# stablecabal/gyre

Measured on AMD Instinct MI355X. Metric: SD1.5 512px 50-step images/sec (node), higher is better.
Workload: dtype bf16

## Files before the change

gyre_amd/_lib.py:

```python
from __future__ import annotations

import ctypes as C
import os
from typing import Optional

import torch

_HERE = os.path.dirname(os.path.abspath(__file__))
MAX_LEVELS = 8

F32, BF16, F16 = 0, 1, 2
_TORCH_DTYPE = {torch.float32: F32, torch.bfloat16: BF16, torch.float16: F16}
LIB_PATHS = {BF16: os.environ.get("GYRE_HIP_LIB") or os.path.join(_HERE, "libgyre_hip.so"),
             F16: os.environ.get("GYRE_HIP_LIB_F16") or os.path.join(_HERE, "libgyre_hip_f16.so")}
LIB_PATH = LIB_PATHS[BF16]
_default_storage = F16 if os.environ.get("GYRE_STORAGE", "").lower() in ("f16", "fp16", "float16", "half") else BF16
STORAGE_TORCH_DTYPE = {BF16: torch.bfloat16, F16: torch.float16}


def default_storage() -> int:
    return _default_storage


def set_default_storage(storage: int) -> int:
    global _default_storage
    if storage not in LIB_PATHS:
        raise ValueError("storage must be _lib.BF16 or _lib.F16")
    old, _default_storage = _default_storage, storage
    return old


def storage_for(dtype: torch.dtype) -> int:
    return F16 if dtype == torch.float16 else BF16 if dtype == torch.bfloat16 else _default_storage


class GyreError(RuntimeError):
    pass


class UNetCfg(C.Structure):
    _fields_ = [("in_channels", C.c_int32), ("out_channels", C.c_int32), ("n_levels", C.c_int32),
                ("block_out_channels", C.c_int32 * MAX_LEVELS), ("layers_per_block", C.c_int32),
                ("attn_levels", C.c_int32 * MAX_LEVELS), ("num_heads", C.c_int32 * MAX_LEVELS),
                ("transformer_depth", C.c_int32 * MAX_LEVELS), ("cross_attention_dim", C.c_int32),
                ("norm_num_groups", C.c_int32), ("use_linear_projection", C.c_int32),
                ("flip_sin_to_cos", C.c_int32), ("freq_shift", C.c_float)]


class VAECfg(C.Structure):
    _fields_ = [("in_channels", C.c_int32), ("out_channels", C.c_int32), ("latent_channels", C.c_int32),
                ("n_levels", C.c_int32), ("block_out_channels", C.c_int32 * MAX_LEVELS),
                ("layers_per_block", C.c_int32), ("norm_num_groups", C.c_int32)]


class T2ICfg(C.Structure):
    _fields_ = [("kind", C.c_int32), ("cin", C.c_int32), ("channels", C.c_int32 * 4), ("n_levels", C.c_int32),
                ("nums_rb", C.c_int32), ("ksize", C.c_int32), ("sk", C.c_int32), ("use_conv", C.c_int32)]


class CtrlCfg(C.Structure):
    _fields_ = [("in_channels", C.c_int32), ("n_levels", C.c_int32), ("block_out_channels", C.c_int32 * MAX_LEVELS),
                ("layers_per_block", C.c_int32), ("attn_levels", C.c_int32 * MAX_LEVELS), ("num_heads", C.c_int32 * MAX_LEVELS),
                ("transformer_depth", C.c_int32 * MAX_LEVELS), ("cross_attention_dim", C.c_int32), ("norm_num_groups", C.c_int32),
                ("use_linear_projection", C.c_int32), ("flip_sin_to_cos", C.c_int32), ("freq_shift", C.c_float),
                ("cond_channels", C.c_int32), ("cond_embed_channels", C.c_int32 * 4)]


class RRDBCfg(C.Structure):
    _fields_ = [(n, C.c_int32) for n in ("num_in_ch", "num_out_ch", "num_feat", "num_block", "num_grow_ch", "scale", "plus")]


class SwinIRCfg(C.Structure):
    _fields_ = [("in_chans", C.c_int32), ("embed_dim", C.c_int32), ("num_layers", C.c_int32), ("depths", C.c_int32 * 16),
                ("num_heads", C.c_int32 * 16), ("window_size", C.c_int32), ("mlp_hidden", C.c_int32), ("upscale", C.c_int32),
                ("img_range", C.c_float), ("resi_3conv", C.c_int32)]


class RdbEpilogue(C.Structure):
    _fields_ = [("bias", C.c_void_p), ("alpha", C.c_float), ("act", C.c_int32), ("r1", C.c_void_p), ("ldr1", C.c_int32),
                ("beta1", C.c_float), ("r2", C.c_void_p), ("ldr2", C.c_int32), ("beta2", C.c_float)]


class RdbConvArgs(C.Structure):
    _fields_ = [("x", C.c_void_p)] + [(n, C.c_int32) for n in ("ldx", "Cin", "B", "H", "W", "ups")] + [("w", C.c_void_p)] + \
               [(n, C.c_int32) for n in ("w_rows", "NT", "N_live")] + [("out", C.c_void_p), ("c0", C.c_int32), ("ldo", C.c_int32),
                                                                        ("epi", C.POINTER(RdbEpilogue)), ("wpack", C.c_void_p),
                                                                        ("wpack_bytes", C.c_size_t)]


class GemmTestArgs(C.Structure):
    _fields_ = [(n, C.c_int32) for n in ("conv", "M", "K", "N", "geglu", "B", "Hi", "Wi", "Cin", "stride", "pad", "ups", "Hup", "Wup",
                                         "wrap", "C1", "lda", "lda2", "ldc", "ldr", "rows_per_sample", "ld_rowbias", "samples",
                                         "out_mode", "out_dtype", "tokens", "ldt", "colstat_unit")] + \
               [(n, C.c_void_p) for n in ("A", "A2", "W", "bias", "rowbias", "residual", "out", "ws")] + [("ws_bytes", C.c_size_t)] + \
               [("sc_A", C.c_void_p), ("sc_A2", C.c_void_p)] + [(n, C.c_int32) for n in ("sc_K", "sc_C1", "sc_lda", "sc_lda2")]


class LoraPair(C.Structure):
    _fields_ = [("up", C.c_void_p), ("down", C.c_void_p), ("dtype", C.c_int), ("rank", C.c_int), ("scale", C.c_float)]


class DeltaTerm(C.Structure):
    _fields_ = [("kind", C.c_int), ("up", C.c_void_p * 2), ("down", C.c_void_p * 2), ("dtype", C.c_int * 2), ("rank", C.c_int * 2),
                ("w1", C.c_void_p), ("O1", C.c_int), ("I1", C.c_int), ("scale", C.c_float)]


LORA_MAX_PAIRS = 8
DELTA_MAX_TERMS = 8
DELTA_LORA, DELTA_HADA, DELTA_KRON, DELTA_FULL = 0, 1, 2, 3
_vp, _i, _sz, _f = C.c_void_p, C.c_int, C.c_size_t, C.c_float
_SIGS = {
    "gyre_abi_version": (C.c_int, []),
    "gyre_storage_dtype": (C.c_int, []),
    "gyre_last_error": (C.c_char_p, []),
    "gyre_last_launch_count": (C.c_int64, []),
    "gyre_unet_create": (_i, [C.POINTER(UNetCfg), _i, C.POINTER(_vp)]),
    "gyre_unet_destroy": (None, [_vp]),
    "gyre_unet_num_params": (_i, [_vp]),
    "gyre_unet_param_key": (C.c_char_p, [_vp, _i]),
    "gyre_unet_set_weight": (_i, [_vp, C.c_char_p, _vp, _i, C.POINTER(C.c_int64), _i, _vp]),
    "gyre_unet_set_weight_lora": (_i, [_vp, C.c_char_p, _vp, _i, C.POINTER(C.c_int64), _i, _i, C.POINTER(LoraPair), _vp]),
    "gyre_unet_set_weight_delta": (_i, [_vp, C.c_char_p, _vp, _i, C.POINTER(C.c_int64), _i, _i, C.POINTER(DeltaTerm), _vp]),
    "gyre_unet_finalize": (_i, [_vp, _vp]),
    "gyre_unet_workspace_bytes": (_sz, [_vp, _i, _i, _i, _i]),
    "gyre_unet_forward": (_i, [_vp, _vp, _vp, _i, _vp, _vp, _i, _i, _i, _i, _i, _vp, _sz, _vp, _i]),
    "gyre_unet_set_context": (_i, [_vp, _vp, _vp, _i, _i, _i]),
    "gyre_unet_set_context_slot": (_i, [_vp, _vp, _vp, _i, _i, _i, _i]),
    "gyre_unet_select_context": (_i, [_vp, _i]),
    "gyre_unet_hint_uniform_timestep": (_i, [_vp, _i]),
    "gyre_unet_hint_cfg_pairs": (_i, [_vp, _i]),
    "gyre_unet_set_tome": (_i, [_vp, _i]),
    "gyre_unet_set_tiling": (_i, [_vp, _i]),
    "gyre_vae_set_tiling": (_i, [_vp, _i]),
    "gyre_unet_debug_tap": (_i, [_vp, C.c_char_p, _vp, _sz]),
    "gyre_unet_debug_grad_tap": (_i, [_vp, C.c_char_p, _vp, _sz]),
    "gyre_unet_forward_ex": (_i, [_vp, _vp, _vp, _i, _vp, _vp, _i, _i, _i, _i, _i, _vp, _sz, _vp, _i, _vp]),
    "gyre_unet_forward_ctrl": (_i, [_vp, _vp, _vp, _i, _vp, _vp, _i, _i, _i, _i, _i, _vp, _sz, _vp, _i, _vp,
                                    C.POINTER(_vp), _i, _i, _vp, C.POINTER(_vp), _i]),
    "gyre_unet_vjp_workspace_bytes": (_sz, [_vp, _i, _i, _i, _i]),
    "gyre_unet_vjp": (_i, [_vp, _vp, _vp, _i, _vp, _vp, _i, _i, _i, _i, _i, _vp, _i, _vp, _sz, _vp, _i, _vp, _i, _vp]),
    "gyre_unet_vjp_begin": (_i, [_vp, _vp, _vp, _i, _vp, _vp, _i, _i, _i, _i, _i, _vp, _sz, _vp, _i, _vp]),
    "gyre_unet_vjp_finish": (_i, [_vp, _vp, _vp, _i, _vp, _i]),
    "gyre_unet_vjp_finish_range": (_i, [_vp, _vp, _vp, _i, _vp, _i, _i, _i]),
    "gyre_unet_vjp_pending": (_i, [_vp]),
    "gyre_vae_create": (_i, [C.POINTER(VAECfg), _i, C.POINTER(_vp)]),
    "gyre_vae_destroy": (None, [_vp]),
    "gyre_vae_num_params": (_i, [_vp]),
    "gyre_vae_param_key": (C.c_char_p, [_vp, _i]),
    "gyre_vae_set_weight": (_i, [_vp, C.c_char_p, _vp, _i, C.POINTER(C.c_int64), _i, _vp]),
    "gyre_vae_finalize": (_i, [_vp, _vp]),
    "gyre_vae_workspace_bytes": (_sz, [_vp, _i, _i, _i, _i]),
    "gyre_vae_encode": (_i, [_vp, _vp, _vp, _i, _i, _i, _i, _vp, _sz, _vp, _i]),
    "gyre_vae_decode": (_i, [_vp, _vp, _vp, _i, _i, _i, _i, _vp, _sz, _vp, _i]),
    "gyre_vae_decode_vjp_workspace_bytes": (_sz, [_vp, _i, _i, _i]),
    "gyre_vae_decode_vjp": (_i, [_vp, _vp, _vp, _i, _i, _i, _i, _vp, _i, _vp, _sz, _vp, _i, _vp, _i]),
    "gyre_t2i_create": (_i, [C.POINTER(T2ICfg), _i, C.POINTER(_vp)]),
    "gyre_t2i_destroy": (None, [_vp]),
    "gyre_t2i_num_params": (_i, [_vp]),
    "gyre_t2i_param_key": (C.c_char_p, [_vp, _i]),
    "gyre_t2i_set_weight": (_i, [_vp, C.c_char_p, _vp, _i, C.POINTER(C.c_int64), _i, _vp]),
    "gyre_t2i_finalize": (_i, [_vp, _vp]),
    "gyre_t2i_workspace_bytes": (_sz, [_vp, _i, _i, _i]),
    "gyre_t2i_forward": (_i, [_vp, _vp, _vp, _i, _i, _i, _i, _vp, _sz, C.POINTER(_vp), _i, _i]),
    "gyre_rrdb_create": (_i, [C.POINTER(RRDBCfg), _i, C.POINTER(_vp)]),
    "gyre_rrdb_destroy": (None, [_vp]),
    "gyre_rrdb_num_params": (_i, [_vp]),
    "gyre_rrdb_param_key": (C.c_char_p, [_vp, _i]),
    "gyre_rrdb_set_weight": (_i, [_vp, C.c_char_p, _vp, _i, C.POINTER(C.c_int64), _i, _vp]),
    "gyre_rrdb_finalize": (_i, [_vp, _vp]),
    "gyre_rrdb_workspace_bytes": (_sz, [_vp, _i, _i, _i]),
    "gyre_rrdb_forward": (_i, [_vp, _vp, _vp, _i, _i, _i, _i, _vp, _sz, _vp, _i]),
    "gyre_rrdb_set_path": (_i, [_vp, _i]),
    "gyre_swinir_create": (_i, [C.POINTER(SwinIRCfg), _i, C.POINTER(_vp)]),
    "gyre_swinir_destroy": (None, [_vp]),
    "gyre_swinir_num_params": (_i, [_vp]),
    "gyre_swinir_param_key": (C.c_char_p, [_vp, _i]),
    "gyre_swinir_set_weight": (_i, [_vp, C.c_char_p, _vp, _i, C.POINTER(C.c_int64), _i, _vp]),
    "gyre_swinir_finalize": (_i, [_vp, _vp]),
    "gyre_swinir_workspace_bytes": (_sz, [_vp, _i, _i, _i]),
    "gyre_swinir_forward": (_i, [_vp, _vp, _vp, _i, _i, _i, _i, _vp, _sz, _vp, _i]),
    "gyre_ctrl_create": (_i, [C.POINTER(CtrlCfg), _i, C.POINTER(_vp)]),
    "gyre_ctrl_destroy": (None, [_vp]),
    "gyre_ctrl_num_params": (_i, [_vp]),
    "gyre_ctrl_param_key": (C.c_char_p, [_vp, _i]),
    "gyre_ctrl_set_weight": (_i, [_vp, C.c_char_p, _vp, _i, C.POINTER(C.c_int64), _i, _vp]),
    "gyre_ctrl_finalize": (_i, [_vp, _vp]),
    "gyre_ctrl_bind_workspace_bytes": (_sz, [_vp, _i, _i, _i, _i]),
    "gyre_ctrl_bind": (_i, [_vp, _vp, _vp, _i, _i, _i, _i, _vp, _i, _i, _i, _vp, _sz]),
    "gyre_ctrl_workspace_bytes": (_sz, [_vp, _i, _i, _i, _i]),
    "gyre_ctrl_forward": (_i, [_vp, _vp, _vp, _i, _vp, _i, _i, _i, _vp, _sz, C.POINTER(_f), _i, _i, _i, C.POINTER(_vp), _i, _i]),
    "gyre_prof_set_mask": (_i, [C.c_uint64]),
    "gyre_prof_num_classes": (_i, []),
    "gyre_prof_class_name": (C.c_char_p, [_i]),
    "gyre_prof_collect": (_i, [C.POINTER(C.c_int64), C.POINTER(C.c_double), C.POINTER(C.c_double), C.POINTER(C.c_double)]),
    "gyre_debug_force_gemm_cfg": (_i, [_i]),
    "gyre_debug_set_splitk_workspace": (_i, [_vp, _sz]),
    "gyre_debug_set_ar_workspace": (_i, [_vp, _sz]),
    "gyre_debug_set_wblk_workspace": (_i, [_vp, _sz]),
    "gyre_debug_attn_redo_count": (C.c_long, []),
    "gyre_debug_attn_plan": (_i, [_i] * 10 + [C.POINTER(C.c_int32)]),
    "gyre_debug_attn_bwd_plan": (_i, [_i] * 6 + [C.POINTER(C.c_int32)]),
    "gyre_debug_attn_tables": (_i, [_i, C.POINTER(C.c_int32), _i]),
    "gyre_debug_xattn_stamps": (_i, [_vp]),
    "gyre_debug_force_attn_variant": (_i, [_i]),
    "gyre_debug_gemm_ablation": (_i, [_i]),
    "gyre_debug_ln_linear_folds": (_i, [_i, _i, _i, _i]),
    "gyre_debug_gn_uses_small": (_i, [_i, _i, _i, _i]),
    "gyre_op_gemm_test": (_i, [_vp, C.POINTER(GemmTestArgs)]),
    "gyre_debug_gemm_plan": (_i, [C.POINTER(GemmTestArgs), C.POINTER(C.c_int32)]),
    "gyre_debug_gemm_tiles": (_i, [C.POINTER(C.c_int32), _i]),
    "gyre_set_batch_invariant": (_i, [_i]),
    "gyre_get_batch_invariant": (_i, []),
    "gyre_op_groupnorm": (_i, [_vp, _vp, _vp, _i, _i, _i, _i, _i, _vp, _vp, _f, _i, _vp, _sz, _vp]),
    "gyre_op_groupnorm_workspace": (_sz, [_i, _i, _i, _i]),
    "gyre_op_gemm_splitk_bytes": (_sz, [_i, _i, _i, _i, _i]),
    "gyre_op_conv3x3_colstats": (_i, [_vp, _vp, _i, _i, _i, _i, _vp, _i, _vp, _vp, _i, _i, _i, _vp, _vp, _sz, _vp, _sz, _vp]),
    "gyre_op_linear_colstats": (_i, [_vp, _vp, _i, _i, _vp, _i, _vp, _vp, _i, _i, _vp, _vp, _sz, _vp, _sz, _vp]),
    "gyre_op_groupnorm_colstats": (_i, [_vp, _vp, _vp, _i, _i, _i, _i, _i, _vp, _vp, _f, _i, _vp, _i, _vp, _i, _i, _vp, _sz, _vp]),
    "gyre_op_gn_fold": (_i, [_vp, _vp, _i, _i, _i, _i, _vp, _vp, _f, _vp, _vp, _i, _vp, _i, _i, _vp, _sz, _vp, _vp]),
    "gyre_op_layernorm": (_i, [_vp, _vp, _i, _i, _vp, _vp, _f, _vp]),
    "gyre_op_linear": (_i, [_vp, _vp, _i, _i, _vp, _i, _vp, _vp, _i, _vp]),
    "gyre_op_linear_t": (_i, [_vp, _vp, _i, _i, _vp, _i, _vp, _i, _i, _vp]),
    "gyre_op_ln_linear_workspace": (_sz, [_i, _i, _i]),
    "gyre_op_ln_linear": (_i, [_vp, _vp, _i, _i, _vp, _vp, _f, _vp, _i, _vp, _i, _i, _vp, _i, _vp, _i, _vp, _sz, _vp]),
    "gyre_op_linear_rowstats_parts": (_i, [_i, _i, _i, _i]),
    "gyre_op_linear_rowstats": (_i, [_vp, _vp, _i, _i, _vp, _i, _vp, _vp, _vp, _vp]),
    "gyre_op_conv3x3": (_i, [_vp, _vp, _i, _i, _i, _i, _vp, _i, _vp, _vp, _i, _i, _i, _vp]),
    "gyre_op_conv3x3_shortcut": (_i, [_vp, _vp, _i, _i, _i, _i, _vp, _i, _vp, _vp, _i, _vp, _i, _vp, _vp, _vp, _sz, _vp]),
    "gyre_op_compose_proj_out": (_i, [_vp, _vp, _vp, _vp, _vp, _i, _vp, _vp]),
    "gyre_op_conv3x3_nchw": (_i, [_vp, _vp, _i, _i, _i, _i, _vp, _i, _vp, _vp, _i, _i]),
    "gyre_op_repack_conv_weight": (_i, [_vp, _vp, _i, _i, _i, _i, _i, _vp]),
    "gyre_op_repack_conv_weight_scaled": (_i, [_vp, _vp, _i, _i, _i, _i, _i, _i, _f, _vp]),
    "gyre_op_repack_linear_weight": (_i, [_vp, _vp, _i, _i, _i, _vp]),
    "gyre_op_repack_bias": (_i, [_vp, _vp, _i, _i, _vp]),
    "gyre_op_repack_lora": (_i, [_vp, _vp, _i, _i, _i, _i, _i, _i, _i, _f, _i, C.POINTER(LoraPair), _vp]),
    "gyre_op_repack_delta": (_i, [_vp, _vp, _i, _i, _i, _i, _i, _i, _i, _f, _i, C.POINTER(DeltaTerm), _vp]),
    "gyre_op_lyco_core": (_i, [_vp, _vp, _i, _vp, _i, _i, _i, _i, _i, _vp]),
    "gyre_op_merge_delta": (_i, [_vp, _vp, _i, _i, _i, _i, C.POINTER(DeltaTerm), _vp, _i]),
    "gyre_op_attention": (_i, [_vp, _vp, _i, _vp, _i, _vp, _i, _i, _i, _i, _i, _i, _vp, _i]),
    "gyre_op_qkv": (_i, [_vp, _vp, _i, _i, _vp, _i, _vp, _vp, _i]),
    "gyre_op_attention_ex": (_i, [_vp, _vp, _i, _vp, _i, _vp, _i, _i, _i, _i, _i, _i, _vp, _i, _i]),
    "gyre_op_groupnorm_bwd_workspace": (_sz, [_i, _i, _i, _i]),
    "gyre_op_groupnorm_bwd": (_i, [_vp, _vp, _vp, _i, _i, _i, _i, _i, _vp, _vp, _f, _i, _vp, _vp, _vp, _sz, _vp, _vp]),
    "gyre_op_layernorm_bwd": (_i, [_vp, _vp, _vp, _i, _i, _vp, _f, _vp, _vp]),
    "gyre_op_geglu_bwd": (_i, [_vp, _vp, _vp, _i, _i, _vp]),
    "gyre_op_attention_bwd_workspace": (_sz, [_i, _i, _i, _i, _i]),
    "gyre_op_attention_bwd": (_i, [_vp, _vp, _i, _vp, _i, _vp, _i, _vp, _i, _vp, _i, _i, _i, _i, _i, _i, _i, _vp, _sz,
                                   _vp, _i, _vp, _i, _vp, _i]),
    "gyre_op_tome_workspace": (_sz, [_i, _i, _i]),
    "gyre_op_tome_merge": (_i, [_vp, _vp, _i, _vp, _i, _i, _i, _i, _i, _vp, _sz, _vp, _vp, _i, _vp, _vp]),
    "gyre_op_tome_merge_ex": (_i, [_vp, _vp, _i, _vp, _i, _i, _i, _i, _i, _vp, _sz, _vp, _vp, _i, _vp, _vp, _vp, _vp]),
    "gyre_op_tome_unmerge": (_i, [_vp, _vp, _i, _i, _i, _i, _vp, _vp, _vp, _vp, _i]),
    "gyre_op_timestep_embedding": (_i, [_vp, _vp, _i, _i, _i, _f, _vp]),
    "gyre_op_rowvec_linear": (_i, [_vp, _vp, _i, _i, _vp, _vp, _i, _i, _vp, _i]),
    "gyre_op_timestep_linear": (_i, [_vp, _vp, _i, _i, _i, _f, _vp, _vp, _vp, _i, _vp, _i]),
    "gyre_op_cross_attention_block": (_i, [_vp, _vp, _i, _i, _i, _i, _vp, _vp, _f, _vp, _vp, _vp, _i, _i, _vp, _vp, _vp, _sz, _vp, _vp]),
    "gyre_op_nchw_to_nhwc": (_i, [_vp, _vp, _i, _i, _i, _i, _i, _vp]),
    "gyre_op_copy_probe": (_i, [_vp, _vp, _vp, _sz]),
    "gyre_op_pixel_unshuffle8": (_i, [_vp, _vp, _i, _i, _i, _i, _i, _vp]),
    "gyre_op_avgpool2": (_i, [_vp, _vp, _i, _i, _i, _i, _vp]),
    "gyre_op_relu": (_i, [_vp, _vp, _sz]),
    "gyre_op_silu": (_i, [_vp, _vp, _sz]),
    "gyre_op_rdb_tile": (_i, [C.POINTER(C.c_int32), C.POINTER(C.c_int32)]),
    "gyre_op_rdb_conv": (_i, [_vp, C.POINTER(RdbConvArgs)]),
    "gyre_op_rdb_epilogue": (_i, [_vp, _vp, _i, _i, _i, _sz, C.POINTER(RdbEpilogue)]),
    "gyre_op_pixel_unshuffle": (_i, [_vp, _vp, _i, _i, _i, _i, _i, _i, _vp]),
    "gyre_op_win_bias": (_i, [_vp, _vp, _i, _vp]),
    "gyre_op_win_attn": (_i, [_vp, _vp, _i, _vp, _i, _vp, _i, _i, _i, _i, _i]),
    "gyre_op_ln_live": (_i, [_vp, _vp, _i, _sz, _i, _vp, _vp, _f, _vp, _i]),
    "gyre_op_swin_act": (_i, [_vp, _vp, _sz, _i, _f]),
    "gyre_op_swin_entry": (_i, [_vp, _vp, _i, _i, _sz, _vp, _f, _vp]),
    "gyre_op_swin_exit": (_i, [_vp, _vp, _i, _i, _sz, _vp, _f, _vp, _i]),
    "gyre_op_ctrl_emit": (_i, [_vp, _vp, _i, _i, _i, _i, _f, _i, _vp, _i, _i, _i]),
}
EXPORTED_SYMBOLS = tuple(_SIGS)

_libs: dict = {}
import threading as _threading
_tls = _threading.local()


def lib(storage: Optional[int] = None) -> C.CDLL:
    storage = _default_storage if storage is None else storage
    l = _libs.get(storage)
    if l is None:
        path = LIB_PATHS[storage]
        if not os.path.exists(path):
            raise GyreError(f"{path} is missing: run `python -c 'import __graft_entry__ as g; g.build()'` "
                            f"(hipcc --offload-arch=gfx950).  There is no non-HIP fallback.")
        try:
            l = C.CDLL(path, mode=getattr(os, "RTLD_LOCAL", 0) | getattr(os, "RTLD_NOW", 2))
        except OSError as e:
            raise GyreError(f"cannot load {path}: {e}") from e
# ... 67 lines not shown
```

gyre_amd/csrc/kernels.h:

```cpp
#pragma once
#include "common.h"

int launch_nchw_to_nhwc(hipStream_t st, const void* x, int dtype, int B, int C, int HW, int Cpad, bf16_t* y);
int launch_add_nchw_into_nhwc(hipStream_t st, const void* r, int dtype, int B, int C, int HW, int Cpad, bf16_t* y);
int launch_ctx_to_bf16(hipStream_t st, const void* x, int dtype, size_t n, bf16_t* y);
int launch_dup_batch(hipStream_t st, const void* src, void* dst, size_t outer, size_t inner_bytes);
int launch_add_f32(hipStream_t st, float* y, const float* x, size_t n);
int launch_compose_proj(hipStream_t st, const bf16_t* Wp, const bf16_t* W2, const float* b2, const float* bp, int C, bf16_t* Wc, float* bc);
int launch_verify_hints(hipStream_t st, const int64_t* t, int B, int check_t, const void* x, size_t bytes_per_half, int check_pairs, int* flag);
int launch_timestep_embedding(hipStream_t st, const int64_t* t, int B, int dim, int flip, float shift, float* out);
int launch_rowvec_linear(hipStream_t st, float* x, int B, int K, const bf16_t* W, const float* bias, int N,
                         int act_in_silu, float* out, int ldo);
int launch_timestep_linear(hipStream_t st, const int64_t* t, int B, int dim, int flip, float shift, float* emb_scratch,
                           const bf16_t* W, const float* bias, int N, float* out, int ldo);

struct GnParams {
    const bf16_t* x; const bf16_t* x2; int C1;
    int B, HW, C, G;
    const float* gamma; const float* beta; float eps; int silu;
    float* partial;
    float* scale_shift;
    int nchunks;
    bf16_t* y;
    float* mean_rstd = nullptr;
    const float* cs_x = nullptr; int cs_x_chunks = 0;
    const float* cs_x2 = nullptr; int cs_x2_chunks = 0;
    int cs_unit = 0;
};
size_t gn_workspace_bytes(int B, int HW, int C, int G);
int gn_pick_chunks(int B, int HW, int C);
int gemm_set_batch_invariant(int canonical_samples);
int gemm_get_batch_invariant();
long gemm_planner_state();
enum : int {
    GEMM_DBG_NO_SM            = 0x20,
    GEMM_DBG_SM_NO_SPLITK     = 0x40,
    GEMM_DBG_NO_SC_FOLD       = 0x80,
    GEMM_DBG_CONV_ZERO_PAGE   = 0x200,
    GEMM_DBG_NO_4S            = 0x400,
    GEMM_DBG_NO_LN_FOLD       = 0x800,
    GEMM_DBG_NO_GN_FOLD       = 0x1000,
    GEMM_DBG_NO_XATTN         = 0x2000,
    GEMM_DBG_NO_GEGLU_4S      = 0x4000,
    GEMM_DBG_LN_STATS_PASS    = 0x8000,
    GEMM_DBG_GEGLU_NO_LN_FOLD = 0x10000,
    GEMM_DBG_GN_STATS_PASS    = 0x20000,
    GEMM_DBG_NO_128x160       = 0x40000,
    GEMM_DBG_NO_CS_128x160    = 0x100000,
    GEMM_DBG_NO_AR            = 0x200000,
    GEMM_DBG_AR_ALL           = 0x400000,
    GEMM_DBG_NO_4S_128_TILES  = 0x800000,
    GEMM_DBG_TWO_STAGE_LINEAR = 0x1000000,
    GEMM_DBG_DEEP_RING        = 0x2000000,
    GEMM_DBG_NO_W_BLOCK       = 0x4000000,
    GEMM_DBG_TWO_STAGE_CONV   = 0x8000000,
    GEMM_DBG_NO_POUT_FOLD     = 0x10000000,
};
int launch_groupnorm_stats(hipStream_t st, const GnParams& p);
int launch_groupnorm_apply(hipStream_t st, const GnParams& p);
bool gn_use_small(int HW, int C, int C1, int G);
bool gn_accepts_colstats(const GnParams& p);
int launch_groupnorm_small(hipStream_t st, const GnParams& p);
int launch_gn_fold(hipStream_t st, const GnParams& p, const bf16_t* W, const float* bias, int N, bf16_t* Wf, float* bf);
int launch_layernorm(hipStream_t st, const bf16_t* x, int M, int C, const float* gamma, const float* beta, float eps,
                     bf16_t* y);
int launch_layernorm_stats(hipStream_t st, const bf16_t* x, int M, int C, float eps, float* stats);

int launch_nhwc_to_nchw_f32(hipStream_t st, const bf16_t* x, int B, int C, int HW, int Cpad, float* y);
int launch_repack_conv(hipStream_t st, const void* w, int dtype, int O, int I, int KH, int KW, int Ipad, bf16_t* out,
                       float scale = 1.f);
int launch_repack_linear(hipStream_t st, const void* w, int dtype, int O, int I, int geglu_interleave, bf16_t* out);
int launch_cast_f32(hipStream_t st, const void* w, int dtype, size_t n, int geglu_interleave, float* out, float scale = 1.f);
int launch_copy_probe(hipStream_t st, const void* src, void* dst, size_t bytes);
#define GYRE_LORA_MAX_PAIRS 8
struct LoraArgs {
    const void* up[GYRE_LORA_MAX_PAIRS];
    const void* down[GYRE_LORA_MAX_PAIRS];
    int dtype[GYRE_LORA_MAX_PAIRS];
    int rank[GYRE_LORA_MAX_PAIRS];
    float s[GYRE_LORA_MAX_PAIRS];
    int n = 0;
};
int launch_repack_lora(hipStream_t st, const void* base, int base_dtype, int O, int I, int KH, int KW, int Ipad, int geglu_interleave,
                       float scale_p, const LoraArgs& la, bf16_t* out);
#define GYRE_DELTA_MAX_TERMS 8
enum { DELTA_LORA = 0, DELTA_HADA = 1, DELTA_KRON = 2, DELTA_FULL = 3 };
struct DeltaArgs {
    int kind[GYRE_DELTA_MAX_TERMS];
    const void* up[GYRE_DELTA_MAX_TERMS][2];
    const void* down[GYRE_DELTA_MAX_TERMS][2];
    int dtype[GYRE_DELTA_MAX_TERMS][2];
    int rank[GYRE_DELTA_MAX_TERMS][2];
    const float* w1[GYRE_DELTA_MAX_TERMS];
    int O1[GYRE_DELTA_MAX_TERMS], I1[GYRE_DELTA_MAX_TERMS];
    float s[GYRE_DELTA_MAX_TERMS];
    int n = 0;
};
int launch_repack_delta(hipStream_t st, const void* base, int base_dtype, int O, int I, int KH, int KW, int Ipad, int geglu_interleave,
                        float scale_p, const DeltaArgs& da, bf16_t* out);
int launch_merge_delta(hipStream_t st, const void* base, int base_dtype, int O, int I, const DeltaArgs& da, void* out, int out_dtype);
int launch_lyco_core(hipStream_t st, const void* core, int core_dtype, const void* right, int right_dtype, int A, int B, int C, int T,
                     float* out);

int launch_pixel_unshuffle8(hipStream_t st, const void* x, int dtype, int B, int c, int H, int W, bf16_t* y);
int launch_avgpool2(hipStream_t st, const bf16_t* x, int B, int H, int W, int C, bf16_t* y);
int launch_relu(hipStream_t st, bf16_t* x, size_t n);
int launch_nhwc_to_nchw(hipStream_t st, const bf16_t* x, int B, int C, int HW, int Cpad, void* y, int dtype);

struct RdbEpilogueArgs {
    const float* bias = nullptr; float alpha = 1.f; int act = 0;
    const bf16_t* r1 = nullptr; int ldr1 = 0; float beta1 = 0.f;
    const bf16_t* r2 = nullptr; int ldr2 = 0; float beta2 = 0.f;
};
void rdb_tile(int* th, int* tw);
size_t rdb_wpack_bytes(int NT, int Cin);
int launch_rdb_wpack(hipStream_t st, const bf16_t* W, int rows, int Cin, int NT, bf16_t* wd);
int launch_rdb_conv(hipStream_t st, const bf16_t* x, int ldx, int Cin, int B, int H, int W, int ups, const bf16_t* wd, int NT,
                    int N_live, bf16_t* out, int ldo, const RdbEpilogueArgs& e);
int rdb_conv_check(const bf16_t* x, int ldx, int Cin, int B, int H, int W, int ups, const bf16_t* wd, int NT, int N_live,
                   const bf16_t* out, int ldo, const RdbEpilogueArgs& e);
int launch_rdb_epilogue(hipStream_t st, bf16_t* x, int ldo, int N_live, size_t npix, const RdbEpilogueArgs& e);
int launch_rdb_copy(hipStream_t st, const bf16_t* src, int lds, bf16_t* dst, int ldd, int C, size_t npix);
int rdb_unshuffle_channels(int c, int r);
int launch_pixel_unshuffle(hipStream_t st, const void* x, int dtype, int B, int c, int H, int W, int r, bf16_t* y);

int win_attn_check(const bf16_t* qkv, int ld_qkv, const bf16_t* o, int ld_o, const float* bias, int B, int H, int W, int heads, int shift);
int launch_win_attn(hipStream_t st, const bf16_t* qkv, int ld_qkv, bf16_t* o, int ld_o, const float* bias, int B, int H, int W, int heads,
                    int shift);
int launch_win_bias(hipStream_t st, const float* table, int heads, float* out);
int launch_ln_live(hipStream_t st, const bf16_t* x, int ldx, size_t M, int C, const float* gamma, const float* beta, float eps, bf16_t* y,
                   int ldy);
int launch_swin_act(hipStream_t st, bf16_t* x, size_t n, int mode, float slope);
int launch_swin_entry(hipStream_t st, const void* x, int dtype, int B, size_t HW, const float* mean3, float range, bf16_t* y);
int launch_swin_exit(hipStream_t st, const bf16_t* x, int ldx, int B, size_t HW, const float* mean3, float range, void* y, int dtype);

int launch_silu(hipStream_t st, bf16_t* x, size_t n);
int launch_ctrl_emit(hipStream_t st, const bf16_t* f, int B, int C, int HW, int Cpad, float scale, int accumulate, void* out,
                     int out_dtype, int out_B, int out_b0);

enum { GEMM_LINEAR = 0, GEMM_CONV3 = 1 };
enum { OUT_BF16 = 0, OUT_NCHW = 1, OUT_BF16_T = 2 };
struct GemmParams {
    const bf16_t* A = nullptr; const bf16_t* A2 = nullptr; int C1 = 0;
    int lda = 0, lda2 = 0;
    int mode = GEMM_LINEAR;
    int Hi = 0, Wi = 0, Cin = 0;
    int Ho = 0, Wo = 0, stride = 1, pad = 1, ups = 0;
    const bf16_t* W = nullptr; int K = 0; int N = 0; int M = 0;
    const float* bias = nullptr;
    const float* rowbias = nullptr;
    int rows_per_sample = 1; int ld_rowbias = 0;
    const bf16_t* residual = nullptr; int ldr = 0;
    int geglu = 0;
    void* out = nullptr; int ldc = 0; int out_mode = OUT_BF16; int out_dtype = 1;
    int tokens_per_batch = 0; int ldt = 0;
    bf16_t* vt_out = nullptr; int vt_col0 = 0;
    const bf16_t* zero_page = nullptr;
    int force_cfg = 0;
    int debug = 0;
    int Hup = 0, Wup = 0;
    int samples = 0;
    float* splitk_ws = nullptr; size_t splitk_ws_bytes = 0;
    int batch = 1; size_t bsA = 0, bsW = 0, bsC = 0;
    const float* ln_colsum = nullptr; const float* ln_stats = nullptr;
    float* rowstat_out = nullptr;
    const float* ln_parts = nullptr; int ln_nparts = 0; float ln_eps = 1e-5f;
    float* colstat_out = nullptr; int colstat_unit = 0;
    const void* w_packed = nullptr; int ar_ok = 0, no_ar = 0;
    const bf16_t* W_blk = nullptr;
    size_t w_sample_stride = 0;
    const bf16_t* sc_A = nullptr; const bf16_t* sc_A2 = nullptr; int sc_lda = 0, sc_lda2 = 0, sc_C1 = 0, sc_K = 0;
    int wrap = 0;
};
int launch_concat_rows(hipStream_t st, const bf16_t* a, int K1, const bf16_t* b, int K2, int N, bf16_t* out);
int launch_ln_fold(hipStream_t st, const bf16_t* W, int N, int K, const float* gamma, const float* beta, const float* bias,
                   bf16_t* Wf, float* colsum, float* bias_out);
size_t gemm_ar_packed_bytes(int N, int K);
int launch_ar_pack(hipStream_t st, const bf16_t* W, int N, int K, void* out);
int launch_w_block(hipStream_t st, const bf16_t* W, int N, int K, bf16_t* out);
bool conv_out_supports(int C, int O);
int launch_conv_out(hipStream_t st, const bf16_t* x, int B, int H, int W, int C, const bf16_t* Wt, const float* bias, int O,
                    void* out, int out_dtype);
struct GemmPlan {
    int cfg = 3, splits = 1;
    size_t ws_bytes = 0;
    int colstat_rows = 0;
    int rowstat_parts = 0;
    bool ln_fold = false;
    bool per_sample_w = false;
    bool shortcut_fold = false;
    bool w_block = false;
    bool ar_pack = false;
    int vt_align = 0;
};
GemmPlan gemm_plan(const GemmParams& p);
int launch_gemm(hipStream_t st, const GemmParams& p);
int launch_gemm(hipStream_t st, const GemmParams& p, const GemmPlan& plan);
void gemm_plan_loop_form(const GemmParams& p, const GemmPlan& plan, int* nst, int* uni);
int gemm_tile_table(int* out, int cap);


struct AttnParams {
    const bf16_t* q; int ldq;
    const bf16_t* k; int ldk;
    const bf16_t* vt; int ldvt;
    bf16_t* o; int ldo;
    int B, H, Nq, Nk, D;
    int k_prescaled = 0;
    int always_check = 0;
    unsigned* redo_counter = nullptr;
};
enum AttnVariant {
    ATTN_VAR_AUTO = 0,
    ATTN_VAR_V1 = 1,
    ATTN_VAR_V2_PLAIN = 2,
    ATTN_VAR_V2_FOLD = 3,
    ATTN_VAR_V2_Q64 = 4,
    ATTN_VAR_V3 = 5,
    ATTN_VAR_NO_QLOOP = 6,
    ATTN_VAR_ALWAYS_CHECK = 7,
    ATTN_VAR_AUTO_ALIAS = 8,
};
enum AttnFamily { ATTN_FAM_V1 = 0, ATTN_FAM_V2_PLAIN = 1, ATTN_FAM_V2_FOLD = 2, ATTN_FAM_V3 = 3 };
struct AttnPlan {
    int status = 0; std::string error;
    int family = 0, D = 0, QI = 0, row = -1;
    int PD = 0, slots = 0, stage_bytes = 0;
    int lds_bytes = 0;
    dim3 grid;
    bool qloop = false; int qiter = 1;
    bool always_check = false;
    int ablation = 0;
    double flops = 0, bytes = 0;
};
AttnPlan attn_plan(const AttnParams& p, int variant);
constexpr int ATTN_PLAN_INTS = 12, ATTN_BWD_PLAN_INTS = 10;
int launch_attention(hipStream_t st, const AttnParams& p);

struct XattnParams {
    const bf16_t* x; int ldx;
    const bf16_t* wq;
    const float* q_colsum; const float* q_bias;
    const float* ln_parts; int ln_nparts; const float* ln_stats; float ln_eps;
    const bf16_t* k; const bf16_t* vt; int ldvt;
    const bf16_t* wo; const float* bo;
    bf16_t* out; int ldo;
    float* rowstat_out;
    int M, rows_per_sample, Nk, heads;
};

bool xattn_supports(int C, int heads, int Nq, int Nk, int M);
int launch_xattn(hipStream_t st, const XattnParams& p, int C);

struct GnBwdParams {
    const bf16_t* x; const bf16_t* x2; int C1;
    int B, HW, C, G;
// ... 55 lines not shown
```

gyre_amd/csrc/kernels_gemm.hip:

```cpp
#include "gemm_shared.h"
#include <cstdio>
#include <cstdlib>
#include <cstdlib>
#include <atomic>
#include <utility>


typedef unsigned gemm_u32x4 __attribute__((ext_vector_type(4)));
__device__ __forceinline__ uint4 nt_load_u4(const void* p) {
    const gemm_u32x4 v = __builtin_nontemporal_load((const gemm_u32x4*)p);
    return make_uint4(v.x, v.y, v.z, v.w);
}

template <int MI, int NI>
__device__ __forceinline__ void gemm_epilogue(const GemmParams& p, f32x4_t (&acc)[MI][NI], int m_base, int n_base,
                                              int fr, int fq) {
#pragma unroll
    for (int i = 0; i < MI; ++i) {
        const int m = m_base + i * 16 + fr;
        if (m >= p.M) continue;
        const float* rbias = p.rowbias ? p.rowbias + (size_t)(m / p.rows_per_sample) * p.ld_rowbias : nullptr;
        if (p.geglu) {
#pragma unroll
            for (int j = 0; j + 1 < NI; j += 2) {
// ... 1086 lines not shown
    GyreProfScope prof_(kcls, st, 2.0 * p.M * (double)p.N * p.K,
                        a_bytes + (double)p.N * p.K * 2.0 + (double)p.M * n_out * 2.0 * (p.residual ? 2.0 : 1.0));
#define GYRE_GEMM8_GO(MODE_, UNI_)                                                                                  \
    do {                                                                                                            \
        auto kern = k_gemm8<BM, BN, WM, WN, MODE_, UNI_>;                                                             \
        static std::atomic<unsigned long long> attr_done{0};                                                                               \
        if (gyre_lds_attr_needed(attr_done))                                                                                            \
            (void)hipFuncSetAttribute((const void*)kern, hipFuncAttributeMaxDynamicSharedMemorySize, lds_attr);     \
        hipLaunchKernelGGL(kern, dim3(grid), dim3(512), lds, st, p, tiles_m, tiles_n, splits, nst);                      \
    } while (0)
    if (p.colstat_out && splits == 1) {
        if constexpr (BN == 320 || BN == 160) {
#define GYRE_GEMM8_CS(MODE_, UNI_)                                                                                  \
    do {                                                                                                            \
        auto kern = k_gemm8<BM, BN, WM, WN, MODE_, UNI_, false, false, true>;                                       \
        static std::atomic<unsigned long long> attr_done{0};                                                        \
        if (gyre_lds_attr_needed(attr_done))                                                                        \
            (void)hipFuncSetAttribute((const void*)kern, hipFuncAttributeMaxDynamicSharedMemorySize, lds_attr);     \
        hipLaunchKernelGGL(kern, dim3(grid), dim3(512), lds, st, p, tiles_m, tiles_n, splits, nst);                      \
    } while (0)
            if (p.mode == GEMM_LINEAR) GYRE_GEMM8_CS(GEMM_LINEAR, true);
            else if (uni) GYRE_GEMM8_CS(GEMM_CONV3, true);
            else GYRE_GEMM8_CS(GEMM_CONV3, false);
#undef GYRE_GEMM8_CS
        } else {
            GYRE_FAIL(-6, "gemm: column statistics exist for the 320- and 160-wide tiles only (see GemmPlan::colstat_rows)");
        }
    } else if (p.mode == GEMM_LINEAR && p.rowstat_out) {
        auto kern = k_gemm8<BM, BN, WM, WN, GEMM_LINEAR, true, false, true>;
        static std::atomic<unsigned long long> attr_done{0};
        if (gyre_lds_attr_needed(attr_done))
            (void)hipFuncSetAttribute((const void*)kern, hipFuncAttributeMaxDynamicSharedMemorySize, lds_attr);
        hipLaunchKernelGGL(kern, dim3(grid), dim3(512), lds, st, p, tiles_m, tiles_n, splits, nst);
    } else if (p.mode == GEMM_LINEAR && p.ln_colsum) {
        auto kern = k_gemm8<BM, BN, WM, WN, GEMM_LINEAR, true, true>;
        static std::atomic<unsigned long long> attr_done{0};
        if (gyre_lds_attr_needed(attr_done))
            (void)hipFuncSetAttribute((const void*)kern, hipFuncAttributeMaxDynamicSharedMemorySize, lds_attr);
        hipLaunchKernelGGL(kern, dim3(grid), dim3(512), lds, st, p, tiles_m, tiles_n, splits, nst);
    } else if (p.mode == GEMM_LINEAR) {
        GYRE_GEMM8_GO(GEMM_LINEAR, true);
    } else {
        if (uni) GYRE_GEMM8_GO(GEMM_CONV3, true); else GYRE_GEMM8_GO(GEMM_CONV3, false);
    }
#undef GYRE_GEMM8_GO
    GYRE_LAUNCH_CHECK();
    prof_.stop();
    if (splits > 1) return launch_splitk_reduce(st, p, splits);
    return 0;
}

static const GemmTile g_tiles[] = {
    {   1, 128, 128, GEMM_K_4W,  true,    0,   0,     false,   false,  false,       false,   false },
    {   2, 256,  64, GEMM_K_4W,  true,    0,   0,     false,   false,  false,       false,   false },
    {   3,  64,  64, GEMM_K_4W,  true,    0,   0,     false,   false,  false,       false,   false },
    {   4, 256, 320, GEMM_K_8W,  false, 160, 256,     true,    true,   true,        false,   true  },
    {   5, 128, 320, GEMM_K_8W,  false,  80, 128,     true,    true,   true,        false,   true  },
    {   6, 256, 256, GEMM_K_8W,  true,  128,   0,     true,    true,   true,        false,   true  },
    {   7, 128, 256, GEMM_K_8W,  true,   64,   0,     true,    true,   true,        false,   true  },
    {   8, 128, 160, GEMM_K_8W,  false,  80, 128,     true,    true,   true,        false,   true  },
    {  12, 256, 128, GEMM_K_8W,  true,    0,   0,     false,   false,  false,       false,   true  },
    {  20, 192, 320, GEMM_K_4S,  true,    0,   0,     false,   false,  false,       false,   true  },
    {  21, 256, 256, GEMM_K_4S,  true,    0,   0,     false,   false,  false,       false,   true  },
    {  22, 128, 320, GEMM_K_4S,  true,    0,   0,     false,   false,  false,       false,   true  },
    {  23, 128, 256, GEMM_K_4S,  true,    0,   0,     false,   false,  false,       false,   true  },
    {  24, 256, 320, GEMM_K_4S,  true,    0, 256,     false,   true,   false,       true,    true  },
    {  30, 256,  64, GEMM_K_AR,  true,   64,   0,     true,    true,   false,       false,   false },
    {  32,  64,  64, GEMM_K_SM,  false,  64,   0,     false,   false,  false,       false,   true  },
};
const GemmTile* gemm_tile(int cfg) {
    for (const GemmTile& t : g_tiles)
        if (t.id == cfg) return &t;
    return nullptr;
}
static thread_local void* g_dbg_ar_ws = nullptr;
static thread_local size_t g_dbg_ar_ws_bytes = 0;
static long ar_grid_min() {
    static const long v = getenv("GYRE_AR_GRID_MIN") ? atol(getenv("GYRE_AR_GRID_MIN")) : 192;
    return v;
}
static int pick_cfg(const GemmParams& p, int* splits_out) {
    *splits_out = 1;
    const bool trans = p.out_mode == OUT_BF16_T;
    auto tiles = [&](int bm, int bn) { return (long)((p.M + bm - 1) / bm) * ((p.N + bn - 1) / bn); };
    auto tiles_of = [&](int id) { const GemmTile* t = gemm_tile(id); return tiles(t->bm, t->bn); };
    auto eff = [&](long t, int slots) { long cap = 256L * slots; long waves = (t + cap - 1) / cap; return (double)t / (double)(waves * cap); };
    auto neff = [&](int bn) { long nt = (p.N + bn - 1) / bn; return (double)p.N / (double)(nt * bn); };
    auto meff = [&](int bm) { long mt = (p.M + bm - 1) / bm; return (double)p.M / (double)(mt * bm); };
    double best = -1; int cfg = 3;
    auto consider = [&](int id, double speed, int slots) {
        const GemmTile* t = gemm_tile(id);
        double s = speed * eff(tiles(t->bm, t->bn), slots) * neff(t->bn) * meff(t->bm);
        if (s > best) { best = s; cfg = id; }
    };
    consider(3, 0.30, 4);
    consider(1, 0.55, 2);
    consider(2, 0.50, 2);
    const bool wrap_only4 = p.mode == GEMM_CONV3 && p.wrap != 0;
    if (!trans && p.batch <= 1 && (p.ar_ok || p.w_packed || g_dbg_ar_ws) && !p.no_ar && !(p.debug & GEMM_DBG_NO_AR) && p.M >= 4096 &&
        (p.N >= 3 * p.K || (p.debug & GEMM_DBG_AR_ALL)) && gemm_ar_supports(p) &&
        ((long)((p.M + 255) / 256) * gemm_ar_nsplit(p) >= ar_grid_min() || (p.debug & GEMM_DBG_AR_ALL)))
        return 30;
    if (!trans && p.batch <= 1 && !wrap_only4) {
        auto big = [&](int id, double speed) { if (tiles_of(id) >= 160) consider(id, speed, 1); };
        if (!p.geglu && p.N % 320 == 0) { big(4, 0.92); big(5, 0.88); }
        if (!p.geglu && p.N % 160 == 0 && !(p.debug & GEMM_DBG_NO_128x160)) big(8, 0.90);
        if (p.N % 256 == 0) { big(6, 0.95); big(7, 0.62); }
        if (p.mode == GEMM_CONV3 && !p.geglu && p.N % 128 == 0 && p.N % 256 != 0 && p.N % 160 != 0 && !(p.debug & GEMM_DBG_NO_128x160)) big(12, 0.90);
        const int nk_ = (p.K + BK - 1) / BK;
        if (!(p.debug & GEMM_DBG_NO_4S) && p.N % 320 == 0 && (p.mode == GEMM_CONV3 ? nk_ >= 20 : nk_ >= 32) && gemm4s_supports(p, 24)) {
            big(24, 1.00);
            if (!(p.debug & GEMM_DBG_NO_4S_128_TILES) && p.mode == GEMM_CONV3 && nk_ >= 45 && tiles_of(24) >= 128 && tiles_of(24) < 160) consider(24, 1.25, 1);
        }
        else if (!(p.debug & (GEMM_DBG_NO_4S | GEMM_DBG_NO_GEGLU_4S)) && p.geglu && (long)p.N > (long)p.M && p.N % 320 == 0 && gemm4s_supports(p, 24))
            big(24, 1.00);
        const int nk = (p.K + BK - 1) / BK;
        if (p.out_mode == OUT_BF16 && !p.geglu && p.K >= 2048 && p.N % 4 == 0) {
            auto tryk = [&](int id, double speed) {
                const int bm = gemm_tile(id)->bm, bn = gemm_tile(id)->bn;
                long t = tiles(bm, bn);
                if (t >= 160 || t < 1) return;
                int sp = (int)((id == 8 ? 512 : 256) / t);
                const int min_steps = bm >= 256 ? 16 : 8;
                while (sp > 1 && nk / sp < min_steps) --sp;
                if (sp < 2) return;
                double sc = speed * eff(t * sp, 1) * neff(bn) * 0.85;
                if (sc > best) { best = sc; cfg = id; *splits_out = sp; }
            };
            if (p.N % 320 == 0) tryk(5, 0.88);
            if (p.N % 160 == 0 && !(p.debug & GEMM_DBG_NO_128x160)) tryk(8, 0.92);
            if (p.N % 256 == 0) tryk(7, 0.62);
            if (p.N % 320 == 0 && p.K >= 5000) {
                tryk(4, 1.05);
                if (!(p.debug & GEMM_DBG_NO_4S) && gemm4s_supports(p, 24)) tryk(24, 1.10);
            }
        }
    }
    if (!trans && !(p.debug & GEMM_DBG_NO_SM) && gemm_sm_supports(p)) {
        if (cfg <= 3 && *splits_out == 1) cfg = 32;
        else if (*splits_out > 1 && p.mode == GEMM_LINEAR && tiles_of(32) <= 512 && !(p.debug & GEMM_DBG_SM_NO_SPLITK)) { cfg = 32; *splits_out = 1; }
    }
    return cfg;
}

static thread_local int g_force_cfg = 0;
static thread_local float* g_dbg_ws = nullptr;
static thread_local size_t g_dbg_ws_bytes = 0;
static thread_local int g_gemm_debug = 0;
extern "C" int gyre_debug_gemm_ablation(int bits) { int old = g_gemm_debug; g_gemm_debug = bits; return old; }
extern "C" int gyre_debug_force_gemm_cfg(int cfg) { int old = g_force_cfg; g_force_cfg = cfg; return old; }
extern "C" int gyre_debug_set_splitk_workspace(void* ws, size_t bytes) { g_dbg_ws = (float*)ws; g_dbg_ws_bytes = bytes; return 0; }
extern "C" int gyre_debug_set_ar_workspace(void* ws, size_t bytes) { g_dbg_ar_ws = ws; g_dbg_ar_ws_bytes = bytes; return 0; }

static int pick_cfg_nosplit(const GemmParams& p) {
    GemmParams q = p; q.K = q.K < 2048 ? q.K : 2040;
    int sp; return pick_cfg(q, &sp);
}

static thread_local int g_invariant_batch = 0;
int gemm_set_batch_invariant(int n) { const int old = g_invariant_batch; g_invariant_batch = n < 0 ? 0 : n; return old; }
int gemm_get_batch_invariant() { return g_invariant_batch; }
long gemm_planner_state() {
    return (long)(unsigned)g_gemm_debug | ((long)(g_force_cfg & 0xffff) << 32) | ((long)(g_invariant_batch & 0xfff) << 48) | ((long)(g_dbg_ar_ws ? 1 : 0) << 60);
}

static int plan_cfg(const GemmParams& p, int* splits) {
    const int inv = g_invariant_batch;
    if (inv > 0 && p.samples > 0 && p.M % p.samples == 0) {
        GemmParams q = p;
        q.M = p.M / p.samples * inv;
        int c = pick_cfg(q, splits);
        if (*splits > 1) return c;
        return pick_cfg_nosplit(p);
    }
    return pick_cfg(p, splits);
}

static bool gemm_staged_epilogue_ok(const GemmParams& p) {
    const int n_out = p.geglu ? p.N / 2 : p.N;
    return p.out_mode == OUT_BF16 && (n_out % 8) == 0 && (p.ldc % 8) == 0 && (!p.residual || (p.ldr % 8) == 0) &&
           (((size_t)p.out | (size_t)p.residual) & 15) == 0;
}
static GemmParams gemm_normalised(const GemmParams& p0) {
    GemmParams p = p0;
    if (!p.force_cfg) p.force_cfg = g_force_cfg;
    p.debug = g_gemm_debug;
    if (!p.A2) { p.C1 = p.mode == GEMM_LINEAR ? p.K : p.Cin; p.A2 = p.A; p.lda2 = p.lda; }
    if (p.rows_per_sample <= 0) p.rows_per_sample = 1;
    if (p.sc_K && (!p.sc_A2 || p.sc_A2 == p.sc_A)) { p.sc_A2 = p.sc_A; p.sc_lda2 = p.sc_lda; p.sc_C1 = p.sc_K; }
    return p;
}

GemmPlan gemm_plan(const GemmParams& p0) {
    const GemmParams p = gemm_normalised(p0);
    GemmPlan pl;
    if (p.M <= 0 || p.N <= 0 || p.K <= 0) return pl;
    if (p.force_cfg) { pl.cfg = p.force_cfg & 0xff; pl.splits = std::max(1, (p.force_cfg >> 8) & 0xff); }
    else pl.cfg = plan_cfg(p, &pl.splits);
    if (pl.splits > 1) pl.ws_bytes = (size_t)pl.splits * p.M * p.N * sizeof(float);
    const GemmTile* t = gemm_tile(pl.cfg);
    if (!t) return pl;
    pl.vt_align = t->vt_align;
    pl.ar_pack = t->kind == GEMM_K_AR;
    pl.w_block = t->w_block && !(p.debug & GEMM_DBG_NO_W_BLOCK) && p.K % 64 == 0 && p.N % 8 == 0 && p.K > 1024 && p.batch <= 1 &&
                 !p.w_sample_stride && p.out_mode != OUT_BF16_T && (p.mode != GEMM_CONV3 || (p.Cin % 64 == 0 && p.C1 % 64 == 0));
    if (p.force_cfg || g_invariant_batch > 0 || p.batch > 1 || !gemm_staged_epilogue_ok(p)) return pl;
    const bool one_split = pl.splits == 1;
    const bool plain_linear = p.mode == GEMM_LINEAR && !p0.A2 && p.K % 8 == 0;
    pl.per_sample_w = t->per_sample_w && one_split && plain_linear && !(p.debug & GEMM_DBG_NO_GN_FOLD) && !p.geglu && !p.vt_out &&
                      !p.ln_colsum && p.N % 8 == 0 && p.M % p.rows_per_sample == 0 && p.rows_per_sample % t->bm == 0;
    pl.shortcut_fold = t->shortcut && !(p.debug & GEMM_DBG_NO_SC_FOLD) && p.mode == GEMM_CONV3 && p.sc_K && p.sc_K % BK == 0 &&
                       p.Cin % BK == 0 && p.C1 % BK == 0 && p.K == 9 * p.Cin + p.sc_K && p.stride == 1 && p.pad == 1 && !p.ups &&
                       p.Hi == p.Ho && p.Wi == p.Wo && !p.wrap;
    pl.ln_fold = t->ln_fold && one_split && plain_linear && !(p.debug & GEMM_DBG_NO_LN_FOLD) &&
                 !(p.geglu && ((p.debug & GEMM_DBG_GEGLU_NO_LN_FOLD) || !t->geglu)) && !p.rowbias && p.N % 4 == 0 &&
                 (!p.vt_out || (t->vt_align && p.vt_col0 % t->vt_align == 0));
    if (t->rowstats && one_split && plain_linear && !(p.debug & (GEMM_DBG_LN_STATS_PASS | GEMM_DBG_NO_LN_FOLD)) && !p.geglu &&
        !p.vt_out && !p.ln_colsum && p.N % 8 == 0)
        pl.rowstat_parts = t->kind == GEMM_K_AR ? gemm_ar_nsplit(p) : (p.N + t->bn - 1) / t->bn;
    const int unit = p.colstat_unit;
    if (unit > 0 && !(p.debug & GEMM_DBG_GN_STATS_PASS) && !p.geglu && !p.vt_out && !p.ln_colsum && !p.rowstat_out && p.K % 8 == 0 &&
        p.N % 8 == 0 && p.N % unit == 0 && 320 % unit == 0 && p.M % p.rows_per_sample == 0) {
        int rows = 0;
        if (!one_split) rows = cs_red_colblock(p.N, unit) <= 2048 ? cs_red_rows(p.rows_per_sample) : 0;
        else if (t->bn % unit == 0 && (t->kind != GEMM_K_4S || p.mode == GEMM_CONV3) && !(pl.cfg == 8 && (p.debug & GEMM_DBG_NO_CS_128x160)))
            rows = t->cs_rows;
        if (rows && p.rows_per_sample % rows == 0) pl.colstat_rows = rows;
    }
    return pl;
}

void gemm_plan_loop_form(const GemmParams& p0, const GemmPlan& plan, int* nst, int* uni) {
    const GemmParams p = gemm_normalised(p0);
    const GemmTile* t = gemm_tile(plan.cfg);
    *nst = 0; *uni = 0;
    if (!t) return;
    if (t->kind == GEMM_K_4W) *uni = p.mode == GEMM_CONV3 && gemm_conv_uniform_tap(p) ? 1 : 0;
    if (t->kind != GEMM_K_8W) return;
    bool u = true;
    gemm8_loop_form(p, t->bm, t->bn, plan.splits, nst, &u);
    *uni = p.mode == GEMM_CONV3 && u ? 1 : 0;
}
int gemm_tile_table(int* out, int cap) {
    int n = 0;
    for (const GemmTile& t : g_tiles) {
        if (4 * n + 4 <= cap) { out[4 * n] = t.id; out[4 * n + 1] = t.bm; out[4 * n + 2] = t.bn; out[4 * n + 3] = (int)t.kind; }
        ++n;
    }
    return n;
}

__global__ __launch_bounds__(256) void k_w_block(const bf16_t* __restrict__ W, int N, int K, bf16_t* __restrict__ out) {
    const size_t t = (size_t)blockIdx.x * 256 + threadIdx.x;
    const int kv = K >> 3;
    if (t >= (size_t)N * kv) return;
    const int n = (int)(t / kv), k = (int)(t - (size_t)n * kv) * 8;
    const uint4 v = *(const uint4*)(W + (size_t)n * K + k);
    *(uint4*)(out + ((size_t)(n >> 3) * (K >> 6) + (k >> 6)) * 512 + (n & 7) * 64 + (k & 63)) = v;
}
int launch_w_block(hipStream_t st, const bf16_t* W, int N, int K, bf16_t* out) {
    if (K % 64 || N % 8 || N < 8 || K < 64) GYRE_FAIL(-1, "w_block: K must be a multiple of 64 and N of 8");
    const size_t total = (size_t)N * (K / 8);
    hipLaunchKernelGGL(k_w_block, dim3((unsigned)((total + 255) / 256)), dim3(256), 0, st, W, N, K, out);
    GYRE_LAUNCH_CHECK();
    return 0;
}
static thread_local bf16_t* g_dbg_blk_ws = nullptr;
static thread_local size_t g_dbg_blk_ws_bytes = 0;
extern "C" int gyre_debug_set_wblk_workspace(void* ws, size_t bytes) { g_dbg_blk_ws = (bf16_t*)ws; g_dbg_blk_ws_bytes = bytes; return 0; }
int launch_gemm(hipStream_t st, const GemmParams& p0) { return launch_gemm(st, p0, gemm_plan(p0)); }
int launch_gemm(hipStream_t st, const GemmParams& p0, const GemmPlan& plan) {
    GemmParams p = gemm_normalised(p0);
    if (p.M <= 0 || p.N <= 0 || p.K <= 0) GYRE_FAIL(-1, "gemm: empty problem");
    if (p.K % 8) GYRE_FAIL(-1, "gemm: K must be a multiple of 8");
    if (p.C1 % 8) GYRE_FAIL(-1, "gemm: source split must be a multiple of 8");
    if (p.mode == GEMM_CONV3) {
        if (p.Cin % 8 || p.K != 9 * p.Cin + p.sc_K) GYRE_FAIL(-1, "conv3x3: Cin must be a multiple of 8 and K == 9*Cin (+ the folded shortcut's channels)");
        if (p.sc_K && (p.sc_K % BK || p.Cin % BK || !p.sc_A || p.stride != 1 || p.pad != 1 || p.ups || p.Hi != p.Ho || p.Wi != p.Wo || p.wrap ||
                       (p.sc_A2 && p.sc_A2 != p.sc_A && (p.sc_C1 <= 0 || p.sc_C1 >= p.sc_K || p.sc_C1 % BK))))
            GYRE_FAIL(-1, "conv3x3: a folded shortcut needs a stride-1 / pad-1 convolution and whole 64-channel steps on both sides");
    }
    if (p.out_mode == OUT_BF16 && (p.N % 4 || p.ldc % 4 || (p.residual && p.ldr % 4)))
        GYRE_FAIL(-1, "gemm: N / ldc / ldr must be multiples of 4 for bf16 row-major output");
    if (p.geglu && (p.N % 32)) GYRE_FAIL(-1, "gemm: GEGLU needs N % 32 == 0");
    if (p.out_mode == OUT_BF16_T && p.tokens_per_batch <= 0) GYRE_FAIL(-1, "gemm: tokens_per_batch required");
    if (p.batch > 1 && (p.mode != GEMM_LINEAR || p.out_mode != OUT_BF16 || p.bias || p.residual || p.rowbias || p.geglu || p.vt_out))
        GYRE_FAIL(-1, "gemm: the batched form is a plain bf16 matrix product");
    if (p.vt_out) {
        if (p.out_mode != OUT_BF16 || p.geglu || p.residual || p.tokens_per_batch <= 0 || p.tokens_per_batch % 8 || p.ldt % 8 ||
            p.vt_col0 <= 0 || p.vt_col0 >= p.N || p.N % 8)
            GYRE_FAIL(-1, "gemm: bad fused Q|K|V arguments");
    }
    if (p.rowstat_out && (p.ln_colsum || p.mode != GEMM_LINEAR || p0.A2 || p.geglu || p.vt_out || p.out_mode != OUT_BF16 || p.batch > 1))
        GYRE_FAIL(-1, "gemm: row statistics come from a plain single-source linear problem with bf16 row-major output");
    if (p.ln_colsum && (p.mode != GEMM_LINEAR || p0.A2 || !p.bias || (!p.ln_stats && p.ln_nparts <= 0) || (p.ln_nparts > 0 && !p.ln_parts) ||
                        p.rowbias || p.out_mode != OUT_BF16 || p.batch > 1))
        GYRE_FAIL(-1, "gemm: the folded LayerNorm needs a single-source linear problem with row statistics, bias and bf16 row-major output");
    {
        static const bool dump = getenv("GYRE_GEMM_DUMP") != nullptr;
        if (dump)
            fprintf(stderr, "GYRE_GEMM mode=%d M=%d N=%d K=%d Cin=%d C1=%d Hi=%d Wi=%d stride=%d ups=%d geglu=%d res=%d rowbias=%d "
                            "out=%d vt=%d batch=%d samples=%d cfg=%d splits=%d\n", p.mode, p.M, p.N, p.K, p.Cin, p.C1, p.Hi, p.Wi,
                    p.stride, p.ups, p.geglu, p.residual ? 1 : 0, p.rowbias ? 1 : 0, p.out_mode, p.vt_out ? 1 : 0, p.batch, p.samples,
                    plan.cfg, plan.splits);
    }
    int cfg = plan.cfg, splits = plan.splits;
    if (splits > 1) {
        if (!p.splitk_ws) { p.splitk_ws = g_dbg_ws; p.splitk_ws_bytes = g_dbg_ws_bytes; }
        if (!p.splitk_ws || p.splitk_ws_bytes < (size_t)splits * p.M * p.N * sizeof(float)) {
            splits = 1;
            cfg = pick_cfg_nosplit(p);
        }
    }
    const GemmTile* t = gemm_tile(cfg);
    if (!t) GYRE_FAIL(-1, "gemm: unknown tile config");
    if (p.vt_out && (!t->vt_align || splits > 1 || p.vt_col0 % t->vt_align))
        GYRE_FAIL(-6, "gemm: fused Q|K|V needs an 8-wave tile config whose wave tiles align with the V columns");
    if (p.colstat_out && (plan.colstat_rows <= 0 || splits != plan.splits))
        GYRE_FAIL(-6, "gemm: column statistics are not available for this problem / tile configuration (see GemmPlan::colstat_rows)");
    if (p.w_sample_stride && (!t->per_sample_w || splits > 1 || p.mode != GEMM_LINEAR || p.rows_per_sample % t->bm || p.M % p.rows_per_sample))
        GYRE_FAIL(-6, "gemm: per-sample weights need an unsplit 8-wave tile config whose row blocks do not straddle samples (GemmPlan::per_sample_w)");
    if (p.mode == GEMM_CONV3 && p.wrap && t->kind != GEMM_K_4W) GYRE_FAIL(-6, "gemm: circular padding (tiling) exists in the 4-wave tile configs only");
    if (p.sc_K && !t->shortcut) GYRE_FAIL(-6, "gemm: the folded shortcut exists in the pipelined 256x320 tile only (see GemmPlan::shortcut_fold)");
    if (!p.W_blk && g_dbg_blk_ws && plan.w_block && g_dbg_blk_ws_bytes >= (size_t)p.N * p.K * 2) {
        int rc = launch_w_block(st, p.W, p.N, p.K, g_dbg_blk_ws);
        if (rc) return rc;
        p.W_blk = g_dbg_blk_ws;
    }
    if (p.W_blk && (!t->w_block || p.K % 64 || p.N % 8 || p.w_sample_stride || (p.mode == GEMM_CONV3 && (p.Cin % 64 || p.C1 % 64)))) p.W_blk = nullptr;
    if (t->kind == GEMM_K_AR) {
        if (splits > 1 || !gemm_ar_supports(p)) GYRE_FAIL(-6, "gemm: problem outside the A-resident kernel's domain (K = 320 / 640 linear, bf16 row-major output)");
        const void* wpk = p.w_packed;
        if (!wpk) {
            if (!g_dbg_ar_ws || g_dbg_ar_ws_bytes < gemm_ar_packed_bytes(p.N, p.K))
                GYRE_FAIL(-6, "gemm: the A-resident kernel needs the packed weight copy (GemmParams::w_packed or gyre_debug_set_ar_workspace)");
            int rc = launch_ar_pack(st, p.W, p.N, p.K, g_dbg_ar_ws);
            if (rc) return rc;
            wpk = g_dbg_ar_ws;
        }
        return launch_gemm_ar(st, p, wpk);
    }
    if (t->kind == GEMM_K_SM) {
        if (splits > 1) GYRE_FAIL(-6, "gemm: the small-problem kernel has no split-K form");
        return launch_gemm_sm(st, p);
    }
    if (p.rowstat_out && (!t->rowstats || splits > 1 || !gemm_staged_epilogue_ok(p)))
        GYRE_FAIL(-6, "gemm: row statistics need an unsplit 8-wave tile config with the staged epilogue (see GemmPlan::rowstat_parts)");
    if (p.ln_colsum && (!t->ln_fold || splits > 1 || !gemm_staged_epilogue_ok(p)))
        GYRE_FAIL(-6, "gemm: the folded LayerNorm needs an unsplit 8-wave tile config with the staged epilogue (see GemmPlan::ln_fold)");
    if (t->kind != GEMM_K_4W) {
        if (p.out_mode == OUT_BF16_T) GYRE_FAIL(-6, "gemm: transposed output needs a 4-wave config");
        if (p.geglu && !t->geglu) GYRE_FAIL(-6, "gemm: GEGLU needs an even fragment count per wave");
        p.zero_page = gemm_zero_page_for_current_device();
        if (!p.zero_page) GYRE_FAIL(-5, "gemm: cannot allocate the zero page");
    }
    switch (cfg) {
        case 1: return launch_cfg<128, 128, 2, 2>(st, p);
        case 2: return launch_cfg<256, 64, 4, 1>(st, p);
        case 3: return launch_cfg<64, 64, 2, 2>(st, p);
        case 4: return launch_cfg8<256, 320, 4, 2>(st, p, KC_G8_CONV_256x320, splits);
        case 5: return launch_cfg8<128, 320, 2, 4>(st, p, KC_G8_CONV_128x320, splits);
        case 6: return launch_cfg8<256, 256, 4, 2>(st, p, KC_G8_CONV_256x256, splits);
        case 12:
            if (p.mode != GEMM_CONV3) GYRE_FAIL(-6, "gemm: the 256x128 tile is a convolution config");
            return launch_cfg8<256, 128, 4, 2>(st, p, KC_G8_X1, splits);
        case 7: return launch_cfg8<128, 256, 2, 4>(st, p, KC_G8_CONV_128x256, splits);
        case 8: return launch_cfg8<128, 160, 4, 2>(st, p, KC_G8_CONV_128x160, splits);
        default: return launch_gemm4s(st, p, cfg, splits);
    }
}
```

gyre_amd/csrc/kernels_gemm4s.hip:

```cpp
#include "gemm_shared.h"
#include <atomic>
#include <type_traits>

template <int V> using ic = std::integral_constant<int, V>;

__device__ __forceinline__ void glds_saddr(unsigned lds_addr, unsigned voff, const void* sbase) {
    asm volatile("s_mov_b32 m0, %0\n\ts_nop 0\n\tglobal_load_lds_dwordx4 %1, %2" ::"s"(lds_addr), "v"(voff), "s"(sbase) : "memory");
}
__device__ __forceinline__ void glds_vaddr(unsigned lds_addr, const void* vptr) {
    asm volatile("s_mov_b32 m0, %0\n\ts_nop 0\n\tglobal_load_lds_dwordx4 %1, off" ::"s"(lds_addr), "v"(vptr) : "memory");
}

typedef __attribute__((ext_vector_type(4))) int srd_t;
__device__ __forceinline__ void blds(unsigned lds_addr, unsigned voff, srd_t srd, unsigned soff) {
    asm volatile("s_mov_b32 m0, %0\n\ts_nop 0\n\tbuffer_load_dwordx4 %1, %2, %3 offen lds" ::"s"(lds_addr), "v"(voff), "s"(srd), "s"(soff) : "memory");
}
__device__ __forceinline__ srd_t make_srd(const void* base, unsigned bytes) {
    const size_t a = (size_t)base;
    return srd_t{(int)(unsigned)a, (int)(unsigned)(a >> 32), (int)bytes, 0x00020000};
}

template <int BM, int BN, int WM, int WN, int MODE, int ZFILL, bool LNF = false, bool CS = false>
__global__ __launch_bounds__(WM * WN * 64, WM * WN / 4) void k_gemm4s(GemmParams p, int tiles_m, int tiles_n, int splits, int group_m) {
    constexpr int NW = WM * WN;
    constexpr int TM = BM / WM, TN = BN / WN, MI = TM / 32, NI = TN / 32;
    constexpr int AP = BM / (8 * NW), BP = BN / (8 * NW);
    constexpr int DTOT = AP + BP, DH0 = (DTOT + 1) / 2;
    constexpr int STAGE = (BM + BN) * 128;
    static_assert((NW == 4 || NW == 8) && TM % 32 == 0 && TN % 32 == 0 && BM % (8 * NW) == 0 && BN % (8 * NW) == 0 &&
                  MI * NI * 16 <= (NW == 4 ? 256 : 160) && (NI == 4 || NI == 5), "tile shape");
    extern __shared__ __attribute__((aligned(16))) char smem[];

    const int ntiles = tiles_m * tiles_n;
    const int split = blockIdx.x / ntiles;
    const int bid = xcd_tile_id(blockIdx.x - split * ntiles, ntiles);
    int tm, tn;
    if ((long)p.M < (MODE == GEMM_CONV3 ? 9L : 1L) * p.N) { tn = bid / tiles_m; tm = bid - tn * tiles_m; }
    else {
        const int per = group_m * tiles_n;
        const int g = bid / per, r = bid - g * per;
        const int rows = min(group_m, tiles_m - g * group_m);
        tn = r / rows; tm = g * group_m + (r - tn * rows);
    }
    const int m0 = tm * BM, n0 = tn * BN;
    const int tid = threadIdx.x, lane = tid & 63;
    const int w = __builtin_amdgcn_readfirstlane(tid >> 6);
    const int wm = w / WN, wn = w - wm * WN;
    const int prow = lane >> 3;
    const int kvs = (lane & 7) ^ ((4 * (w & 1) + (lane >> 4)) & 7);
    const bf16_t* zero = p.zero_page;
    const unsigned lds0 = (unsigned)(size_t)(__attribute__((address_space(3))) char*)smem;
#ifdef GYRE_GEMM_ABLATIONS
    const bool abl_zero = p.debug & 1, abl_nodma = p.debug & 2, abl_a0 = p.debug & 8, abl_w0 = p.debug & 16;
#else
    constexpr bool abl_zero = false, abl_nodma = false, abl_a0 = false, abl_w0 = false;
#endif

    unsigned vo_w[BP];
#pragma unroll
    for (int i = 0; i < BP; ++i) {
        const int n = min(n0 + 8 * (w + NW * i) + prow, p.N - 1) - n0;
        vo_w[i] = p.W_blk ? (unsigned)(n >> 3) * (unsigned)(p.K >> 6) * 1024u + (unsigned)(n & 7) * 128u + kvs * 16u
                          : (unsigned)n * (unsigned)p.K * 2u + kvs * 16u;
    }
    const char* w_tile = p.W_blk ? (const char*)(p.W_blk + (size_t)(n0 >> 3) * (p.K >> 6) * 512) : (const char*)(p.W + (size_t)n0 * p.K);
    const bool wblk = p.W_blk != nullptr;
    unsigned vo_a[AP];
    int a_sbp[AP], a_y0[AP], a_x0[AP];
    const int hw_o = MODE == GEMM_CONV3 ? p.Ho * p.Wo : 1;
    const int ns0 = m0 / hw_o;
#pragma unroll
    for (int i = 0; i < AP; ++i) {
        const int row = m0 + 8 * (w + NW * i) + prow;
        if (MODE == GEMM_LINEAR) {
            const unsigned rl = (unsigned)(min(row, p.M - 1) - m0);
            vo_a[i] = rl * (unsigned)p.lda * 2u + kvs * 16u;
        } else {
            const int n = row / hw_o, rem = row - n * hw_o;
            const int oy = rem / p.Wo, ox = rem - oy * p.Wo;
            a_sbp[i] = (n - ns0) * p.Hi * p.Wi;
            a_y0[i] = row < p.M ? oy * p.stride - p.pad : 0x40000000;
            a_x0[i] = ox * p.stride - p.pad;
        }
    }
    const char* a_tile = (const char*)(p.A + (size_t)m0 * p.lda);
    int a_split = (MODE == GEMM_LINEAR && p.A2 != p.A) ? p.C1 : 0x7fffffff;
    const int Hlim = p.ups ? (p.Hup ? p.Hup : 2 * p.Hi) : p.Hi, Wlim = p.ups ? (p.Wup ? p.Wup : 2 * p.Wi) : p.Wi;
    const int ups = p.ups ? 1 : 0;
    const size_t spix = (size_t)ns0 * p.Hi * p.Wi;
    const char* cA = (const char*)(p.A + spix * p.lda);
    const char* cA2 = (const char*)(p.A2 + spix * p.lda2);
    srd_t srdA{}, srdA2{};
    if (MODE == GEMM_CONV3 && ZFILL == 0) {
        const size_t left = (size_t)(p.M / hw_o - ns0) * p.Hi * p.Wi;
        const size_t b1 = left * p.lda * 2, b2 = left * p.lda2 * 2;
        srdA = make_srd(cA, (unsigned)(b1 < 0x7ffffff0ull ? b1 : 0x7ffffff0ull));
        srdA2 = make_srd(cA2, (unsigned)(b2 < 0x7ffffff0ull ? b2 : 0x7ffffff0ull));
    }
    const int nk_conv = MODE == GEMM_CONV3 ? 9 * (p.Cin / BK) : 0;
    int src_C1 = p.C1;
    unsigned src_ld = (unsigned)p.lda * 2u, src_ld2 = (unsigned)p.lda2 * 2u;
    bool on_shortcut = false;
    struct StepSrc { const char* ab; const char* wb; srd_t srd; unsigned soff, ld2; int ky, kx; bool live, live_w; };
    auto step_src = [&](int kc, bool live0) {
        StepSrc s;
        const bool live = live0 && !abl_a0;
        s.live_w = live0 && !abl_w0;
        s.live = live;
        int kw;
        if (MODE == GEMM_LINEAR) {
            kw = kc * BK;
            if (kw >= a_split) {
                a_split = 0x7fffffff;
                a_tile = (const char*)(p.A2 + (size_t)m0 * p.lda2) - (size_t)p.C1 * 2;
#pragma unroll
                for (int i = 0; i < AP; ++i) {
                    const unsigned rl = (unsigned)(min(m0 + 8 * (w + NW * i) + prow, p.M - 1) - m0);
                    vo_a[i] = rl * (unsigned)p.lda2 * 2u + kvs * 16u;
                }
            }
            s.ab = live ? a_tile + (size_t)kw * 2 : (const char*)zero;
        } else {
            int c0;
            if (kc >= nk_conv && p.sc_K) {
                if (!on_shortcut) {
                    on_shortcut = true;
                    cA = (const char*)(p.sc_A + spix * p.sc_lda);
                    cA2 = (const char*)(p.sc_A2 + spix * p.sc_lda2);
                    src_C1 = p.sc_C1; src_ld = (unsigned)p.sc_lda * 2u; src_ld2 = (unsigned)p.sc_lda2 * 2u;
                    if (ZFILL == 0) {
                        const size_t left = (size_t)(p.M / hw_o - ns0) * p.Hi * p.Wi;
                        const size_t b1 = left * p.sc_lda * 2, b2 = left * p.sc_lda2 * 2;
                        srdA = make_srd(cA, (unsigned)(b1 < 0x7ffffff0ull ? b1 : 0x7ffffff0ull));
                        srdA2 = make_srd(cA2, (unsigned)(b2 < 0x7ffffff0ull ? b2 : 0x7ffffff0ull));
                    }
                }
                c0 = (kc - nk_conv) * BK;
                s.ky = p.pad; s.kx = p.pad;
                kw = 9 * p.Cin + c0;
            } else {
                const int chunk = kc / 9, tap = kc - chunk * 9;
                s.ky = tap / 3; s.kx = tap - s.ky * 3;
                c0 = chunk * BK;
                kw = tap * p.Cin + c0;
            }
            const bool first = c0 < src_C1;
            s.soff = (unsigned)(first ? c0 : c0 - src_C1) * 2u;
            s.ld2 = first ? src_ld : src_ld2;
            s.srd = first ? srdA : srdA2;
            s.ab = (first ? cA : cA2) + s.soff;
        }
        s.wb = s.live_w ? w_tile + (wblk ? (size_t)(kw >> 6) * 1024 : (size_t)kw * 2) : (const char*)zero;
        return s;
    };
    auto dma_piece = [&](const StepSrc& s, int buf, auto d_c) {
        constexpr int D = decltype(d_c)::value;
        if (abl_nodma) return;
        const unsigned dst = lds0 + buf * STAGE + w * 1024;
        if constexpr (D < AP) {
            constexpr int i = D;
            if (MODE == GEMM_LINEAR) {
                glds_saddr(dst + i * (NW * 1024), s.live ? +vo_a[i] : 0u, s.ab);
            } else {
#ifdef GYRE_GEMM_ABLATIONS
                if ((p.debug & 0x80) && (s.ky | s.kx)) return;
                if ((p.debug & 0x200) && s.kx) return;
#endif
                const int iy = a_y0[i] + s.ky, ix = a_x0[i] + s.kx;
                const bool ok = ((unsigned)iy < (unsigned)Hlim) & ((unsigned)ix < (unsigned)Wlim) & s.live;
                const unsigned pix = (unsigned)(a_sbp[i] + (iy >> ups) * p.Wi + (ix >> ups));
                const unsigned off = __umul24(pix, s.ld2) + kvs * 16u;
                if constexpr (ZFILL == 0) {
                    blds(dst + i * (NW * 1024), ok ? off : 0x80000000u, s.srd, s.soff);
                } else {
                    const char* ptr = s.ab + off;
                    glds_vaddr(dst + i * (NW * 1024), ok ? ptr : (const char*)zero);
                }
            }
        } else {
            constexpr int i = D - AP;
            glds_saddr(dst + BM * 128 + i * (NW * 1024), s.live_w ? +vo_w[i] : 0u, s.wb);
        }
    };
    auto dma_range = [&](const StepSrc& s, int buf, auto d0_c, auto d1_c) {
        constexpr int D0 = decltype(d0_c)::value, D1 = decltype(d1_c)::value;
        static_assert(D1 - D0 <= 9, "piece range");
        if constexpr (D0 + 0 < D1) dma_piece(s, buf, ic<D0 + 0>{});
        if constexpr (D0 + 1 < D1) dma_piece(s, buf, ic<D0 + 1>{});
        if constexpr (D0 + 2 < D1) dma_piece(s, buf, ic<D0 + 2>{});
        if constexpr (D0 + 3 < D1) dma_piece(s, buf, ic<D0 + 3>{});
        if constexpr (D0 + 4 < D1) dma_piece(s, buf, ic<D0 + 4>{});
        if constexpr (D0 + 5 < D1) dma_piece(s, buf, ic<D0 + 5>{});
        if constexpr (D0 + 6 < D1) dma_piece(s, buf, ic<D0 + 6>{});
        if constexpr (D0 + 7 < D1) dma_piece(s, buf, ic<D0 + 7>{});
        if constexpr (D0 + 8 < D1) dma_piece(s, buf, ic<D0 + 8>{});
    };

    f32x16_t acc[MI][NI];
#pragma unroll
    for (int i = 0; i < MI; ++i)
#pragma unroll
        for (int j = 0; j < NI; ++j)
#pragma unroll
            for (int e = 0; e < 16; ++e) acc[i][j][e] = 0.f;
    bf16x8_t af[2][MI], wf[2][NI];
    const unsigned lo = (unsigned)(lane & 31) * 128u + ((unsigned)((lane >> 5) ^ ((lane >> 1) & 7)) << 4);

    auto phase = [&](auto use_c, auto rd_c, auto ks_c, const char* sb_rd, auto half_c, const StepSrc& ss, int buf_dma) {
        constexpr int U = decltype(use_c)::value, R = decltype(rd_c)::value, KS = decltype(ks_c)::value;
        constexpr int H = decltype(half_c)::value;
        constexpr int RT = MI + NI;
        constexpr int DB = H == 1 ? DH0 : 0, DN = H == 1 ? DTOT - DH0 : DH0;
        const unsigned o = lo ^ (unsigned)(KS << 5);
        const char* pa = sb_rd + wm * (TM * 128) + o;
        const char* pw = sb_rd + BM * 128 + wn * (TN * 128) + o;
        auto chunk = [&](auto c_c) {
            constexpr int c = decltype(c_c)::value;
#pragma unroll
            for (int i = 0; i < MI; ++i)
                acc[i][c] = GYRE_MFMA_32x32x16(wf[U][c], af[U][i], acc[i][c], 0, 0, 0);
            if constexpr (R >= 0 && c < NI - 1) {
                constexpr int r0 = c * RT / (NI - 1), r1 = (c + 1) * RT / (NI - 1);
#pragma unroll
                for (int r = r0; r < r1; ++r) {
                    if (r < MI) af[R][r] = *(const bf16x8_t*)(pa + r * 4096);
                    else wf[R][r - MI] = *(const bf16x8_t*)(pw + (r - MI) * 4096);
                }
            }
            if constexpr (H >= 0) dma_range(ss, buf_dma, ic<DB + c * DN / NI>{}, ic<DB + (c + 1) * DN / NI>{});
            __builtin_amdgcn_sched_barrier(0);
        };
        chunk(ic<0>{}); chunk(ic<1>{}); chunk(ic<2>{}); chunk(ic<3>{});
        if constexpr (NI > 4) chunk(ic<4>{});
    };

    const int nk_all = (p.K + BK - 1) / BK;
    const int nk_per = (nk_all + splits - 1) / splits;
    const int kc0 = split * nk_per;
    const int nk = min(nk_all, kc0 + nk_per);

    {
        const StepSrc s0 = step_src(kc0, true);
        dma_range(s0, 0, ic<0>{}, ic<DH0>{});
        dma_range(s0, 0, ic<DH0>{}, ic<DTOT>{});
        asm volatile("s_waitcnt vmcnt(0)" ::: "memory");
        __builtin_amdgcn_s_barrier();
        const char* pa = smem + wm * (TM * 128) + lo;
        const char* pw = smem + BM * 128 + wn * (TN * 128) + lo;
#pragma unroll
        for (int i = 0; i < MI; ++i) af[0][i] = *(const bf16x8_t*)(pa + i * 4096);
#pragma unroll
        for (int j = 0; j < NI; ++j) wf[0][j] = *(const bf16x8_t*)(pw + j * 4096);
        const StepSrc s1 = step_src(kc0 + 1, kc0 + 1 < nk && !abl_zero);
        dma_range(s1, 1, ic<0>{}, ic<DH0>{});
    }
    const StepSrc none{};
    for (int kc = kc0; kc < nk; ++kc) {
        const int cur = (kc - kc0) & 1;
        const char* sb = smem + cur * STAGE;
        const StepSrc s1 = step_src(kc + 1, kc + 1 < nk && !abl_zero);
        phase(ic<0>{}, ic<1>{}, ic<1>{}, sb, ic<1>{}, s1, cur ^ 1);
        phase(ic<1>{}, ic<0>{}, ic<2>{}, sb, ic<-1>{}, none, 0);
        phase(ic<0>{}, ic<1>{}, ic<3>{}, sb, ic<-1>{}, none, 0);
        asm volatile("s_waitcnt vmcnt(0) lgkmcnt(0)" ::: "memory");
        __builtin_amdgcn_s_barrier();
        const StepSrc s2 = step_src(kc + 2, kc + 2 < nk && !abl_zero);
        phase(ic<1>{}, ic<0>{}, ic<0>{}, smem + (cur ^ 1) * STAGE, ic<0>{}, s2, cur);
    }
    asm volatile("s_waitcnt vmcnt(0) lgkmcnt(0)" ::: "memory");
    __builtin_amdgcn_s_barrier();

    const int hi = lane >> 5, l31 = lane & 31;
    const int m_base = m0 + wm * TM, n_base = n0 + wn * TN;
    if (!LNF && !CS && splits > 1) {
        float* slab = p.splitk_ws + (size_t)split * p.M * p.N;
#pragma unroll
        for (int i = 0; i < MI; ++i) {
            const int m = m_base + i * 32 + l31;
            if (m >= p.M) continue;
#pragma unroll
            for (int j = 0; j < NI; ++j)
#pragma unroll
                for (int g = 0; g < 4; ++g) {
                    const int n = n_base + j * 32 + 8 * g + 4 * hi;
                    if (n < p.N)
                        *(float4*)(slab + (size_t)m * p.N + n) =
                            make_float4(acc[i][j][4 * g], acc[i][j][4 * g + 1], acc[i][j][4 * g + 2], acc[i][j][4 * g + 3]);
                }
        }
        return;
    }
    if (!LNF && !CS && (p.debug & 4)) {
        float sum = 0.f;
#pragma unroll
        for (int i = 0; i < MI; ++i)
#pragma unroll
            for (int j = 0; j < NI; ++j)
#pragma unroll
                for (int e = 0; e < 16; ++e) sum += acc[i][j][e];
        if (sum == 12345.678f) ((float*)p.out)[0] = sum;
        return;
    }

    if constexpr (CS) {
        constexpr int NPC = (NI + 1) / 2, ROWC = 2 * 32 + 4, FST = 20;
        static_assert(64 * FST <= 32 * ROWC, "fold area exceeds the wave's slab");
        float* slabc = (float*)smem + w * (32 * ROWC);
        float2* cs_all = (float2*)((float*)smem + NW * 32 * ROWC);
        float2* chan = cs_all + NW * TN;
#pragma unroll
        for (int ps = 0; ps < NPC; ++ps) {
            const int j0 = 2 * ps, j1 = j0 + 2 < NI ? j0 + 2 : NI;
            const int vpr = (j1 - j0) * 4, R = 64 / vpr;
            const int c8 = lane & (vpr - 1), r0 = lane / vpr;
            const int nn = n_base + j0 * 32 + c8 * 8;
            float cs_s[8], cs_q[8];
#pragma unroll
            for (int e = 0; e < 8; ++e) { cs_s[e] = 0.f; cs_q[e] = 0.f; }
#pragma unroll
            for (int i = 0; i < MI; ++i) {
                const int m = m_base + i * 32 + l31;
                const float* rbias = (p.rowbias && m < p.M) ? p.rowbias + (size_t)(m / p.rows_per_sample) * p.ld_rowbias : nullptr;
#pragma unroll
                for (int j = j0; j < j1; ++j)
#pragma unroll
                    for (int g = 0; g < 4; ++g) {
                        const int n = n_base + j * 32 + 8 * g + 4 * hi;
                        float4 o = make_float4(acc[i][j][4 * g], acc[i][j][4 * g + 1], acc[i][j][4 * g + 2], acc[i][j][4 * g + 3]);
                        if (n < p.N) {
                            if (p.bias) { const float4 bv = *(const float4*)(p.bias + n); o.x += bv.x; o.y += bv.y; o.z += bv.z; o.w += bv.w; }
                            if (rbias) { const float4 tv = *(const float4*)(rbias + n); o.x += tv.x; o.y += tv.y; o.z += tv.z; o.w += tv.w; }
                        }
                        *(float4*)(slabc + l31 * ROWC + (j - j0) * 32 + 8 * g + 4 * hi) = o;
                    }
                for (int row = r0; row < 32; row += R) {
                    const int mm = m_base + i * 32 + row;
                    if (mm < p.M && nn < p.N) {
                        const float4 a = *(const float4*)(slabc + row * ROWC + c8 * 8);
                        const float4 b = *(const float4*)(slabc + row * ROWC + c8 * 8 + 4);
                        float f[8] = {a.x, a.y, a.z, a.w, b.x, b.y, b.z, b.w};
                        if (p.residual) {
                            float r[8];
                            unpack8(*(const uint4*)(p.residual + (size_t)mm * p.ldr + nn), r);
#pragma unroll
                            for (int e = 0; e < 8; ++e) f[e] += r[e];
                        }
                        const uint4 pk = pack8(f);
                        *(uint4*)((bf16_t*)p.out + (size_t)mm * p.ldc + nn) = pk;
                        unpack8(pk, f);
#pragma unroll
                        for (int e = 0; e < 8; ++e) { cs_s[e] += f[e]; cs_q[e] = fmaf(f[e], f[e], cs_q[e]); }
                    }
                }
            }
            __builtin_amdgcn_wave_barrier();
            float* fold = slabc + lane * FST;
            *(float4*)(fold) = make_float4(cs_s[0], cs_s[1], cs_s[2], cs_s[3]);
            *(float4*)(fold + 4) = make_float4(cs_s[4], cs_s[5], cs_s[6], cs_s[7]);
            *(float4*)(fold + 8) = make_float4(cs_q[0], cs_q[1], cs_q[2], cs_q[3]);
            *(float4*)(fold + 12) = make_float4(cs_q[4], cs_q[5], cs_q[6], cs_q[7]);
            __builtin_amdgcn_wave_barrier();
            if (lane < (j1 - j0) * 32) {
                const int cv = lane >> 3, e = lane & 7;
                float su = 0.f, sq = 0.f;
                for (int r = 0; r < R; ++r) { const float* src = slabc + (cv + vpr * r) * FST; su += src[e]; sq += src[8 + e]; }
                cs_all[w * TN + j0 * 32 + lane] = make_float2(su, sq);
            }
            __builtin_amdgcn_wave_barrier();
        }
        __syncthreads();
        for (int t = tid; t < BN; t += NW * 64) {
            const int wn_ = t / TN, col = t - wn_ * TN;
            float su = 0.f, sq = 0.f;
#pragma unroll
            for (int ww = 0; ww < WM; ++ww) { const float2 v = cs_all[(ww * WN + wn_) * TN + col]; su += v.x; sq += v.y; }
            chan[t] = make_float2(su, sq);
        }
        __syncthreads();
        const int unit = p.colstat_unit;
        for (int u = tid; u * unit < BN; u += NW * 64) {
            const int n = n0 + u * unit;
            if (n < p.N) {
                float su = 0.f, sq = 0.f;
                for (int c = 0; c < unit; ++c) { const float2 v = chan[u * unit + c]; su += v.x; sq += v.y; }
                ((float2*)p.colstat_out)[(size_t)tm * (p.N / unit) + n / unit] = make_float2(su, sq);
            }
        }
        return;
    }
    constexpr int NPASS = NW == 8 ? 2 : 1;
    constexpr int JP = (NI + NPASS - 1) / NPASS;
    constexpr int ROWF = JP * 32 + 4;
    static_assert((size_t)NW * 32 * ROWF * 4 <= 160 * 1024, "epilogue slabs exceed LDS");
    float* slab = (float*)smem + w * (32 * ROWF);
    const bool gg = p.geglu != 0;
    const int n_out = gg ? p.N / 2 : p.N;
#pragma unroll
    for (int i = 0; i < MI; ++i) {
        const int m = m_base + i * 32 + l31;
        const float* rbias = (p.rowbias && m < p.M) ? p.rowbias + (size_t)(m / p.rows_per_sample) * p.ld_rowbias : nullptr;
        float lrstd = 1.f, lrmu = 0.f;
        if constexpr (LNF) {
            if (m < p.M) {
                if (p.ln_nparts > 0) {
                    float su = 0.f, sq = 0.f;
                    for (int t = 0; t < p.ln_nparts; ++t) {
                        const float2 v = ((const float2*)p.ln_parts)[(size_t)t * p.M + m];
                        su += v.x; sq += v.y;
                    }
                    const float invk = 1.0f / (float)p.K;
                    const float mean = su * invk;
                    lrstd = 1.0f / sqrtf(fmaxf(sq * invk - mean * mean, 0.f) + p.ln_eps);
                    lrmu = lrstd * mean;
                } else {
                    const float2 rs = ((const float2*)p.ln_stats)[m];
                    lrstd = rs.x; lrmu = rs.y;
                }
            }
        }
        auto affine = [&](float a0, float a1, float a2, float a3, const float4& b, const float4& c) {
            if (LNF) return make_float4(fmaf(a0, lrstd, fmaf(-lrmu, c.x, b.x)), fmaf(a1, lrstd, fmaf(-lrmu, c.y, b.y)),
                                        fmaf(a2, lrstd, fmaf(-lrmu, c.z, b.z)), fmaf(a3, lrstd, fmaf(-lrmu, c.w, b.w)));
            return make_float4(a0 + b.x, a1 + b.y, a2 + b.z, a3 + b.w);
        };
#pragma unroll
        for (int ps = 0; ps < NPASS; ++ps) {
            constexpr int dummy = 0; (void)dummy;
            const int j0 = ps * JP, j1 = (ps + 1) * JP < NI ? (ps + 1) * JP : NI;
            if (gg) {
#pragma unroll
                for (int j = j0; j < j1; ++j)
#pragma unroll
                    for (int g = 0; g < 2; ++g) {
                        const int nin = n_base + j * 32 + 8 * g + 4 * hi;
                        float4 bv = make_float4(0, 0, 0, 0), bg = make_float4(0, 0, 0, 0), cv = bv, cg = bv;
                        if (p.bias && nin < p.N) { bv = *(const float4*)(p.bias + nin); bg = *(const float4*)(p.bias + nin + 16); }
                        if (LNF && nin < p.N) { cv = *(const float4*)(p.ln_colsum + nin); cg = *(const float4*)(p.ln_colsum + nin + 16); }
                        const float4 val = affine(acc[i][j][4 * g + 0], acc[i][j][4 * g + 1], acc[i][j][4 * g + 2], acc[i][j][4 * g + 3], bv, cv);
                        const float4 gate = affine(acc[i][j][4 * g + 8], acc[i][j][4 * g + 9], acc[i][j][4 * g + 10], acc[i][j][4 * g + 11], bg, cg);
                        float4 o;
                        o.x = val.x * gelu_erf_f(gate.x);
                        o.y = val.y * gelu_erf_f(gate.y);
                        o.z = val.z * gelu_erf_f(gate.z);
                        o.w = val.w * gelu_erf_f(gate.w);
                        *(float4*)(slab + l31 * ROWF + (j - j0) * 16 + 8 * g + 4 * hi) = o;
                    }
            } else {
#pragma unroll
                for (int j = j0; j < j1; ++j)
#pragma unroll
                    for (int g = 0; g < 4; ++g) {
                        const int n = n_base + j * 32 + 8 * g + 4 * hi;
                        float4 o = make_float4(acc[i][j][4 * g], acc[i][j][4 * g + 1], acc[i][j][4 * g + 2], acc[i][j][4 * g + 3]);
                        if (n < p.N) {
                            if (LNF) o = affine(o.x, o.y, o.z, o.w, *(const float4*)(p.bias + n), *(const float4*)(p.ln_colsum + n));
                            else if (p.bias) { const float4 bv = *(const float4*)(p.bias + n); o.x += bv.x; o.y += bv.y; o.z += bv.z; o.w += bv.w; }
                            if (rbias) { const float4 tv = *(const float4*)(rbias + n); o.x += tv.x; o.y += tv.y; o.z += tv.z; o.w += tv.w; }
                        }
                        *(float4*)(slab + l31 * ROWF + (j - j0) * 32 + 8 * g + 4 * hi) = o;
                    }
            }
            const int vpr = (j1 - j0) * (gg ? 2 : 4);
            const int n_pass = (gg ? n_base / 2 + j0 * 16 : n_base + j0 * 32);
            for (int v = lane; v < 32 * vpr; v += 64) {
                const int row = v / vpr, c8 = v - row * vpr;
                const int mm = m_base + i * 32 + row, nn = n_pass + c8 * 8;
                if (mm < p.M && nn < n_out) {
                    const float4 a = *(const float4*)(slab + row * ROWF + c8 * 8);
                    const float4 b = *(const float4*)(slab + row * ROWF + c8 * 8 + 4);
                    float f[8] = {a.x, a.y, a.z, a.w, b.x, b.y, b.z, b.w};
                    if (p.residual) {
                        float r[8];
                        unpack8(*(const uint4*)(p.residual + (size_t)mm * p.ldr + nn), r);
#pragma unroll
                        for (int e = 0; e < 8; ++e) f[e] += r[e];
                    }
                    *(uint4*)((bf16_t*)p.out + (size_t)mm * p.ldc + nn) = pack8(f);
                }
            }
        }
    }
}

bool gemm4s_supports(const GemmParams& p, int cfg) {
    const GemmTile* t = gemm_tile(cfg);
    if (!t || t->kind != GEMM_K_4S) return false;
    const int bn = t->bn;
    if (p.out_mode != OUT_BF16 || p.vt_out) return false;
    const int n_out = p.geglu ? p.N / 2 : p.N;
    if (n_out % 8 || p.ldc % 8 || (p.residual && p.ldr % 8) || (((size_t)p.out | (size_t)p.residual) & 15)) return false;
    if (p.N % 8) return false;
    if (p.geglu && p.N % 32) return false;
    const int c1 = p.A2 ? p.C1 : (p.mode == GEMM_LINEAR ? p.K : p.Cin);
    if (p.mode == GEMM_LINEAR) {
        if (p.K % BK) return false;
        if (p.A2 && p.A2 != p.A && (cfg != 24 || p.C1 <= 0 || p.C1 >= p.K || p.C1 % BK || p.lda2 % 8 || ((size_t)p.A2 & 15))) return false;
    }
    else if (p.Cin % BK || c1 % BK || p.K != 9 * p.Cin + p.sc_K || (p.sc_K && (p.sc_K % BK || cfg != 24))) return false;
    if (p.mode == GEMM_CONV3) {
        const size_t span = ((size_t)256 / ((size_t)p.Ho * p.Wo) + 2) * p.Hi * p.Wi;
        const size_t ld = p.lda > p.lda2 ? p.lda : p.lda2;
        if (span >= (1u << 24) || ld * 2 >= (1u << 24) || span * ld * 2 >= 0x7ff00000ull) return false;
    }
    if ((size_t)bn * p.K * 2 >= (1ull << 32) || (size_t)256 * (size_t)(p.lda > p.lda2 ? p.lda : p.lda2) * 2 >= (1ull << 32)) return false;
    return true;
}

template <int BM, int BN, int WM, int WN>
static int launch_cfg4s(hipStream_t st, const GemmParams& p, int kcls_base, int splits) {
    const int tiles_m = (p.M + BM - 1) / BM, tiles_n = (p.N + BN - 1) / BN;
    const int nk_all = (p.K + BK - 1) / BK;
    if (splits > nk_all) splits = nk_all;
    while (splits > 1 && (splits - 1) * ((nk_all + splits - 1) / splits) >= nk_all) --splits;
    const int grid = tiles_m * tiles_n * splits;
    constexpr int NW = WM * WN, NI = BN / WN / 32, JP = NW == 8 ? (NI + 1) / 2 : NI;
    constexpr size_t ring = (size_t)2 * (BM + BN) * 128,
                     epi = (size_t)NW * 32 * (JP * 32 + 4) * 4 + (size_t)(NW * (BN / WN) + BN) * 8;
    constexpr size_t lds = ring > epi ? ring : epi;
    int group_m = 1;
    if (tiles_n >= 2) { group_m = 32 / tiles_n; if (group_m < 1) group_m = 1; if (tiles_n >= 8) group_m = 4; }
    if (group_m > tiles_m) group_m = tiles_m;
    const int kcls = kcls_base + (p.mode == GEMM_CONV3 ? 0 : 1);
    const double n_out = p.geglu ? p.N / 2.0 : (double)p.N;
    const double a_bytes = p.mode == GEMM_CONV3 ? (double)(p.M / (p.Ho * p.Wo)) * p.Hi * p.Wi * p.Cin * 2.0
                                                : (double)p.M * p.K * 2.0;
    GyreProfScope prof_(kcls, st, 2.0 * p.M * (double)p.N * p.K,
                        a_bytes + (double)p.N * p.K * 2.0 + (double)p.M * n_out * 2.0 * (p.residual ? 2.0 : 1.0));
#define GYRE_GEMM4S_GO(MODE_, ZF_)                                                                                       \
    do {                                                                                                            \
        auto kern = k_gemm4s<BM, BN, WM, WN, MODE_, ZF_>;                                                                        \
        static std::atomic<unsigned long long> attr_done{0};                                                        \
        if (gyre_lds_attr_needed(attr_done))                                                                        \
            (void)hipFuncSetAttribute((const void*)kern, hipFuncAttributeMaxDynamicSharedMemorySize, (int)lds);     \
        hipLaunchKernelGGL(kern, dim3(grid), dim3(NW * 64), lds, st, p, tiles_m, tiles_n, splits, group_m);             \
    } while (0)
    if (p.mode == GEMM_LINEAR && p.ln_colsum) {
        if constexpr (BM == 256 && BN == 320 && NW == 8) {
            auto kern = k_gemm4s<BM, BN, WM, WN, GEMM_LINEAR, 0, true>;
            static std::atomic<unsigned long long> attr_done{0};
            if (gyre_lds_attr_needed(attr_done))
                (void)hipFuncSetAttribute((const void*)kern, hipFuncAttributeMaxDynamicSharedMemorySize, (int)lds);
            hipLaunchKernelGGL(kern, dim3(grid), dim3(NW * 64), lds, st, p, tiles_m, tiles_n, splits, group_m);
        } else {
            GYRE_FAIL(-6, "gemm: the folded LayerNorm exists for the 8-wave 256x320 pipelined tile only");
        }
    } else if (p.colstat_out && splits == 1) {
        if constexpr (BM == 256 && BN == 320 && NW == 8) {
            if (p.mode != GEMM_CONV3) GYRE_FAIL(-6, "gemm: the pipelined tile emits column statistics for convolutions only");
            auto kern = k_gemm4s<BM, BN, WM, WN, GEMM_CONV3, 0, false, true>;
            static std::atomic<unsigned long long> attr_done{0};
            if (gyre_lds_attr_needed(attr_done))
                (void)hipFuncSetAttribute((const void*)kern, hipFuncAttributeMaxDynamicSharedMemorySize, (int)lds);
            hipLaunchKernelGGL(kern, dim3(grid), dim3(NW * 64), lds, st, p, tiles_m, tiles_n, splits, group_m);
        } else {
            GYRE_FAIL(-6, "gemm: column statistics exist for the 8-wave 256x320 pipelined tile only");
        }
    } else if (p.mode == GEMM_LINEAR) GYRE_GEMM4S_GO(GEMM_LINEAR, 0);
#ifndef GYRE_GEMM_ABLATIONS
    else if (p.debug & GEMM_DBG_CONV_ZERO_PAGE) GYRE_GEMM4S_GO(GEMM_CONV3, 1);
#endif
    else GYRE_GEMM4S_GO(GEMM_CONV3, 0);
#undef GYRE_GEMM4S_GO
    GYRE_LAUNCH_CHECK();
    prof_.stop();
    if (splits > 1) return launch_splitk_reduce(st, p, splits);
    return 0;
}

int launch_gemm4s(hipStream_t st, const GemmParams& p, int cfg, int splits) {
    if (!gemm4s_supports(p, cfg)) GYRE_FAIL(-6, "gemm: the one-wave-per-SIMD tile configs need K in whole 64-channel steps and bf16 row-major output");
    switch (cfg) {
        case 20: return launch_cfg4s<192, 320, 2, 2>(st, p, KC_G4S_192x320, splits);
        case 21: return launch_cfg4s<256, 256, 2, 2>(st, p, KC_G4S_256x256, splits);
        case 22: return launch_cfg4s<128, 320, 2, 2>(st, p, KC_G4S_128x320, splits);
        case 23: return launch_cfg4s<128, 256, 2, 2>(st, p, KC_G4S_128x256, splits);
        case 24: return launch_cfg4s<256, 320, 4, 2>(st, p, KC_G4S_256x320, splits);
    }
    GYRE_FAIL(-1, "gemm: unknown tile config");
}
```

gyre_amd/csrc/model.hip:

```cpp
#include "model_impl.h"

static thread_local std::string g_err;
static thread_local int64_t g_launches = 0;
void gyre_set_error(const std::string& msg) { g_err = msg; }
int64_t& gyre_launch_counter() { return g_launches; }
extern "C" const char* gyre_last_error(void) { return g_err.c_str(); }
extern "C" int gyre_abi_version(void) { return GYRE_ABI_VERSION; }
extern "C" int gyre_storage_dtype(void) { return GYRE_STORAGE_DTYPE; }
extern "C" int64_t gyre_last_launch_count(void) { return g_launches; }

namespace {
struct ProfRec { hipEvent_t a, b; int kclass; double flops, bytes; };
struct ProfState {
    unsigned long long mask = 0;
    std::vector<ProfRec> recs;
    std::vector<std::pair<hipEvent_t, hipEvent_t>> pool;
};
thread_local ProfState g_prof;
static_assert(KC_COUNT <= 64, "profiler mask is 64 bits wide");
}
GyreProfScope::GyreProfScope(int kclass, hipStream_t st, double flops, double bytes) : st_(st) {
    if (!(g_prof.mask >> kclass & 1ull)) return;
    hipEvent_t a, b;
    if (!g_prof.pool.empty()) { a = g_prof.pool.back().first; b = g_prof.pool.back().second; g_prof.pool.pop_back(); }
// ... 680 lines not shown
        const int Hin = a->ups ? (a->Hup ? a->Hup : 2 * a->Hi) : a->Hi, Win = a->ups ? (a->Wup ? a->Wup : 2 * a->Wi) : a->Wi;
        if (Hin + (a->pad ? 2 : 1) < 3 || Win + (a->pad ? 2 : 1) < 3) GYRE_FAIL(GYRE_ERR_INVALID, "gemm_test: image smaller than the window");
        const int Ho = (Hin + (a->pad ? 2 : 1) - 3) / a->stride + 1, Wo = (Win + (a->pad ? 2 : 1) - 3) / a->stride + 1;
        if ((long)a->B * Ho * Wo > lim) GYRE_FAIL(GYRE_ERR_INVALID, "gemm_test: too many output pixels");
        M = a->B * Ho * Wo; K = 9 * a->Cin; width = a->Cin;
        p.mode = GEMM_CONV3; p.Hi = a->Hi; p.Wi = a->Wi; p.Cin = a->Cin; p.Ho = Ho; p.Wo = Wo; p.stride = a->stride; p.pad = a->pad;
        p.ups = a->ups; p.Hup = a->ups ? a->Hup : 0; p.Wup = a->ups ? a->Wup : 0; p.wrap = a->wrap;
        p.samples = a->B; p.rows_per_sample = Ho * Wo;
        if (a->samples && a->samples != a->B) GYRE_FAIL(GYRE_ERR_INVALID, "gemm_test: samples of a convolution is B");
        if (a->rows_per_sample && a->rows_per_sample != Ho * Wo) GYRE_FAIL(GYRE_ERR_INVALID, "gemm_test: rows_per_sample of a convolution is Ho * Wo");
    } else {
        if (a->M <= 0 || a->K <= 0 || a->M > lim || a->K > lim || a->K % 8) GYRE_FAIL(GYRE_ERR_INVALID, "gemm_test: M and K must be positive, K a multiple of 8");
        if (a->out_mode == OUT_NCHW) GYRE_FAIL(GYRE_ERR_INVALID, "gemm_test: NCHW output is a convolution form");
        M = a->M; K = a->K; width = a->K;
        p.mode = GEMM_LINEAR; p.rows_per_sample = a->rows_per_sample > 0 ? a->rows_per_sample : 1;
        if (M % p.rows_per_sample) GYRE_FAIL(GYRE_ERR_INVALID, "gemm_test: rows_per_sample must divide M");
        p.samples = a->samples;
        if (a->samples && M % a->samples) GYRE_FAIL(GYRE_ERR_INVALID, "gemm_test: samples must divide M");
    }
    if (a->sc_K < 0 || a->sc_K > 65536 || a->sc_C1 < 0 || a->sc_lda < 0 || a->sc_lda2 < 0 || a->sc_lda > lim || a->sc_lda2 > lim)
        GYRE_FAIL(GYRE_ERR_INVALID, "gemm_test: negative or oversized shortcut field");
    if (a->sc_K) {
        if (!a->conv || a->sc_K % 8) GYRE_FAIL(GYRE_ERR_INVALID, "gemm_test: the folded shortcut belongs to a convolution, sc_K a multiple of 8");
        if (need_device_pointers && !a->sc_A) GYRE_FAIL(GYRE_ERR_INVALID, "gemm_test: null shortcut source");
        p.sc_A = (const bf16_t*)a->sc_A; p.sc_K = a->sc_K; p.sc_C1 = a->sc_K; p.sc_lda = a->sc_lda ? a->sc_lda : a->sc_K;
        if (a->sc_A2) {
            if (a->sc_C1 <= 0 || a->sc_C1 >= a->sc_K || a->sc_C1 % 8) GYRE_FAIL(GYRE_ERR_INVALID, "gemm_test: sc_C1 must be a multiple of 8 inside sc_K");
            p.sc_A2 = (const bf16_t*)a->sc_A2; p.sc_C1 = a->sc_C1; p.sc_lda = a->sc_lda ? a->sc_lda : a->sc_C1;
            p.sc_lda2 = a->sc_lda2 ? a->sc_lda2 : a->sc_K - a->sc_C1;
            if (p.sc_lda2 < a->sc_K - a->sc_C1 || p.sc_lda2 % 8 || ((size_t)a->sc_A2 & 15)) GYRE_FAIL(GYRE_ERR_INVALID, "gemm_test: bad second shortcut source");
        }
        if (p.sc_lda < p.sc_C1 || p.sc_lda % 8 || ((size_t)a->sc_A & 15)) GYRE_FAIL(GYRE_ERR_INVALID, "gemm_test: bad shortcut source stride / alignment");
        K += a->sc_K;
    }
    p.M = M; p.K = K; p.N = n_w; p.geglu = a->geglu;
    p.A = (const bf16_t*)a->A; p.W = (const bf16_t*)a->W; p.lda = a->lda ? a->lda : width;
    if (a->A2) {
        if (a->C1 <= 0 || a->C1 >= width || a->C1 % 8) GYRE_FAIL(GYRE_ERR_INVALID, "gemm_test: C1 must be a multiple of 8 inside the A rows");
        p.A2 = (const bf16_t*)a->A2; p.C1 = a->C1; p.lda2 = a->lda2 ? a->lda2 : width - a->C1;
        if (p.lda < a->C1 || p.lda2 < width - a->C1) GYRE_FAIL(GYRE_ERR_INVALID, "gemm_test: lda / lda2 below the width of their source");
        if (p.lda2 % 8 || ((size_t)a->A2 & 15)) GYRE_FAIL(GYRE_ERR_INVALID, "gemm_test: the second source needs 16-byte rows");
    } else if (p.lda < width) GYRE_FAIL(GYRE_ERR_INVALID, "gemm_test: lda below the width of the A rows");
    if (p.lda % 8 || ((size_t)a->A & 15) || ((size_t)a->W & 15)) GYRE_FAIL(GYRE_ERR_INVALID, "gemm_test: A and W need 16-byte rows");
    p.bias = a->bias; p.residual = (const bf16_t*)a->residual; p.out = a->out; p.out_mode = a->out_mode; p.out_dtype = a->out_dtype;
    p.ldc = a->ldc ? a->ldc : n_out; p.ldr = a->ldr ? a->ldr : n_out;
    if (a->out_mode == OUT_BF16 && (p.ldc < n_out || (a->residual && p.ldr < n_out))) GYRE_FAIL(GYRE_ERR_INVALID, "gemm_test: ldc / ldr below N");
    if (a->out_mode != OUT_BF16 && (a->residual || a->geglu || a->rowbias)) GYRE_FAIL(GYRE_ERR_INVALID, "gemm_test: residual / GEGLU / row bias need 16-bit row-major output");
    if (((size_t)a->out & 7) || ((size_t)a->residual & 7) || ((size_t)a->bias & 15))
        GYRE_FAIL(GYRE_ERR_INVALID, "gemm_test: out / residual need 8-byte, bias 16-byte alignment");
    if (a->rowbias) {
        if (a->geglu) GYRE_FAIL(GYRE_ERR_INVALID, "gemm_test: no row bias with GEGLU");
        p.rowbias = a->rowbias; p.ld_rowbias = a->ld_rowbias ? a->ld_rowbias : n_out;
        if (p.ld_rowbias < n_out || p.ld_rowbias % 4 || ((size_t)a->rowbias & 15)) GYRE_FAIL(GYRE_ERR_INVALID, "gemm_test: ld_rowbias below N or rows not 16-byte aligned");
    }
    if (a->out_mode == OUT_BF16_T) {
        if (a->tokens <= 0 || M % a->tokens || a->ldt < a->tokens) GYRE_FAIL(GYRE_ERR_INVALID, "gemm_test: tokens must divide M, ldt >= tokens");
        p.tokens_per_batch = a->tokens; p.ldt = a->ldt;
    }
    p.colstat_unit = a->colstat_unit;
    if (a->ws && a->ws_bytes) { p.splitk_ws = (float*)a->ws; p.splitk_ws_bytes = a->ws_bytes; }
    return 0;
}
int gyre_op_gemm_test(void* st, const gyre_gemm_test_args* a) {
    GemmParams p;
    TRY(gemm_test_problem(p, a, true));
    p.colstat_unit = 0;
    const GemmPlan pl = gemm_plan(p);
    if (pl.splits > 1 && (!p.splitk_ws || p.splitk_ws_bytes < pl.ws_bytes))
        GYRE_FAIL(GYRE_ERR_WORKSPACE, "gemm_test: the plan runs in K slices and needs ws_bytes of slab space in ws (gyre_debug_gemm_plan)");
    return launch_gemm((hipStream_t)st, p, pl);
}
int gyre_debug_gemm_plan(const gyre_gemm_test_args* a, int32_t* out) {
    if (!out) GYRE_FAIL(GYRE_ERR_INVALID, "gemm_plan: null output");
    GemmParams p;
    TRY(gemm_test_problem(p, a, false));
    const GemmPlan pl = gemm_plan(p);
    int nst = 0, uni = 0;
    gemm_plan_loop_form(p, pl, &nst, &uni);
    out[0] = pl.cfg; out[1] = pl.splits; out[2] = (int32_t)(pl.ws_bytes & 0xffffffffu); out[3] = (int32_t)(pl.ws_bytes >> 32);
    out[4] = pl.w_block ? 1 : 0; out[5] = pl.colstat_rows; out[6] = pl.rowstat_parts; out[7] = pl.ln_fold ? 1 : 0;
    out[8] = pl.per_sample_w ? 1 : 0; out[9] = pl.shortcut_fold ? 1 : 0; out[10] = nst; out[11] = uni;
    return 0;
}
int gyre_debug_gemm_tiles(int32_t* out, int cap) { return gemm_tile_table(out, out ? cap : 0); }
int gyre_op_ln_linear(void* st, const void* x, int M, int K, const float* gamma, const float* beta, float eps, const void* w,
                      int N, const float* bias, int geglu, int qkv_tokens, void* vt_out, int ldt, const float* row_parts,
                      int n_parts, void* ws, size_t ws_bytes, void* y) {
    if (!x || !w || !y || !gamma || !beta || !ws) GYRE_FAIL(GYRE_ERR_INVALID, "null argument");
    GemmParams p;
    if (qkv_tokens > 0 && (!vt_out || M % qkv_tokens || N != 3 * K || geglu)) GYRE_FAIL(GYRE_ERR_INVALID, "bad fused Q|K|V arguments");
    ln_linear_problem(p, M, K, N, geglu, qkv_tokens, ldt);
    p.A = (const bf16_t*)x; p.W = (const bf16_t*)w; p.bias = bias; p.out = y;
    if (qkv_tokens > 0) p.vt_out = (bf16_t*)vt_out;
    if (ws_bytes < gyre_op_ln_linear_workspace(p.N, K, M)) GYRE_FAIL(GYRE_ERR_WORKSPACE, "ln_linear: workspace too small");
    if (!gemm_plan(p).ln_fold) GYRE_FAIL(GYRE_ERR_UNSUPPORTED, "ln_linear: the planner's kernel for this shape cannot fold the LayerNorm");
    bf16_t* wf = (bf16_t*)ws;
    float* cs = (float*)((char*)ws + align_up((size_t)p.N * K * 2, 256));
    float* bb = (float*)((char*)cs + align_up((size_t)p.N * 4, 256));
    TRY(launch_ln_fold((hipStream_t)st, p.W, p.N, K, gamma, beta, bias, wf, cs, bb));
    if (row_parts && n_parts > 0) {
        p.ln_parts = row_parts; p.ln_nparts = n_parts; p.ln_eps = eps;
    } else {
        float* stats = (float*)((char*)bb + align_up((size_t)p.N * 4, 256));
        TRY(launch_layernorm_stats((hipStream_t)st, p.A, M, K, eps, stats));
        p.ln_stats = stats;
    }
    p.W = wf; p.bias = bb; p.ln_colsum = cs;
    return launch_gemm((hipStream_t)st, p);
}
int gyre_op_attention_ex(void* st, const void* q, int ldq, const void* k, int ldk, const void* vt, int ldvt, int B,
                         int heads, int Nq, int Nk, int D, void* o, int ldo, int k_prescaled) {
    if (!q || !k || !vt || !o) GYRE_FAIL(GYRE_ERR_INVALID, "null argument");
    AttnParams a;
    a.q = (const bf16_t*)q; a.ldq = ldq; a.k = (const bf16_t*)k; a.ldk = ldk; a.vt = (const bf16_t*)vt; a.ldvt = ldvt;
    a.o = (bf16_t*)o; a.ldo = ldo; a.B = B; a.H = heads; a.Nq = Nq; a.Nk = Nk; a.D = D; a.k_prescaled = k_prescaled ? 1 : 0;
    return launch_attention((hipStream_t)st, a);
}
int gyre_op_cross_attention_block(void* st, const void* x, int M, int tokens, int C, int heads, const float* gamma, const float* beta,
                                  float eps, const void* wq, const void* k, const void* vt, int Nk, int ldvt, const void* wo,
                                  const float* bo, void* ws, size_t ws_bytes, void* out, float* row_stats) {
    if (!x || !gamma || !beta || !wq || !k || !vt || !wo || !ws || !out) GYRE_FAIL(GYRE_ERR_INVALID, "null argument");
    if (tokens <= 0 || M % tokens) GYRE_FAIL(GYRE_ERR_INVALID, "cross_attention_block: M must be a multiple of tokens");
    if (!xattn_supports(C, heads, tokens, Nk, M)) GYRE_FAIL(GYRE_ERR_UNSUPPORTED, "cross_attention_block: shape outside the fused kernel's domain");
    if (ws_bytes < gyre_op_ln_linear_workspace(C, C, M)) GYRE_FAIL(GYRE_ERR_WORKSPACE, "cross_attention_block: workspace too small");
    bf16_t* wf = (bf16_t*)ws;
    float* cs = (float*)((char*)ws + align_up((size_t)C * C * 2, 256));
    float* bb = (float*)((char*)cs + align_up((size_t)C * 4, 256));
    float* stats = (float*)((char*)bb + align_up((size_t)C * 4, 256));
    TRY(launch_ln_fold((hipStream_t)st, (const bf16_t*)wq, C, C, gamma, beta, nullptr, wf, cs, bb));
    TRY(launch_layernorm_stats((hipStream_t)st, (const bf16_t*)x, M, C, eps, stats));
    XattnParams xp;
    xp.x = (const bf16_t*)x; xp.ldx = C; xp.wq = wf; xp.q_colsum = cs; xp.q_bias = bb;
    xp.ln_parts = nullptr; xp.ln_nparts = 0; xp.ln_stats = stats; xp.ln_eps = eps;
    xp.k = (const bf16_t*)k; xp.vt = (const bf16_t*)vt; xp.ldvt = ldvt; xp.wo = (const bf16_t*)wo; xp.bo = bo;
    xp.out = (bf16_t*)out; xp.ldo = C; xp.rowstat_out = row_stats; xp.M = M; xp.rows_per_sample = tokens; xp.Nk = Nk; xp.heads = heads;
    return launch_xattn((hipStream_t)st, xp, C);
}
int gyre_op_nchw_to_nhwc(void* st, const void* x, int dtype, int B, int C, int HW, int Cpad, void* y) {
    if (!x || !y) GYRE_FAIL(GYRE_ERR_INVALID, "null argument");
    return launch_nchw_to_nhwc((hipStream_t)st, x, dtype, B, C, HW, Cpad, (bf16_t*)y);
}
int gyre_op_copy_probe(void* st, const void* src, void* dst, size_t bytes) {
    if (!src || !dst) GYRE_FAIL(GYRE_ERR_INVALID, "null argument");
    return launch_copy_probe((hipStream_t)st, src, dst, bytes);
}

}
```

gyre_amd/csrc/model_impl.h:

```cpp
#pragma once
#include "../../include/gyre_hip.h"
#include "kernels.h"
#include <cstdlib>
#include <cstdio>
#include <cmath>

#include <algorithm>
#include <array>
#include <cstring>
#include <map>
#include <memory>
#include <string>
#include <unordered_map>
#include <vector>

#define TRY(expr) do { int rc_ = (expr); if (rc_) return rc_; } while (0)

static_assert(GYRE_DELTA_LORA == DELTA_LORA && GYRE_DELTA_HADA == DELTA_HADA && GYRE_DELTA_KRON == DELTA_KRON && GYRE_DELTA_FULL == DELTA_FULL,
              "term kinds of the C ABI and of the kernel");
static inline int delta_terms_to_args(int n_terms, const gyre_delta_term* terms, DeltaArgs& da) {
    if (n_terms < 0 || n_terms > GYRE_DELTA_MAX_TERMS || (n_terms > 0 && !terms)) GYRE_FAIL(GYRE_ERR_INVALID, "0 to 8 delta terms per call");
    da.n = n_terms;
    for (int j = 0; j < n_terms; ++j) {
        da.kind[j] = terms[j].kind;
        for (int q = 0; q < 2; ++q) {
            da.up[j][q] = terms[j].up[q]; da.down[j][q] = terms[j].down[q]; da.dtype[j][q] = terms[j].dtype[q]; da.rank[j][q] = terms[j].rank[q];
        }
        da.w1[j] = terms[j].w1; da.O1[j] = terms[j].O1; da.I1[j] = terms[j].I1; da.s[j] = terms[j].scale;
    }
    return 0;
}
static inline size_t align_up(size_t v, size_t a) { return (v + a - 1) / a * a; }
static inline int pad8(int c) { return (c + 7) / 8 * 8; }

struct Arena {
    char* base = nullptr;
    size_t cap = 0, peak = 0;
    bool dry = false;
    std::map<size_t, size_t> free_;
    void reset(char* b, size_t c, bool d) {
        base = b; cap = c; dry = d; peak = 0;
        free_.clear();
        free_[0] = d ? ((size_t)1 << 60) : c;
    }
    size_t alloc(size_t bytes) {
        bytes = align_up(bytes ? bytes : 1, 256);
        for (auto it = free_.begin(); it != free_.end(); ++it) {
            if (it->second >= bytes) {
                size_t off = it->first, rem = it->second - bytes;
                free_.erase(it);
                if (rem) free_[off + bytes] = rem;
                peak = std::max(peak, off + bytes);
                return off;
            }
        }
        return (size_t)-1;
    }
    void release(size_t off, size_t bytes) {
        bytes = align_up(bytes ? bytes : 1, 256);
        auto it = free_.emplace(off, bytes).first;
        auto nx = std::next(it);
        if (nx != free_.end() && it->first + it->second == nx->first) { it->second += nx->second; free_.erase(nx); }
        if (it != free_.begin()) {
            auto pv = std::prev(it);
            if (pv->first + pv->second == it->first) { pv->second += it->second; free_.erase(it); }
        }
    }
};

struct Tn {
    bf16_t* p = nullptr; size_t off = (size_t)-1, bytes = 0;
    int B = 0, H = 0, W = 0, C = 0;
    float* cs = nullptr; size_t cs_off = (size_t)-1, cs_bytes = 0; int cs_chunks = 0, cs_unit = 0;
    int rows() const { return B * H * W; }
    bool valid() const { return off != (size_t)-1; }
};

enum ParamKind { PK_CONV3 = 0, PK_MAT = 1, PK_VEC = 2, PK_MAT_GEGLU = 3, PK_VEC_GEGLU = 4,
                 PK_MAT_HEAD30 = 5, PK_VEC_HEAD30 = 6, PK_TABLE_F32 = 7 };
struct Param {
    std::string key;
    std::vector<int64_t> shape;
    int kind = PK_VEC;
    int o_pad = 0, i_pad = 0;
    void* dev = nullptr;
    float scale = 1.f;
    bool set = false;
};

struct Store {
    int device = 0;
    std::vector<std::unique_ptr<Param>> params;
    std::unordered_map<std::string, Param*> by_key;
    std::vector<void*> allocs;
    uint64_t weights_version = 1;
    enum Kind {
        DC_TRANSPOSED,
        DC_LN_FOLD,
        DC_PACKED,
        DC_BLOCKED,
        DC_SHORTCUT,
        DC_PROJ_OUT,
        DC_WIN_BIAS,
        DC_RDB_CHUNKED
    };
    struct DKey {
        int kind; const void* src;
        bool operator==(const DKey& o) const { return kind == o.kind && src == o.src; }
    };
    struct DKeyHash { size_t operator()(const DKey& k) const { return std::hash<const void*>()(k.src) * 31 + (size_t)k.kind; } };
    struct Derived { void* p = nullptr; size_t bytes = 0; uint64_t version = 0; int tag = 0; };
    std::unordered_map<DKey, Derived, DKeyHash> derived_;
    void* derived(Kind kind, const void* src, size_t bytes, bool* fresh, int tag = 0) {
        Derived& en = derived_[DKey{kind, src}];
        if (!en.p || en.bytes < bytes) {
            if (en.p) dfree(en.p);
            en.p = dmalloc(bytes, false);
            if (!en.p) { (void)hipGetLastError(); en.bytes = 0; en.version = weights_version; return nullptr; }
            en.bytes = bytes; en.version = 0;
        }
        *fresh = en.version == weights_version && en.tag == tag;
        en.version = weights_version; en.tag = tag;
        return en.p;
    }
    bool derived_failed(Kind kind, const void* src) const {
        auto it = derived_.find(DKey{kind, src});
        return it != derived_.end() && !it->second.p && it->second.version == weights_version;
    }
    void dfree(void* ptr) {
        for (size_t i = 0; i < allocs.size(); ++i)
            if (allocs[i] == ptr) { allocs[i] = allocs.back(); allocs.pop_back(); (void)hipDeviceSynchronize(); (void)hipFree(ptr); return; }
    }
    ~Store() { for (void* a : allocs) (void)hipFree(a); }
    void* dmalloc(size_t bytes, bool zero) {
        void* p = nullptr;
        if (hipMalloc(&p, bytes ? bytes : 16) != hipSuccess) return nullptr;
        if (zero) (void)hipMemset(p, 0, bytes);
        allocs.push_back(p);
        return p;
    }
    Param* add(const std::string& key, std::vector<int64_t> shape, int kind, void* dev, int o_pad = 0, int i_pad = 0) {
        auto p = std::make_unique<Param>();
        p->key = key; p->shape = std::move(shape); p->kind = kind; p->dev = dev; p->o_pad = o_pad; p->i_pad = i_pad;
        Param* raw = p.get();
        by_key[key] = raw;
        params.push_back(std::move(p));
        return raw;
    }
    bf16_t* conv3(const std::string& pfx, int O, int I, float** bias) {
        int ip = pad8(I), op = pad8(O);
        bf16_t* w = (bf16_t*)dmalloc((size_t)op * 9 * ip * 2, true);
        add(pfx + ".weight", {O, I, 3, 3}, PK_CONV3, w, op, ip);
        float* b = (float*)dmalloc((size_t)pad8(O) * 4, true);
        add(pfx + ".bias", {O}, PK_VEC, b);
        *bias = b;
        return w;
    }
    bf16_t* mat(const std::string& pfx, int O, int I, bool conv1x1, bool has_bias, float** bias, int kind = PK_MAT) {
        int ip = pad8(I), op = pad8(O);
        bf16_t* w = (bf16_t*)dmalloc((size_t)op * ip * 2, true);
        std::vector<int64_t> shp = conv1x1 ? std::vector<int64_t>{O, I, 1, 1} : std::vector<int64_t>{O, I};
        add(pfx + ".weight", shp, kind, w, op, ip);
        if (bias) *bias = nullptr;
        if (has_bias) {
            float* b = (float*)dmalloc((size_t)op * 4, true);
            add(pfx + ".bias", {O}, kind == PK_MAT_GEGLU ? PK_VEC_GEGLU : PK_VEC, b);
            *bias = b;
        }
        return w;
    }
    void vec(const std::string& key, int n, float** out) {
        float* b = (float*)dmalloc((size_t)n * 4, true);
        add(key, {n}, PK_VEC, b);
        *out = b;
    }
    int locate(const char* key, int dtype, const int64_t* shape, int ndim, Param** out, const char* matrices_only = nullptr) {
        auto it = by_key.find(key);
        if (it == by_key.end()) GYRE_FAIL(GYRE_ERR_KEY, std::string("unknown weight key: ") + key);
        Param& p = *it->second;
        if (matrices_only && p.kind >= PK_MAT_HEAD30)
            GYRE_FAIL(GYRE_ERR_UNSUPPORTED, std::string(matrices_only) + " is not built for the SwinIR weight " + key);
        if (matrices_only && (p.kind == PK_VEC || p.kind == PK_VEC_GEGLU))
            GYRE_FAIL(GYRE_ERR_INVALID, std::string(matrices_only) + " applies to matrices and convolutions, not to the vector " + key);
        if (dtype < 0 || dtype > 2) GYRE_FAIL(GYRE_ERR_INVALID, "bad dtype");
        bool ok = (int)p.shape.size() == ndim;
        for (int i = 0; ok && i < ndim; ++i) ok = p.shape[i] == shape[i];
        if (!ok) {
            std::string m = std::string("shape mismatch for ") + key + ": expected [";
            for (auto d : p.shape) m += std::to_string(d) + ",";
            m += "] got [";
            for (int i = 0; i < ndim; ++i) m += std::to_string(shape[i]) + ",";
            GYRE_FAIL(GYRE_ERR_KEY, m + "]");
        }
        *out = &p;
        return 0;
    }
    void mark_set(Param& p, bool* was_set = nullptr) {
        if (was_set) *was_set = p.set;
        p.set = true;
        ++weights_version;
    }
    int set_weight(const char* key, const void* src, int dtype, const int64_t* shape, int ndim, hipStream_t st) {
        Param* pp;
        TRY(locate(key, dtype, shape, ndim, &pp));
        Param& p = *pp;
        int O = (int)p.shape[0];
// ... 40 lines not shown
        TRY(locate(key, dtype, shape, ndim, &pp, "a LoRA"));
        Param& p = *pp;
        if (n_pairs < 0 || n_pairs > GYRE_LORA_MAX_PAIRS || (n_pairs > 0 && !pairs)) GYRE_FAIL(GYRE_ERR_INVALID, "set_weight_lora: 0 to 8 LoRA pairs per call");
        LoraArgs la;
        la.n = n_pairs;
        for (int j = 0; j < n_pairs; ++j) {
            if (!pairs[j].up || !pairs[j].down) GYRE_FAIL(GYRE_ERR_INVALID, "set_weight_lora: null factor");
            if (pairs[j].dtype < 0 || pairs[j].dtype > 2) GYRE_FAIL(GYRE_ERR_INVALID, "set_weight_lora: bad factor dtype");
            if (pairs[j].rank < 1) GYRE_FAIL(GYRE_ERR_INVALID, "set_weight_lora: rank must be >= 1");
            la.up[j] = pairs[j].up; la.down[j] = pairs[j].down; la.dtype[j] = pairs[j].dtype; la.rank[j] = pairs[j].rank; la.s[j] = pairs[j].scale;
        }
        const int O = (int)p.shape[0], I = (int)p.shape[1];
        if (p.kind == PK_CONV3) {
            TRY(launch_repack_lora(st, src, dtype, O, I, 3, 3, p.i_pad, 0, 1.f, la, (bf16_t*)p.dev));
        } else if (p.kind == PK_MAT_GEGLU) {
            if (p.i_pad != I) GYRE_FAIL(GYRE_ERR_UNSUPPORTED, "geglu weight with padded K");
            TRY(launch_repack_lora(st, src, dtype, O, I, 1, 1, I, 1, 1.f, la, (bf16_t*)p.dev));
        } else {
            TRY(launch_repack_lora(st, src, dtype, O, I, 1, 1, p.i_pad, 0, p.scale, la, (bf16_t*)p.dev));
        }
        mark_set(p, was_set);
        return 0;
    }
    int set_weight_delta(const char* key, const void* src, int dtype, const int64_t* shape, int ndim, int n_terms,
                         const gyre_delta_term* terms, hipStream_t st, bool* was_set) {
        Param* pp;
        TRY(locate(key, dtype, shape, ndim, &pp, "a LyCORIS delta"));
        Param& p = *pp;
        DeltaArgs da;
        TRY(delta_terms_to_args(n_terms, terms, da));
        const int O = (int)p.shape[0], I = (int)p.shape[1];
        if (p.kind == PK_CONV3) {
            TRY(launch_repack_delta(st, src, dtype, O, I, 3, 3, p.i_pad, 0, 1.f, da, (bf16_t*)p.dev));
        } else if (p.kind == PK_MAT_GEGLU) {
            if (p.i_pad != I) GYRE_FAIL(GYRE_ERR_UNSUPPORTED, "geglu weight with padded K");
            TRY(launch_repack_delta(st, src, dtype, O, I, 1, 1, I, 1, 1.f, da, (bf16_t*)p.dev));
        } else {
            TRY(launch_repack_delta(st, src, dtype, O, I, 1, 1, p.i_pad, 0, p.scale, da, (bf16_t*)p.dev));
        }
        mark_set(p, was_set);
        return 0;
    }
    int finalize() {
        for (auto& p : params)
            if (!p->set) GYRE_FAIL(GYRE_ERR_INCOMPLETE, "weight not set: " + p->key);
        return 0;
    }
};

struct ResW {
    int cin = 0, cout = 0;
    float *n1g, *n1b, *n2g, *n2b;
    bf16_t *c1w, *c2w, *scw = nullptr;
    float *c1b, *c2b, *scb = nullptr;
    int temb_off = -1;
};
struct AttnW {
    int c = 0, heads = 1, kv_dim = 0;
    bf16_t *wqk = nullptr, *wq = nullptr, *wk = nullptr, *wv = nullptr, *wo = nullptr;
    int k_prescaled = 0;
    bool qkv_fused = false;
    float *bqk = nullptr, *bq = nullptr, *bk = nullptr, *bv = nullptr, *bo = nullptr;
};
struct TBlockW {
    float *ln1g, *ln1b, *ln2g, *ln2b, *ln3g, *ln3b;
    AttnW a1, a2;
    bf16_t *ff1, *ff2;
    float *ff1b, *ff2b;
};
struct TransW {
    int c = 0, heads = 1;
    float *ng, *nb;
    bf16_t *pin, *pout;
    float *pinb, *poutb;
    std::vector<TBlockW> blocks;
};
struct ConvW { bf16_t* w = nullptr; float* b = nullptr; int cin = 0, cout = 0; };

struct CtxKV { bf16_t* k; bf16_t* vt; };
struct MhaSave { Tn ao, qk, km, vm, idx; int idx_B = 0, idx_b0 = 0; };
struct ResSave { Tn h1; };
struct TBlockSave { Tn h0, n1, h1, n2, h2, n3; MhaSave a1, a2; };
struct TransSave { std::vector<TBlockSave> blocks; Tn hlast; };
struct Exec {
    Arena arena;
    hipStream_t st = nullptr;
    Store* store = nullptr;
    int groups = 32;
    std::string fail;
    const std::vector<CtxKV>* ctx_cache = nullptr;
    size_t ctx_layer = 0;
    int batch = 0;
    int cs_unit = 0;
    int tome_r = 0;
    int tiling = 0;
    bool keep_proj_out = false;
    int pout_fold_dry = -1;

    bool dry() const { return arena.dry; }
    int alloc(Tn& t, int B, int H, int W, int C, size_t elt = 2) {
        t.B = B; t.H = H; t.W = W; t.C = C;
        t.cs = nullptr; t.cs_off = (size_t)-1; t.cs_bytes = 0; t.cs_chunks = 0; t.cs_unit = 0;
        t.bytes = (size_t)B * H * W * C * elt;
        t.off = arena.alloc(t.bytes);
        if (t.off == (size_t)-1 || (!arena.dry && t.off + t.bytes > arena.cap))
            GYRE_FAIL(GYRE_ERR_WORKSPACE, "workspace too small: need " + std::to_string(t.bytes) + " B at offset " +
                      std::to_string((long long)t.off) + ", capacity " + std::to_string(arena.cap) + " B (tensor " +
                      std::to_string(B) + "x" + std::to_string(H) + "x" + std::to_string(W) + "x" + std::to_string(C) + ")");
        t.p = arena.dry ? nullptr : (bf16_t*)(arena.base + t.off);
        return 0;
    }
    int alloc_raw(Tn& t, size_t bytes) { return alloc(t, 1, 1, 1, (int)((bytes + 1) / 2)); }
    void free(Tn& t) {
        if (t.valid()) { arena.release(t.off, t.bytes); t.off = (size_t)-1; t.p = nullptr; }
        if (t.cs_off != (size_t)-1) { arena.release(t.cs_off, t.cs_bytes); t.cs_off = (size_t)-1; t.cs = nullptr; t.cs_chunks = 0; }
    }
    int attach_colstats(GemmParams& p, Tn& y, int rps) {
        if (!cs_unit || !store || rps <= 256 || (p.rowbias && p.rows_per_sample != rps)) return 0;
        if (!p.samples) p.samples = batch;
        GemmParams q = p;
        q.colstat_unit = cs_unit; q.rows_per_sample = rps;
        const int rows = gemm_plan(q).colstat_rows;
        if (rows <= 0 || rps / rows > 64) return 0;
        y.cs_chunks = rps / rows; y.cs_unit = cs_unit;
        y.cs_bytes = (size_t)y.B * y.cs_chunks * (p.N / cs_unit) * 2 * sizeof(float);
        y.cs_off = arena.alloc(y.cs_bytes);
        if (y.cs_off == (size_t)-1 || (!arena.dry && y.cs_off + y.cs_bytes > arena.cap))
            GYRE_FAIL(GYRE_ERR_WORKSPACE, "workspace too small (GroupNorm statistics)");
        y.cs = arena.dry ? nullptr : (float*)(arena.base + y.cs_off);
        p.colstat_unit = cs_unit; p.rows_per_sample = rps; p.colstat_out = y.cs;
        return 0;
    }

    int dup_batch(const Tn& x, Tn& y) {
        TRY(alloc(y, 2 * x.B, x.H, x.W, x.C));
        if (x.cs_chunks > 0) {
            y.cs_chunks = x.cs_chunks; y.cs_unit = x.cs_unit; y.cs_bytes = 2 * x.cs_bytes;
            y.cs_off = arena.alloc(y.cs_bytes);
            if (y.cs_off == (size_t)-1 || (!arena.dry && y.cs_off + y.cs_bytes > arena.cap))
                GYRE_FAIL(GYRE_ERR_WORKSPACE, "workspace too small (GroupNorm statistics)");
            y.cs = arena.dry ? nullptr : (float*)(arena.base + y.cs_off);
        }
        if (dry()) return 0;
        TRY(launch_dup_batch(st, x.p, y.p, 1, x.bytes));
        if (x.cs_chunks > 0) TRY(launch_dup_batch(st, x.cs, y.cs, 1, x.cs_bytes));
        return 0;
    }
    int groupnorm(const Tn& x, const Tn* x2, const float* g, const float* b, float eps, int silu, Tn& y) {
        int C = x.C + (x2 ? x2->C : 0);
        int HW = x.H * x.W;
        Tn ws;
        TRY(alloc_raw(ws, gn_workspace_bytes(x.B, HW, C, groups)));
        TRY(alloc(y, x.B, x.H, x.W, C));
        if (!dry()) {
            GnParams p;
            p.x = x.p; p.x2 = x2 ? x2->p : x.p; p.C1 = x.C; p.B = x.B; p.HW = HW; p.C = C; p.G = groups;
            p.gamma = g; p.beta = b; p.eps = eps; p.silu = silu;
            p.nchunks = gn_pick_chunks(x.B, HW, C);
            p.partial = (float*)ws.p;
            p.scale_shift = (float*)((char*)ws.p + align_up((size_t)x.B * p.nchunks * groups * 2 * sizeof(float), 256));
            p.y = y.p;
            if (gn_use_small(HW, C, x.C, groups)) {
                TRY(launch_groupnorm_small(st, p));
            } else {
                if (x.cs_chunks > 0 && (!x2 || (x2->cs_chunks > 0 && x2->cs_unit == x.cs_unit))) {
                    p.cs_unit = x.cs_unit;
                    if (gn_accepts_colstats(p)) {
                        p.cs_x = x.cs; p.cs_x_chunks = x.cs_chunks;
                        if (x2) { p.cs_x2 = x2->cs; p.cs_x2_chunks = x2->cs_chunks; }
                    }
                }
                if (!p.cs_x) TRY(launch_groupnorm_stats(st, p));
                TRY(launch_groupnorm_apply(st, p));
            }
        }
        free(ws);
        return 0;
    }
    int prep_ar(GemmParams& p, const GemmPlan& pl) {
        if (dry() || !pl.ar_pack) return 0;
        bool fresh = false;
        void* pk = store ? store->derived(Store::DC_PACKED, p.W, gemm_ar_packed_bytes(p.N, p.K), &fresh, pl.cfg) : nullptr;
        if (!pk) GYRE_FAIL(GYRE_ERR_HIP, "cannot allocate the packed weight copy of the A-resident GEMM");
        if (!fresh) TRY(launch_ar_pack(st, p.W, p.N, p.K, pk));
        p.w_packed = pk;
        return 0;
    }
    int prep_blk(GemmParams& p, const GemmPlan& pl) {
        if (dry() || !store || p.W_blk || !pl.w_block) return 0;
        bool fresh = false;
        bf16_t* b = (bf16_t*)store->derived(Store::DC_BLOCKED, p.W, (size_t)p.N * p.K * 2, &fresh);
        if (!b) return 0;
        if (!fresh) TRY(launch_w_block(st, p.W, p.N, p.K, b));
        p.W_blk = b;
        return 0;
    }
    int run_gemm(GemmParams& p) {
        if (!p.samples) p.samples = batch;
        const GemmPlan pl = gemm_plan(p);
        TRY(prep_ar(p, pl));
        TRY(prep_blk(p, pl));
        Tn ws;
        if (pl.ws_bytes) {
            TRY(alloc_raw(ws, pl.ws_bytes));
            p.splitk_ws = (float*)ws.p; p.splitk_ws_bytes = pl.ws_bytes;
        }
        int rc = dry() ? 0 : launch_gemm(st, p, pl);
        free(ws);
        return rc;
    }
    int conv3(const Tn& x, const ConvW& w, int stride, int pad, int ups, const float* rowbias, int ld_rowbias,
              const Tn* residual, Tn& y, int Hup = 0, int Wup = 0, const Tn* sc_x = nullptr, const Tn* sc_skip = nullptr,
              const bf16_t* sc_w = nullptr, const float* sc_b = nullptr) {
        if (ups && ((Hup && (Hup > 2 * x.H || Hup < 2 * x.H - 1)) || (Wup && (Wup > 2 * x.W || Wup < 2 * x.W - 1))))
            GYRE_FAIL(GYRE_ERR_INVALID, "upsample target must be 2x or 2x-1 of the input");
        int Hin = ups ? (Hup ? Hup : 2 * x.H) : x.H, Win = ups ? (Wup ? Wup : 2 * x.W) : x.W;
        int Ho = (Hin + (pad ? 2 : 1) - 3) / stride + 1, Wo = (Win + (pad ? 2 : 1) - 3) / stride + 1;
        TRY(alloc(y, x.B, Ho, Wo, pad8(w.cout)));
        GemmParams p;
        p.A = x.p; p.lda = x.C; p.mode = GEMM_CONV3;
        p.Hi = x.H; p.Wi = x.W; p.Cin = x.C; p.Ho = Ho; p.Wo = Wo; p.stride = stride; p.pad = pad; p.ups = ups;
        p.Hup = ups ? Hin : 0; p.Wup = ups ? Win : 0;
        p.W = w.w; p.K = 9 * x.C; p.N = pad8(w.cout); p.M = x.B * Ho * Wo;
        p.bias = w.b; p.rowbias = rowbias; p.rows_per_sample = Ho * Wo; p.ld_rowbias = ld_rowbias;
        if (residual) { p.residual = residual->p; p.ldr = residual->C; }
        p.out = y.p; p.ldc = y.C; p.out_mode = OUT_BF16;
        p.wrap = pad ? tiling : 0;
        if (sc_x) {
            fill_shortcut(p, *sc_x, sc_skip);
            if (!dry()) {
                bool fresh = false;
                const size_t wbytes = align_up((size_t)p.N * p.K * 2, 256);
                bf16_t* fw = (bf16_t*)store->derived(Store::DC_SHORTCUT, w.w, wbytes + align_up((size_t)p.N * 4, 256), &fresh);
                if (!fw) GYRE_FAIL(GYRE_ERR_HIP, "cannot allocate the folded conv + shortcut weights");
                float* fb = (float*)((char*)fw + wbytes);
                if (!fresh) {
                    TRY(launch_concat_rows(st, w.w, 9 * x.C, sc_w, p.sc_K, p.N, fw));
                    GYRE_HIP_CHECK(hipMemcpyAsync(fb, w.b, (size_t)p.N * sizeof(float), hipMemcpyDeviceToDevice, st));
                    if (sc_b) TRY(launch_add_f32(st, fb, sc_b, (size_t)p.N));
                }
                p.W = fw; p.bias = fb;
            }
        }
        TRY(attach_colstats(p, y, Ho * Wo));
        return run_gemm(p);
    }
    void fill_shortcut(GemmParams& p, const Tn& sx, const Tn* sskip) const {
        p.sc_A = sx.p; p.sc_lda = sx.C; p.sc_C1 = sx.C; p.sc_K = sx.C;
        if (sskip) { p.sc_A2 = sskip->p; p.sc_lda2 = sskip->C; p.sc_K = sx.C + sskip->C; }
        p.K = 9 * p.Cin + p.sc_K;
    }
    bool conv3_shortcut_foldable(const Tn& b, int cout, const Tn& sx, const Tn* sskip) {
        if (!store || tiling || b.C % 64 || sx.C % 64 || (sskip && sskip->C % 64) || sx.H != b.H || sx.W != b.W) return false;
        GemmParams p;
        p.A = b.p; p.lda = b.C; p.mode = GEMM_CONV3;
        p.Hi = b.H; p.Wi = b.W; p.Cin = b.C; p.Ho = b.H; p.Wo = b.W; p.stride = 1; p.pad = 1;
        p.N = pad8(cout); p.M = b.B * b.H * b.W; p.rows_per_sample = b.H * b.W; p.samples = batch;
        p.out = (void*)(uintptr_t)256; p.ldc = p.N; p.out_mode = OUT_BF16;
        if (dry()) p.A = (const bf16_t*)(uintptr_t)256;
        fill_shortcut(p, sx, sskip);
        if (dry()) { p.sc_A = (const bf16_t*)(uintptr_t)256; if (sskip) p.sc_A2 = (const bf16_t*)(uintptr_t)256; }
        return gemm_plan(p).shortcut_fold;
    }
    int conv3_nchw(const Tn& x, const ConvW& w, void* out, int out_dtype) {
        if (dry()) return 0;
        if (!tiling && conv_out_supports(x.C, w.cout))
            return launch_conv_out(st, x.p, x.B, x.H, x.W, x.C, w.w, w.b, w.cout, out, out_dtype);
        GemmParams p;
        p.A = x.p; p.lda = x.C; p.mode = GEMM_CONV3;
        p.Hi = x.H; p.Wi = x.W; p.Cin = x.C; p.Ho = x.H; p.Wo = x.W; p.stride = 1; p.pad = 1;
        p.W = w.w; p.K = 9 * x.C; p.N = w.cout; p.M = x.rows();
        p.bias = w.b; p.rows_per_sample = x.H * x.W;
        p.out = out; p.out_mode = OUT_NCHW; p.out_dtype = out_dtype; p.wrap = tiling;
        return launch_gemm(st, p);
    }
    struct RowStatBuf { Tn t; int nparts = 0; };
    int linear(const bf16_t* x, int lda, const bf16_t* x2, int lda2, int C1, int M, int K, const bf16_t* w, int N,
               const float* bias, const bf16_t* residual, int ldr, int geglu, bf16_t* y, int ldc, RowStatBuf* rs = nullptr,
               Tn* cs_for = nullptr) {
        GemmParams p;
        p.A = x; p.lda = lda; p.A2 = x2; p.lda2 = lda2; p.C1 = C1; p.mode = GEMM_LINEAR;
        if (dry() && lda2 > 0) { p.A = (const bf16_t*)(uintptr_t)256; p.A2 = (const bf16_t*)(uintptr_t)512; }
        p.W = w; p.K = K; p.N = N; p.M = M; p.bias = bias; p.residual = residual; p.ldr = ldr; p.geglu = geglu;
        p.out = y; p.ldc = ldc; p.out_mode = OUT_BF16;
        p.ar_ok = store != nullptr; p.no_ar = cs_for != nullptr;
        if (cs_for && !rs) TRY(attach_colstats(p, *cs_for, cs_for->H * cs_for->W));
        if (rs) {
            if (!p.samples) p.samples = batch;
            rs->nparts = store ? gemm_plan(p).rowstat_parts : 0;
            if (rs->nparts > 0) {
                TRY(alloc_raw(rs->t, (size_t)rs->nparts * M * 2 * sizeof(float)));
                p.rowstat_out = (float*)rs->t.p;
                if (dry()) p.rowstat_out = nullptr;
            }
        }
        return run_gemm(p);
    }
    int linear_t(const bf16_t* x, int lda, int M, int K, const bf16_t* w, int N, const float* bias, int tokens, int ldt,
                 bf16_t* y) {
        if (dry()) return 0;
        GemmParams p;
        p.A = x; p.lda = lda; p.mode = GEMM_LINEAR; p.W = w; p.K = K; p.N = N; p.M = M; p.bias = bias;
        p.out = y; p.out_mode = OUT_BF16_T; p.tokens_per_batch = tokens; p.ldt = ldt;
        return launch_gemm(st, p);
    }
    int gn_fold_linear(const Tn& x, const float* g, const float* b, float eps, const bf16_t* w, const float* bias, int N, Tn& y,
                       RowStatBuf* rs, bool* folded) {
        *folded = false;
        const int C = x.C, HW = x.H * x.W, M = x.rows();
        if (!store || HW < 8 * N || gn_use_small(HW, C, C, groups) || C % groups) return 0;
        GemmParams p;
        p.A = x.p; p.lda = C; p.mode = GEMM_LINEAR; p.W = w; p.K = C; p.N = N; p.M = M; p.samples = batch;
        p.out = y.p; p.ldc = y.C; p.out_mode = OUT_BF16; p.rows_per_sample = HW; p.ld_rowbias = N;
        p.rowbias = (const float*)(uintptr_t)256;
        const GemmPlan pl = gemm_plan(p);
        if (!pl.per_sample_w) return 0;
        Tn ws, wf, bfv;
        TRY(alloc_raw(ws, gn_workspace_bytes(x.B, HW, C, groups)));
        TRY(alloc_raw(wf, (size_t)x.B * N * C * 2));
        TRY(alloc_raw(bfv, (size_t)x.B * N * sizeof(float)));
        if (rs) {
            rs->nparts = pl.rowstat_parts;
            if (rs->nparts > 0) TRY(alloc_raw(rs->t, (size_t)rs->nparts * M * 2 * sizeof(float)));
        }
        if (!dry()) {
            GnParams gp;
            gp.x = x.p; gp.x2 = x.p; gp.C1 = C; gp.B = x.B; gp.HW = HW; gp.C = C; gp.G = groups;
            gp.gamma = g; gp.beta = b; gp.eps = eps; gp.silu = 0;
// ... 1043 lines not shown
```

include/gyre_hip.h:

```cpp
#ifndef GYRE_HIP_H
#define GYRE_HIP_H

#include <stddef.h>
#include <stdint.h>

#ifdef __cplusplus
extern "C" {
#endif

#define GYRE_ABI_VERSION 1

typedef enum { GYRE_F32 = 0, GYRE_BF16 = 1, GYRE_F16 = 2 } gyre_dtype;

typedef enum {
    GYRE_OK = 0,
    GYRE_ERR_INVALID = -1,
    GYRE_ERR_KEY = -2,
    GYRE_ERR_INCOMPLETE = -3,
    GYRE_ERR_WORKSPACE = -4,
    GYRE_ERR_HIP = -5,
    GYRE_ERR_UNSUPPORTED = -6
} gyre_status;

#define GYRE_MAX_LEVELS 8
// ... 178 lines not shown
size_t gyre_vae_workspace_bytes(gyre_vae* h, int B, int H, int W, int decode);
int gyre_vae_encode(gyre_vae* h, void* stream, const void* image_nchw, int in_dtype, int B, int H, int W,
                    void* workspace, size_t workspace_bytes, void* moments_out_nchw, int out_dtype);
int gyre_vae_decode(gyre_vae* h, void* stream, const void* z_nchw, int in_dtype, int B, int h_lat, int w_lat,
                    void* workspace, size_t workspace_bytes, void* image_out_nchw, int out_dtype);

int gyre_t2i_create(const gyre_t2i_cfg* cfg, int device, gyre_t2i** out);
void gyre_t2i_destroy(gyre_t2i* h);
int gyre_t2i_num_params(const gyre_t2i* h);
const char* gyre_t2i_param_key(const gyre_t2i* h, int i);
int gyre_t2i_set_weight(gyre_t2i* h, const char* key, const void* dev_ptr, int dtype, const int64_t* shape, int ndim, void* stream);
int gyre_t2i_finalize(gyre_t2i* h, void* stream);
size_t gyre_t2i_workspace_bytes(gyre_t2i* h, int B, int H, int W);
int gyre_t2i_forward(gyre_t2i* h, void* stream, const void* image_nchw, int in_dtype, int B, int H, int W,
                     void* workspace, size_t workspace_bytes, void* const* features_out_nchw, int n, int out_dtype);

int gyre_rrdb_create(const gyre_rrdb_cfg* cfg, int device, gyre_rrdb** out);
void gyre_rrdb_destroy(gyre_rrdb* h);
int gyre_rrdb_num_params(const gyre_rrdb* h);
const char* gyre_rrdb_param_key(const gyre_rrdb* h, int i);
int gyre_rrdb_set_weight(gyre_rrdb* h, const char* key, const void* dev_ptr, int dtype, const int64_t* shape, int ndim, void* stream);
int gyre_rrdb_finalize(gyre_rrdb* h, void* stream);
size_t gyre_rrdb_workspace_bytes(gyre_rrdb* h, int B, int H, int W);
int gyre_rrdb_forward(gyre_rrdb* h, void* stream, const void* image_nchw, int in_dtype, int B, int H, int W,
                      void* workspace, size_t workspace_bytes, void* out_nchw, int out_dtype);
int gyre_rrdb_set_path(gyre_rrdb* h, int path);

int gyre_swinir_create(const gyre_swinir_cfg* cfg, int device, gyre_swinir** out);
void gyre_swinir_destroy(gyre_swinir* h);
int gyre_swinir_num_params(const gyre_swinir* h);
const char* gyre_swinir_param_key(const gyre_swinir* h, int i);
int gyre_swinir_set_weight(gyre_swinir* h, const char* key, const void* dev_ptr, int dtype, const int64_t* shape, int ndim, void* stream);
int gyre_swinir_finalize(gyre_swinir* h, void* stream);
size_t gyre_swinir_workspace_bytes(gyre_swinir* h, int B, int H, int W);
int gyre_swinir_forward(gyre_swinir* h, void* stream, const void* image_nchw, int in_dtype, int B, int H, int W,
                        void* workspace, size_t workspace_bytes, void* out_nchw, int out_dtype);

int gyre_ctrl_create(const gyre_ctrl_cfg* cfg, int device, gyre_ctrl** out);
void gyre_ctrl_destroy(gyre_ctrl* h);
int gyre_ctrl_num_params(const gyre_ctrl* h);
const char* gyre_ctrl_param_key(const gyre_ctrl* h, int i);
int gyre_ctrl_set_weight(gyre_ctrl* h, const char* key, const void* dev_ptr, int dtype, const int64_t* shape, int ndim, void* stream);
int gyre_ctrl_finalize(gyre_ctrl* h, void* stream);
size_t gyre_ctrl_bind_workspace_bytes(gyre_ctrl* h, int image_B, int image_H, int image_W, int B);
int gyre_ctrl_bind(gyre_ctrl* h, void* stream, const void* image_nchw, int image_dtype, int image_B, int image_H, int image_W,
                   const void* context, int ctx_dtype, int B, int S, void* workspace, size_t workspace_bytes);
size_t gyre_ctrl_workspace_bytes(gyre_ctrl* h, int B, int H, int W, int S);
int gyre_ctrl_forward(gyre_ctrl* h, void* stream, const void* x_nchw, int x_dtype, const int64_t* t, int B, int H, int W,
                      void* workspace, size_t workspace_bytes, const float* scales, int accumulate, int out_B, int out_b0,
                      void* const* outs_nchw, int n_outs, int out_dtype);

int gyre_prof_set_mask(unsigned long long mask);
int gyre_prof_num_classes(void);
const char* gyre_prof_class_name(int kclass);
int gyre_prof_collect(int64_t* launches, double* ms, double* flops, double* bytes);

int gyre_debug_force_gemm_cfg(int cfg);
int gyre_debug_set_splitk_workspace(void* ws_dev, size_t bytes);
int gyre_debug_set_ar_workspace(void* ws_dev, size_t bytes);
int gyre_debug_set_wblk_workspace(void* ws_dev, size_t bytes);
int gyre_debug_force_attn_variant(int v);
long gyre_debug_attn_redo_count(void);
int gyre_debug_attn_plan(int B, int H, int Nq, int Nk, int D, int k_prescaled, int ldq, int ldk, int ldvt, int ldo, int32_t* out);
int gyre_debug_attn_bwd_plan(int B, int H, int Nq, int Nk, int D, int with_dk, int32_t* out);
int gyre_debug_attn_tables(int which, int32_t* out, int cap);
int gyre_debug_xattn_stamps(void* dev_buf);
int gyre_debug_gemm_ablation(int bits);
int gyre_debug_ln_linear_folds(int M, int K, int N, int geglu);
int gyre_debug_gn_uses_small(int HW, int C, int C1, int groups);
typedef struct gyre_gemm_test_args {
    int32_t conv, M, K, N, geglu;
    int32_t B, Hi, Wi, Cin, stride, pad, ups, Hup, Wup, wrap;
    int32_t C1, lda, lda2, ldc, ldr;
    int32_t rows_per_sample, ld_rowbias, samples;
    int32_t out_mode, out_dtype, tokens, ldt;
    int32_t colstat_unit;
    const void* A; const void* A2; const void* W;
    const float* bias; const float* rowbias; const void* residual;
    void* out; void* ws; size_t ws_bytes;
    const void* sc_A; const void* sc_A2; int32_t sc_K, sc_C1, sc_lda, sc_lda2;
} gyre_gemm_test_args;
int gyre_op_gemm_test(void* stream, const gyre_gemm_test_args* a);
int gyre_debug_gemm_plan(const gyre_gemm_test_args* a, int32_t* out);
int gyre_debug_gemm_tiles(int32_t* out, int cap);

int gyre_set_batch_invariant(int canonical_samples);
int gyre_get_batch_invariant(void);

int gyre_op_groupnorm(void* stream, const void* x, const void* x2, int C1, int B, int HW, int C, int groups,
                      const float* gamma, const float* beta, float eps, int silu,
                      void* workspace, size_t workspace_bytes, void* y);
size_t gyre_op_groupnorm_workspace(int B, int HW, int C, int groups);
size_t gyre_op_gemm_splitk_bytes(int conv, int M, int N, int K, int B);
int gyre_op_conv3x3_colstats(void* stream, const void* x, int B, int Hi, int Wi, int Cin, const void* w_repacked, int Cout,
                             const float* bias, const void* residual, int stride, int ups, int unit, void* y, float* stats_out,
                             size_t stats_bytes, void* workspace, size_t workspace_bytes, int* rows_out);
int gyre_op_linear_colstats(void* stream, const void* x, int M, int K, const void* w_bf16_rowmajor, int N, const float* bias,
                            const void* residual, int rows_per_sample, int unit, void* y, float* stats_out, size_t stats_bytes,
                            void* workspace, size_t workspace_bytes, int* rows_out);
int gyre_op_groupnorm_colstats(void* stream, const void* x, const void* x2, int C1, int B, int HW, int C, int groups,
                               const float* gamma, const float* beta, float eps, int silu, const float* cs_x, int cs_x_chunks,
                               const float* cs_x2, int cs_x2_chunks, int unit, void* workspace, size_t workspace_bytes, void* y);
int gyre_op_gn_fold(void* stream, const void* x, int B, int HW, int C, int groups, const float* gamma, const float* beta, float eps,
                    const void* W, const float* bias, int N, const float* cs_x, int cs_x_chunks, int unit,
                    void* workspace, size_t workspace_bytes, void* Wf_out, float* bf_out);
int gyre_op_layernorm(void* stream, const void* x, int M, int C, const float* gamma, const float* beta,
                      float eps, void* y);
int gyre_op_linear(void* stream, const void* x, int M, int K, const void* w_bf16_rowmajor, int N,
                   const float* bias, const void* residual, int geglu, void* y);
size_t gyre_op_ln_linear_workspace(int w_rows, int K, int M);
int gyre_op_ln_linear(void* stream, const void* x, int M, int K, const float* gamma, const float* beta, float eps,
                      const void* w_bf16_rowmajor, int N, const float* bias, int geglu, int qkv_tokens, void* vt_out, int ldt,
                      const float* row_parts, int n_parts, void* workspace, size_t workspace_bytes, void* y);
int gyre_op_linear_rowstats_parts(int M, int K, int N, int has_residual);
int gyre_op_linear_rowstats(void* stream, const void* x, int M, int K, const void* w_bf16_rowmajor, int N, const float* bias,
                            const void* residual, void* y, float* stats_out);
int gyre_op_linear_t(void* stream, const void* x, int M, int K, const void* w_bf16_rowmajor, int N,
                     const float* bias, int tokens_per_batch, int ldt, void* y);
int gyre_op_conv3x3(void* stream, const void* x, int B, int Hi, int Wi, int Cin, const void* w_krsc, int Cout,
                    const float* bias, const void* residual, int stride, int ups, int asym, void* y);
int gyre_op_conv3x3_shortcut(void* stream, const void* x, int B, int H, int W, int Cin, const void* w_krsc, int Cout, const float* bias,
                             const void* sx, int C1, const void* sx2, int C2, const void* w_sc, const float* bias_sc, void* ws,
                             size_t ws_bytes, void* y);
int gyre_op_compose_proj_out(void* stream, const void* wp, const void* w2, const float* b2, const float* bp, int C, void* wc_out,
                             float* bc_out);
int gyre_op_conv3x3_nchw(void* stream, const void* x, int B, int H, int W, int Cin, const void* w_krsc, int Cout,
                         const float* bias, void* y, int y_dtype, int force_tiles);
int gyre_op_repack_conv_weight(void* stream, const float* w_oihw, int Cout, int Cin, int KH, int KW, int Cin_pad,
                               void* w_krsc_bf16);
int gyre_op_repack_conv_weight_scaled(void* stream, const void* w_oihw, int dtype, int Cout, int Cin, int KH, int KW, int Cin_pad,
                                      float scale, void* w_krsc);
int gyre_op_repack_linear_weight(void* stream, const float* w_oi, int O, int I, int geglu_interleave, void* w_bf16);
int gyre_op_repack_bias(void* stream, const float* b, int n, int geglu_interleave, float* out);
int gyre_op_repack_lora(void* stream, const void* base, int base_dtype, int O, int I, int KH, int KW, int I_pad,
                        int geglu_interleave, float scale_p, int n_pairs, const gyre_lora_pair* pairs, void* out);
int gyre_op_repack_delta(void* stream, const void* base, int base_dtype, int O, int I, int KH, int KW, int I_pad,
                         int geglu_interleave, float scale_p, int n_terms, const gyre_delta_term* terms, void* out);
int gyre_op_lyco_core(void* stream, const void* core, int core_dtype, const void* right, int right_dtype, int A, int B, int C, int T,
                      float* out);
int gyre_op_merge_delta(void* stream, const void* base, int base_dtype, int O, int I, int n_terms, const gyre_delta_term* terms,
                        void* out, int out_dtype);
int gyre_op_attention(void* stream, const void* q, int ldq, const void* k, int ldk, const void* vt, int ldvt,
                      int B, int heads, int Nq, int Nk, int D, void* o, int ldo);
int gyre_op_qkv(void* stream, const void* x, int M, int C, const void* w_qkv, int tokens, void* qk_out, void* vt_out, int ldt);
int gyre_op_attention_ex(void* stream, const void* q, int ldq, const void* k, int ldk, const void* vt, int ldvt,
                         int B, int heads, int Nq, int Nk, int D, void* o, int ldo, int k_prescaled);
size_t gyre_vae_decode_vjp_workspace_bytes(gyre_vae* h, int B, int h_lat, int w_lat);
int gyre_vae_decode_vjp(gyre_vae* h, void* stream, const void* z_nchw, int z_dtype, int B, int h_lat, int w_lat,
                        const void* d_image_nchw, int d_dtype, void* workspace, size_t workspace_bytes,
                        void* image_out_nchw, int out_dtype, void* dz_out_nchw, int dz_dtype);

size_t gyre_op_groupnorm_bwd_workspace(int B, int HW, int C, int groups);
int gyre_op_groupnorm_bwd(void* stream, const void* x, const void* x2, int C1, int B, int HW, int C, int groups,
                          const float* gamma, const float* beta, float eps, int silu, const void* dy, const void* addend,
                          void* workspace, size_t workspace_bytes, void* dx, void* dx2);
int gyre_op_layernorm_bwd(void* stream, const void* x, const void* dy, int M, int C, const float* gamma, float eps,
                          const void* addend, void* dx);
int gyre_op_geglu_bwd(void* stream, const void* pre, const void* dy, int M, int F, void* dpre);
size_t gyre_op_attention_bwd_workspace(int B, int heads, int Nq, int Nk, int D);
int gyre_op_attention_bwd(void* stream, const void* q, int ldq, const void* k, int ldk, const void* v, int ldv,
                          const void* o, int ldo, const void* d_o, int lddo, int B, int heads, int Nq, int Nk, int D,
                          int k_prescaled, void* workspace, size_t workspace_bytes, void* dq, int lddq, void* dk, int lddk,
                          void* dv, int lddv);
size_t gyre_op_tome_workspace(int B, int N, int C);
int gyre_op_tome_merge(void* stream, const void* k, int ldk, const void* v, int ldv, int B, int N, int C, int r,
                       void* workspace, size_t workspace_bytes, void* k_out, void* vt_out, int ldvt,
// ... 40 lines not shown
```

Before: 9.083.

## Fold nearest-2x upsample into conv3x3 as four-parity 2x2 convolutions

Adds a four-parity form for the upsample-then-3x3-conv: the 3x3 weights are pre-summed into four 2x2 kernels, one per output parity, and the GEMM reads the low-resolution input directly with K=4*Cin instead of 9*Cin. Output rows are scattered back to the interleaved high-resolution layout in the epilogue. This cuts the MACs and input gathers of the upsampler convolutions by more than half. The cost is a cached composed-weight buffer, a restriction to the 256x320 pipelined tile, and extra index arithmetic in the epilogue.

```diff
diff --git a/gyre_amd/_lib.py b/gyre_amd/_lib.py
--- a/gyre_amd/_lib.py
+++ b/gyre_amd/_lib.py
@@ -94,6 +94,12 @@
                                          "out_mode", "out_dtype", "tokens", "ldt", "colstat_unit")] + \
                [(n, C.c_void_p) for n in ("A", "A2", "W", "bias", "rowbias", "residual", "out", "ws")] + [("ws_bytes", C.c_size_t)] + \
                [("sc_A", C.c_void_p), ("sc_A2", C.c_void_p)] + [(n, C.c_int32) for n in ("sc_K", "sc_C1", "sc_lda", "sc_lda2")]
+
+
+class UpsampleConvTestArgs(C.Structure):
+    _fields_ = [(n, C.c_int32) for n in ("B", "Hi", "Wi", "Cin", "N", "splits", "colstat_unit")] + \
+               [(n, C.c_void_p) for n in ("x", "w", "bias", "out", "colstat_out", "scratch")] + [("scratch_bytes", C.c_size_t)] + \
+               [("ws", C.c_void_p), ("ws_bytes", C.c_size_t)]
 
 
 class LoraPair(C.Structure):
@@ -209,6 +215,8 @@
     "gyre_op_gemm_test": (_i, [_vp, C.POINTER(GemmTestArgs)]),
     "gyre_debug_gemm_plan": (_i, [C.POINTER(GemmTestArgs), C.POINTER(C.c_int32)]),
     "gyre_debug_gemm_tiles": (_i, [C.POINTER(C.c_int32), _i]),
+    "gyre_debug_ups4_plan": (_i, [_i] * 9 + [C.POINTER(C.c_int32)]),
+    "gyre_op_upsample_conv_test": (_i, [_vp, C.POINTER(UpsampleConvTestArgs)]),
     "gyre_set_batch_invariant": (_i, [_i]),
     "gyre_get_batch_invariant": (_i, []),
     "gyre_op_groupnorm": (_i, [_vp, _vp, _vp, _i, _i, _i, _i, _i, _vp, _vp, _f, _i, _vp, _sz, _vp]),
diff --git a/gyre_amd/csrc/kernels.h b/gyre_amd/csrc/kernels.h
--- a/gyre_amd/csrc/kernels.h
+++ b/gyre_amd/csrc/kernels.h
@@ -55,6 +55,8 @@
     GEMM_DBG_NO_W_BLOCK       = 0x4000000,
     GEMM_DBG_TWO_STAGE_CONV   = 0x8000000,
     GEMM_DBG_NO_POUT_FOLD     = 0x10000000,
+    GEMM_DBG_NO_UPS4          = 0x20000000,
+    GEMM_DBG_UPS4_ALL         = 0x40000000,
 };
 int launch_groupnorm_stats(hipStream_t st, const GnParams& p);
 int launch_groupnorm_apply(hipStream_t st, const GnParams& p);
@@ -171,7 +173,10 @@
     size_t w_sample_stride = 0;
     const bf16_t* sc_A = nullptr; const bf16_t* sc_A2 = nullptr; int sc_lda = 0, sc_lda2 = 0, sc_C1 = 0, sc_K = 0;
     int wrap = 0;
-};
+    int ups4 = 0;
+};
+int launch_compose_ups4(hipStream_t st, const bf16_t* W, int N, int Cin, bf16_t* out);
+bool gemm4s_supports(const GemmParams& p, int cfg);
 int launch_concat_rows(hipStream_t st, const bf16_t* a, int K1, const bf16_t* b, int K2, int N, bf16_t* out);
 int launch_ln_fold(hipStream_t st, const bf16_t* W, int N, int K, const float* gamma, const float* beta, const float* bias,
                    bf16_t* Wf, float* colsum, float* bias_out);
diff --git a/gyre_amd/csrc/kernels_gemm.hip b/gyre_amd/csrc/kernels_gemm.hip
--- a/gyre_amd/csrc/kernels_gemm.hip
+++ b/gyre_amd/csrc/kernels_gemm.hip
@@ -1192,11 +1192,12 @@
 static int pick_cfg(const GemmParams& p, int* splits_out) {
     *splits_out = 1;
     const bool trans = p.out_mode == OUT_BF16_T;
-    auto tiles = [&](int bm, int bn) { return (long)((p.M + bm - 1) / bm) * ((p.N + bn - 1) / bn); };
+    auto mtiles = [&](int bm) { return p.ups4 ? 4L * ((p.M / 4 + bm - 1) / bm) : (long)((p.M + bm - 1) / bm); };
+    auto tiles = [&](int bm, int bn) { return mtiles(bm) * ((p.N + bn - 1) / bn); };
     auto tiles_of = [&](int id) { const GemmTile* t = gemm_tile(id); return tiles(t->bm, t->bn); };
     auto eff = [&](long t, int slots) { long cap = 256L * slots; long waves = (t + cap - 1) / cap; return (double)t / (double)(waves * cap); };
     auto neff = [&](int bn) { long nt = (p.N + bn - 1) / bn; return (double)p.N / (double)(nt * bn); };
-    auto meff = [&](int bm) { long mt = (p.M + bm - 1) / bm; return (double)p.M / (double)(mt * bm); };
+    auto meff = [&](int bm) { long mt = mtiles(bm); return (double)p.M / (double)(mt * bm); };
     double best = -1; int cfg = 3;
     auto consider = [&](int id, double speed, int slots) {
         const GemmTile* t = gemm_tile(id);
@@ -1207,6 +1208,7 @@
     consider(1, 0.55, 2);
     consider(2, 0.50, 2);
     const bool wrap_only4 = p.mode == GEMM_CONV3 && p.wrap != 0;
+    if (p.ups4 && (p.debug & GEMM_DBG_UPS4_ALL) && gemm4s_supports(p, 24)) return 24;
     if (!trans && p.batch <= 1 && (p.ar_ok || p.w_packed || g_dbg_ar_ws) && !p.no_ar && !(p.debug & GEMM_DBG_NO_AR) && p.M >= 4096 &&
         (p.N >= 3 * p.K || (p.debug & GEMM_DBG_AR_ALL)) && gemm_ar_supports(p) &&
         ((long)((p.M + 255) / 256) * gemm_ar_nsplit(p) >= ar_grid_min() || (p.debug & GEMM_DBG_AR_ALL)))
@@ -1335,6 +1337,7 @@
         if (!one_split) rows = cs_red_colblock(p.N, unit) <= 2048 ? cs_red_rows(p.rows_per_sample) : 0;
         else if (t->bn % unit == 0 && (t->kind != GEMM_K_4S || p.mode == GEMM_CONV3) && !(pl.cfg == 8 && (p.debug & GEMM_DBG_NO_CS_128x160)))
             rows = t->cs_rows;
+        if (rows && p.ups4 && one_split && (pl.cfg != 24 || ((long)p.Hi * p.Wi) % rows)) rows = 0;
         if (rows && p.rows_per_sample % rows == 0) pl.colstat_rows = rows;
     }
     return pl;
@@ -1375,6 +1378,35 @@
     GYRE_LAUNCH_CHECK();
     return 0;
 }
+__global__ __launch_bounds__(256) void k_compose_ups4(const bf16_t* __restrict__ W, int N, int Cin, bf16_t* __restrict__ out) {
+    const size_t t = (size_t)blockIdx.x * 256 + threadIdx.x;
+    const int cv = Cin >> 3;
+    if (t >= (size_t)16 * N * cv) return;
+    const int c = (int)(t % cv) * 8;
+    size_t q = t / cv;
+    const int tap = (int)(q & 3); q >>= 2;
+    const int n = (int)(q % N), par = (int)(q / N);
+    const int a = par >> 1, b = par & 1, ty = tap >> 1, tx = tap & 1;
+    const int ky0 = ty ? (a ? 2 : 1) : 0, ky1 = ty ? 2 : (a ? 1 : 0);
+    const int kx0 = tx ? (b ? 2 : 1) : 0, kx1 = tx ? 2 : (b ? 1 : 0);
+    float s[8] = {0.f, 0.f, 0.f, 0.f, 0.f, 0.f, 0.f, 0.f};
+    for (int ky = ky0; ky <= ky1; ++ky)
+        for (int kx = kx0; kx <= kx1; ++kx) {
+            float f[8];
+            unpack8(*(const uint4*)(W + ((size_t)n * 9 + ky * 3 + kx) * Cin + c), f);
+#pragma unroll
+            for (int e = 0; e < 8; ++e) s[e] += f[e];
+        }
+    const int r = par * N + n, k = tap * Cin + c, K4 = 4 * Cin;
+    *(uint4*)(out + ((size_t)(r >> 3) * (K4 >> 6) + (k >> 6)) * 512 + (r & 7) * 64 + (k & 63)) = pack8(s);
+}
+int launch_compose_ups4(hipStream_t st, const bf16_t* W, int N, int Cin, bf16_t* out) {
+    if (Cin % 64 || N % 8 || N < 8 || Cin < 64) GYRE_FAIL(-1, "compose_ups4: Cin must be a multiple of 64 and N of 8");
+    const size_t total = (size_t)16 * N * (Cin / 8);
+    hipLaunchKernelGGL(k_compose_ups4, dim3((unsigned)((total + 255) / 256)), dim3(256), 0, st, W, N, Cin, out);
+    GYRE_LAUNCH_CHECK();
+    return 0;
+}
 static thread_local bf16_t* g_dbg_blk_ws = nullptr;
 static thread_local size_t g_dbg_blk_ws_bytes = 0;
 extern "C" int gyre_debug_set_wblk_workspace(void* ws, size_t bytes) { g_dbg_blk_ws = (bf16_t*)ws; g_dbg_blk_ws_bytes = bytes; return 0; }
@@ -1385,7 +1417,10 @@
     if (p.K % 8) GYRE_FAIL(-1, "gemm: K must be a multiple of 8");
     if (p.C1 % 8) GYRE_FAIL(-1, "gemm: source split must be a multiple of 8");
     if (p.mode == GEMM_CONV3) {
-        if (p.Cin % 8 || p.K != 9 * p.Cin + p.sc_K) GYRE_FAIL(-1, "conv3x3: Cin must be a multiple of 8 and K == 9*Cin (+ the folded shortcut's channels)");
+        if (p.Cin % 8 || p.K != (p.ups4 ? 4 : 9) * p.Cin + p.sc_K)
+            GYRE_FAIL(-1, "conv3x3: Cin must be a multiple of 8 and K == 9*Cin (+ the folded shortcut's channels; four-parity upsampler form: 4*Cin)");
+        if (p.ups4 && (plan.cfg != 24 || !gemm4s_supports(p, 24)))
+            GYRE_FAIL(-6, "conv3x3: the four-parity upsampler form runs on the pipelined 256x320 tile only (exact 2x, one source, Cin % 64 == 0)");
         if (p.sc_K && (p.sc_K % BK || p.Cin % BK || !p.sc_A || p.stride != 1 || p.pad != 1 || p.ups || p.Hi != p.Ho || p.Wi != p.Wo || p.wrap ||
                        (p.sc_A2 && p.sc_A2 != p.sc_A && (p.sc_C1 <= 0 || p.sc_C1 >= p.sc_K || p.sc_C1 % BK))))
             GYRE_FAIL(-1, "conv3x3: a folded shortcut needs a stride-1 / pad-1 convolution and whole 64-channel steps on both sides");
@@ -1419,7 +1454,7 @@
         if (!p.splitk_ws) { p.splitk_ws = g_dbg_ws; p.splitk_ws_bytes = g_dbg_ws_bytes; }
         if (!p.splitk_ws || p.splitk_ws_bytes < (size_t)splits * p.M * p.N * sizeof(float)) {
             splits = 1;
-            cfg = pick_cfg_nosplit(p);
+            cfg = p.ups4 ? 24 : pick_cfg_nosplit(p);
         }
     }
     const GemmTile* t = gemm_tile(cfg);
diff --git a/gyre_amd/csrc/kernels_gemm4s.hip b/gyre_amd/csrc/kernels_gemm4s.hip
--- a/gyre_amd/csrc/kernels_gemm4s.hip
+++ b/gyre_amd/csrc/kernels_gemm4s.hip
@@ -20,13 +20,15 @@
     return srd_t{(int)(unsigned)a, (int)(unsigned)(a >> 32), (int)bytes, 0x00020000};
 }
 
-template <int BM, int BN, int WM, int WN, int MODE, int ZFILL, bool LNF = false, bool CS = false>
+template <int BM, int BN, int WM, int WN, int MODE, int ZFILL, bool LNF = false, bool CS = false, bool U4 = false>
 __global__ __launch_bounds__(WM * WN * 64, WM * WN / 4) void k_gemm4s(GemmParams p, int tiles_m, int tiles_n, int splits, int group_m) {
     constexpr int NW = WM * WN;
     constexpr int TM = BM / WM, TN = BN / WN, MI = TM / 32, NI = TN / 32;
     constexpr int AP = BM / (8 * NW), BP = BN / (8 * NW);
     constexpr int DTOT = AP + BP, DH0 = (DTOT + 1) / 2;
     constexpr int STAGE = (BM + BN) * 128;
+    constexpr int TAPS = U4 ? 4 : 9, TW = U4 ? 2 : 3;
+    static_assert(!U4 || (MODE == GEMM_CONV3 && ZFILL == 0 && !LNF), "the four-parity form is a convolution");
     static_assert((NW == 4 || NW == 8) && TM % 32 == 0 && TN % 32 == 0 && BM % (8 * NW) == 0 && BN % (8 * NW) == 0 &&
                   MI * NI * 16 <= (NW == 4 ? 256 : 160) && (NI == 4 || NI == 5), "tile shape");
     extern __shared__ __attribute__((aligned(16))) char smem[];
@@ -35,14 +37,18 @@
     const int split = blockIdx.x / ntiles;
     const int bid = xcd_tile_id(blockIdx.x - split * ntiles, ntiles);
     int tm, tn;
-    if ((long)p.M < (MODE == GEMM_CONV3 ? 9L : 1L) * p.N) { tn = bid / tiles_m; tm = bid - tn * tiles_m; }
+    if ((long)p.M < (MODE == GEMM_CONV3 ? (long)TAPS : 1L) * p.N) { tn = bid / tiles_m; tm = bid - tn * tiles_m; }
     else {
         const int per = group_m * tiles_n;
         const int g = bid / per, r = bid - g * per;
         const int rows = min(group_m, tiles_m - g * group_m);
         tn = r / rows; tm = g * group_m + (r - tn * rows);
     }
-    const int m0 = tm * BM, n0 = tn * BN;
+    int par = 0, tml = tm;
+    if (U4) { const int tpp = tiles_m >> 2; par = tm / tpp; tml = tm - par * tpp; }
+    const int Mr = U4 ? p.M >> 2 : p.M;
+    const int m0 = tml * BM, n0 = tn * BN;
+    [[maybe_unused]] int m0p = U4 ? m0 | par : 0;
     const int tid = threadIdx.x, lane = tid & 63;
     const int w = __builtin_amdgcn_readfirstlane(tid >> 6);
     const int wm = w / WN, wn = w - wm * WN;
@@ -63,11 +69,13 @@
         vo_w[i] = p.W_blk ? (unsigned)(n >> 3) * (unsigned)(p.K >> 6) * 1024u + (unsigned)(n & 7) * 128u + kvs * 16u
                           : (unsigned)n * (unsigned)p.K * 2u + kvs * 16u;
     }
-    const char* w_tile = p.W_blk ? (const char*)(p.W_blk + (size_t)(n0 >> 3) * (p.K >> 6) * 512) : (const char*)(p.W + (size_t)n0 * p.K);
+    const int n0w = U4 ? par * p.N + n0 : n0;
+    const char* w_tile = p.W_blk ? (const char*)(p.W_blk + (size_t)(n0w >> 3) * (p.K >> 6) * 512) : (const char*)(p.W + (size_t)n0w * p.K);
     const bool wblk = p.W_blk != nullptr;
     unsigned vo_a[AP];
     int a_sbp[AP], a_y0[AP], a_x0[AP];
-    const int hw_o = MODE == GEMM_CONV3 ? p.Ho * p.Wo : 1;
+    const int hw_o = MODE == GEMM_CONV3 ? (U4 ? p.Hi * p.Wi : p.Ho * p.Wo) : 1;
+    const int w_o = U4 ? p.Wi : p.Wo;
     const int ns0 = m0 / hw_o;
 #pragma unroll
     for (int i = 0; i < AP; ++i) {
@@ -77,27 +85,27 @@
             vo_a[i] = rl * (unsigned)p.lda * 2u + kvs * 16u;
         } else {
             const int n = row / hw_o, rem = row - n * hw_o;
-            const int oy = rem / p.Wo, ox = rem - oy * p.Wo;
+            const int oy = rem / w_o, ox = rem - oy * w_o;
             a_sbp[i] = (n - ns0) * p.Hi * p.Wi;
-            a_y0[i] = row < p.M ? oy * p.stride - p.pad : 0x40000000;
-            a_x0[i] = ox * p.stride - p.pad;
+            a_y0[i] = row < Mr ? (U4 ? oy - 1 + (par >> 1) : oy * p.stride - p.pad) : 0x40000000;
+            a_x0[i] = U4 ? ox - 1 + (par & 1) : ox * p.stride - p.pad;
         }
     }
     const char* a_tile = (const char*)(p.A + (size_t)m0 * p.lda);
     int a_split = (MODE == GEMM_LINEAR && p.A2 != p.A) ? p.C1 : 0x7fffffff;
-    const int Hlim = p.ups ? (p.Hup ? p.Hup : 2 * p.Hi) : p.Hi, Wlim = p.ups ? (p.Wup ? p.Wup : 2 * p.Wi) : p.Wi;
-    const int ups = p.ups ? 1 : 0;
+    const int Hlim = (p.ups && !U4) ? (p.Hup ? p.Hup : 2 * p.Hi) : p.Hi, Wlim = (p.ups && !U4) ? (p.Wup ? p.Wup : 2 * p.Wi) : p.Wi;
+    const int ups = (p.ups && !U4) ? 1 : 0;
     const size_t spix = (size_t)ns0 * p.Hi * p.Wi;
     const char* cA = (const char*)(p.A + spix * p.lda);
     const char* cA2 = (const char*)(p.A2 + spix * p.lda2);
     srd_t srdA{}, srdA2{};
     if (MODE == GEMM_CONV3 && ZFILL == 0) {
-        const size_t left = (size_t)(p.M / hw_o - ns0) * p.Hi * p.Wi;
+        const size_t left = (size_t)(Mr / hw_o - ns0) * p.Hi * p.Wi;
         const size_t b1 = left * p.lda * 2, b2 = left * p.lda2 * 2;
         srdA = make_srd(cA, (unsigned)(b1 < 0x7ffffff0ull ? b1 : 0x7ffffff0ull));
         srdA2 = make_srd(cA2, (unsigned)(b2 < 0x7ffffff0ull ? b2 : 0x7ffffff0ull));
     }
-    const int nk_conv = MODE == GEMM_CONV3 ? 9 * (p.Cin / BK) : 0;
+    const int nk_conv = MODE == GEMM_CONV3 ? TAPS * (p.Cin / BK) : 0;
     int src_C1 = p.C1;
     unsigned src_ld = (unsigned)p.lda * 2u, src_ld2 = (unsigned)p.lda2 * 2u;
     bool on_shortcut = false;
@@ -129,7 +137,7 @@
                     cA2 = (const char*)(p.sc_A2 + spix * p.sc_lda2);
                     src_C1 = p.sc_C1; src_ld = (unsigned)p.sc_lda * 2u; src_ld2 = (unsigned)p.sc_lda2 * 2u;
                     if (ZFILL == 0) {
-                        const size_t left = (size_t)(p.M / hw_o - ns0) * p.Hi * p.Wi;
+                        const size_t left = (size_t)(Mr / hw_o - ns0) * p.Hi * p.Wi;
                         const size_t b1 = left * p.sc_lda * 2, b2 = left * p.sc_lda2 * 2;
                         srdA = make_srd(cA, (unsigned)(b1 < 0x7ffffff0ull ? b1 : 0x7ffffff0ull));
                         srdA2 = make_srd(cA2, (unsigned)(b2 < 0x7ffffff0ull ? b2 : 0x7ffffff0ull));
@@ -137,10 +145,10 @@
                 }
                 c0 = (kc - nk_conv) * BK;
                 s.ky = p.pad; s.kx = p.pad;
-                kw = 9 * p.Cin + c0;
+                kw = TAPS * p.Cin + c0;
             } else {
-                const int chunk = kc / 9, tap = kc - chunk * 9;
-                s.ky = tap / 3; s.kx = tap - s.ky * 3;
+                const int chunk = kc / TAPS, tap = kc - chunk * TAPS;
+                s.ky = tap / TW; s.kx = tap - s.ky * TW;
                 c0 = chunk * BK;
                 kw = tap * p.Cin + c0;
             }
@@ -271,20 +279,40 @@
     __builtin_amdgcn_s_barrier();
 
     const int hi = lane >> 5, l31 = lane & 31;
-    const int m_base = m0 + wm * TM, n_base = n0 + wn * TN;
+    int m0e = m0, pare = 0;
+    if constexpr (U4) {
+        asm volatile("" : "+s"(m0p));
+        m0e = m0p & ~3; pare = m0p & 3;
+    }
+    const int m_base = m0e + wm * TM, n_base = n0 + wn * TN;
+    int e_Hi = 0, e_Wi = 0, e_Mr = Mr;
+    if constexpr (U4) {
+        auto* ka = __builtin_amdgcn_kernarg_segment_ptr();
+        asm volatile("" : "+s"(ka));
+        const auto* pk = (const __attribute__((address_space(4))) GemmParams*)ka;
+        e_Hi = pk->Hi; e_Wi = pk->Wi; e_Mr = pk->M >> 2;
+    }
+    auto out_row = [&](int m) {
+        if (!U4) return m;
+        const int hw = e_Hi * e_Wi;
+        const int n = m / hw, rem = m - n * hw;
+        const int i = rem / e_Wi, j = rem - i * e_Wi;
+        return n * 4 * hw + (2 * i + (pare >> 1)) * 2 * e_Wi + 2 * j + (pare & 1);
+    };
     if (!LNF && !CS && splits > 1) {
         float* slab = p.splitk_ws + (size_t)split * p.M * p.N;
 #pragma unroll
         for (int i = 0; i < MI; ++i) {
             const int m = m_base + i * 32 + l31;
-            if (m >= p.M) continue;
+            if (m >= e_Mr) continue;
+            const int mo = out_row(m);
 #pragma unroll
             for (int j = 0; j < NI; ++j)
 #pragma unroll
                 for (int g = 0; g < 4; ++g) {
                     const int n = n_base + j * 32 + 8 * g + 4 * hi;
                     if (n < p.N)
-                        *(float4*)(slab + (size_t)m * p.N + n) =
+                        *(float4*)(slab + (size_t)mo * p.N + n) =
                             make_float4(acc[i][j][4 * g], acc[i][j][4 * g + 1], acc[i][j][4 * g + 2], acc[i][j][4 * g + 3]);
                 }
         }
@@ -320,7 +348,8 @@
 #pragma unroll
             for (int i = 0; i < MI; ++i) {
                 const int m = m_base + i * 32 + l31;
-                const float* rbias = (p.rowbias && m < p.M) ? p.rowbias + (size_t)(m / p.rows_per_sample) * p.ld_rowbias : nullptr;
+                const int mo = m < e_Mr ? out_row(m) : -1;
+                const float* rbias = (p.rowbias && m < e_Mr) ? p.rowbias + (size_t)(mo / p.rows_per_sample) * p.ld_rowbias : nullptr;
 #pragma unroll
                 for (int j = j0; j < j1; ++j)
 #pragma unroll
@@ -334,8 +363,8 @@
                         *(float4*)(slabc + l31 * ROWC + (j - j0) * 32 + 8 * g + 4 * hi) = o;
                     }
                 for (int row = r0; row < 32; row += R) {
-                    const int mm = m_base + i * 32 + row;
-                    if (mm < p.M && nn < p.N) {
+                    const int mm = U4 ? __shfl(mo, row) : m_base + i * 32 + row;
+                    if ((U4 ? mm >= 0 : mm < p.M) && nn < p.N) {
                         const float4 a = *(const float4*)(slabc + row * ROWC + c8 * 8);
                         const float4 b = *(const float4*)(slabc + row * ROWC + c8 * 8 + 4);
                         float f[8] = {a.x, a.y, a.z, a.w, b.x, b.y, b.z, b.w};
@@ -383,7 +412,9 @@
             if (n < p.N) {
                 float su = 0.f, sq = 0.f;
                 for (int c = 0; c < unit; ++c) { const float2 v = chan[u * unit + c]; su += v.x; sq += v.y; }
-                ((float2*)p.colstat_out)[(size_t)tm * (p.N / unit) + n / unit] = make_float2(su, sq);
+                int blk = tm;
+                if (U4) { const int tle = m0e / BM, tps = e_Hi * e_Wi / BM, ns = tle / tps; blk = ns * 4 * tps + pare * tps + (tle - ns * tps); }
+                ((float2*)p.colstat_out)[(size_t)blk * (p.N / unit) + n / unit] = make_float2(su, sq);
             }
         }
         return;
@@ -398,7 +429,8 @@
 #pragma unroll
     for (int i = 0; i < MI; ++i) {
         const int m = m_base + i * 32 + l31;
-        const float* rbias = (p.rowbias && m < p.M) ? p.rowbias + (size_t)(m / p.rows_per_sample) * p.ld_rowbias : nullptr;
+        const int mo = m < e_Mr ? out_row(m) : -1;
+        const float* rbias = (p.rowbias && m < e_Mr) ? p.rowbias + (size_t)(mo / p.rows_per_sample) * p.ld_rowbias : nullptr;
         float lrstd = 1.f, lrmu = 0.f;
         if constexpr (LNF) {
             if (m < p.M) {
@@ -464,8 +496,8 @@
             const int n_pass = (gg ? n_base / 2 + j0 * 16 : n_base + j0 * 32);
             for (int v = lane; v < 32 * vpr; v += 64) {
                 const int row = v / vpr, c8 = v - row * vpr;
-                const int mm = m_base + i * 32 + row, nn = n_pass + c8 * 8;
-                if (mm < p.M && nn < n_out) {
+                const int mm = U4 ? __shfl(mo, row) : m_base + i * 32 + row, nn = n_pass + c8 * 8;
+                if ((U4 ? mm >= 0 : mm < p.M) && nn < n_out) {
                     const float4 a = *(const float4*)(slab + row * ROWF + c8 * 8);
                     const float4 b = *(const float4*)(slab + row * ROWF + c8 * 8 + 4);
                     float f[8] = {a.x, a.y, a.z, a.w, b.x, b.y, b.z, b.w};
@@ -496,9 +528,12 @@
         if (p.K % BK) return false;
         if (p.A2 && p.A2 != p.A && (cfg != 24 || p.C1 <= 0 || p.C1 >= p.K || p.C1 % BK || p.lda2 % 8 || ((size_t)p.A2 & 15))) return false;
     }
-    else if (p.Cin % BK || c1 % BK || p.K != 9 * p.Cin + p.sc_K || (p.sc_K && (p.sc_K % BK || cfg != 24))) return false;
+    else if (p.Cin % BK || c1 % BK || p.K != (p.ups4 ? 4 : 9) * p.Cin + p.sc_K || (p.sc_K && (p.sc_K % BK || cfg != 24))) return false;
+    if (p.ups4 && (p.mode != GEMM_CONV3 || cfg != 24 || p.sc_K || (p.A2 && p.A2 != p.A) || p.stride != 1 || p.pad != 1 || p.wrap ||
+                   p.Ho != 2 * p.Hi || p.Wo != 2 * p.Wi || p.Hi <= 0 || p.Wi <= 0 || p.M % (4 * p.Hi * p.Wi) || p.ln_colsum || p.geglu))
+        return false;
     if (p.mode == GEMM_CONV3) {
-        const size_t span = ((size_t)256 / ((size_t)p.Ho * p.Wo) + 2) * p.Hi * p.Wi;
+        const size_t span = ((size_t)256 / (p.ups4 ? (size_t)p.Hi * p.Wi : (size_t)p.Ho * p.Wo) + 2) * p.Hi * p.Wi;
         const size_t ld = p.lda > p.lda2 ? p.lda : p.lda2;
         if (span >= (1u << 24) || ld * 2 >= (1u << 24) || span * ld * 2 >= 0x7ff00000ull) return false;
     }
@@ -508,10 +543,11 @@
 
 template <int BM, int BN, int WM, int WN>
 static int launch_cfg4s(hipStream_t st, const GemmParams& p, int kcls_base, int splits) {
-    const int tiles_m = (p.M + BM - 1) / BM, tiles_n = (p.N + BN - 1) / BN;
+    const int tiles_m = p.ups4 ? 4 * ((p.M / 4 + BM - 1) / BM) : (p.M + BM - 1) / BM, tiles_n = (p.N + BN - 1) / BN;
     const int nk_all = (p.K + BK - 1) / BK;
     if (splits > nk_all) splits = nk_all;
     while (splits > 1 && (splits - 1) * ((nk_all + splits - 1) / splits) >= nk_all) --splits;
+    if ((long)tiles_m * tiles_n * splits > 0x7fffffffL) GYRE_FAIL(-6, "gemm: grid too large");
     const int grid = tiles_m * tiles_n * splits;
     constexpr int NW = WM * WN, NI = BN / WN / 32, JP = NW == 8 ? (NI + 1) / 2 : NI;
     constexpr size_t ring = (size_t)2 * (BM + BN) * 128,
@@ -534,7 +570,30 @@
             (void)hipFuncSetAttribute((const void*)kern, hipFuncAttributeMaxDynamicSharedMemorySize, (int)lds);     \
         hipLaunchKernelGGL(kern, dim3(grid), dim3(NW * 64), lds, st, p, tiles_m, tiles_n, splits, group_m);             \
     } while (0)
-    if (p.mode == GEMM_LINEAR && p.ln_colsum) {
+    if (p.ups4) {
+        if constexpr (BM == 256 && BN == 320 && NW == 8) {
+            if (!p.W_blk) GYRE_FAIL(-6, "gemm: the four-parity upsampler form reads the composed weights in blocked order (GemmParams::W_blk)");
+            static_assert(std::is_same<decltype(&k_gemm4s<BM, BN, WM, WN, GEMM_CONV3, 0, false, false, true>), void (*)(GemmParams, int, int, int, int)>::value &&
+                          std::is_same<decltype(&k_gemm4s<BM, BN, WM, WN, GEMM_CONV3, 0, false, true, true>), void (*)(GemmParams, int, int, int, int)>::value,
+                          "GemmParams must be the first argument of k_gemm4s");
+            if (p.colstat_out && splits == 1) {
+                if ((p.Hi * p.Wi) % BM) GYRE_FAIL(-6, "gemm: the four-parity form emits column statistics for Hi * Wi % 256 == 0 only");
+                auto kern = k_gemm4s<BM, BN, WM, WN, GEMM_CONV3, 0, false, true, true>;
+                static std::atomic<unsigned long long> attr_done{0};
+                if (gyre_lds_attr_needed(attr_done))
+                    (void)hipFuncSetAttribute((const void*)kern, hipFuncAttributeMaxDynamicSharedMemorySize, (int)lds);
+                hipLaunchKernelGGL(kern, dim3(grid), dim3(NW * 64), lds, st, p, tiles_m, tiles_n, splits, group_m);
+            } else {
+                auto kern = k_gemm4s<BM, BN, WM, WN, GEMM_CONV3, 0, false, false, true>;
+                static std::atomic<unsigned long long> attr_done{0};
+                if (gyre_lds_attr_needed(attr_done))
+                    (void)hipFuncSetAttribute((const void*)kern, hipFuncAttributeMaxDynamicSharedMemorySize, (int)lds);
+                hipLaunchKernelGGL(kern, dim3(grid), dim3(NW * 64), lds, st, p, tiles_m, tiles_n, splits, group_m);
+            }
+        } else {
+            GYRE_FAIL(-6, "gemm: the four-parity upsampler form exists for the 8-wave 256x320 pipelined tile only");
+        }
+    } else if (p.mode == GEMM_LINEAR && p.ln_colsum) {
         if constexpr (BM == 256 && BN == 320 && NW == 8) {
             auto kern = k_gemm4s<BM, BN, WM, WN, GEMM_LINEAR, 0, true>;
             static std::atomic<unsigned long long> attr_done{0};
diff --git a/gyre_amd/csrc/model.hip b/gyre_amd/csrc/model.hip
--- a/gyre_amd/csrc/model.hip
+++ b/gyre_amd/csrc/model.hip
@@ -786,6 +786,52 @@
     out[8] = pl.per_sample_w ? 1 : 0; out[9] = pl.shortcut_fold ? 1 : 0; out[10] = nst; out[11] = uni;
     return 0;
 }
+static int ups4_test_problem(GemmParams& p, int B, int Hi, int Wi, int Cin, int N, int Hup, int Wup) {
+    if (B <= 0 || Hi <= 0 || Wi <= 0 || Cin <= 0 || N <= 0 || B > 4096 || Hi > 2048 || Wi > 2048 || Cin > 65536 || N > (1 << 20) || Cin % 8 || N % 8)
+        GYRE_FAIL(GYRE_ERR_INVALID, "ups4: sizes must be positive, Cin and N multiples of 8");
+    if ((Hup != 0 && Hup != 2 * Hi && Hup != 2 * Hi - 1) || (Wup != 0 && Wup != 2 * Wi && Wup != 2 * Wi - 1))
+        GYRE_FAIL(GYRE_ERR_INVALID, "ups4: the upsample target must be 2x or 2x-1 of the input");
+    const int Ho = Hup ? Hup : 2 * Hi, Wo = Wup ? Wup : 2 * Wi;
+    if ((long)B * Ho * Wo > (1 << 24)) GYRE_FAIL(GYRE_ERR_INVALID, "ups4: too many output pixels");
+    p.mode = GEMM_CONV3; p.lda = Cin; p.Hi = Hi; p.Wi = Wi; p.Cin = Cin; p.Ho = Ho; p.Wo = Wo; p.stride = 1; p.pad = 1; p.ups = 1;
+    p.Hup = Ho; p.Wup = Wo; p.K = 9 * Cin; p.N = N; p.M = B * Ho * Wo; p.rows_per_sample = Ho * Wo; p.samples = B;
+    p.ldc = N; p.out_mode = OUT_BF16;
+    return 0;
+}
+int gyre_debug_ups4_plan(int B, int Hi, int Wi, int Cin, int N, int Hup, int Wup, int tiling, int colstat_unit, int32_t* out) {
+    if (!out || tiling < 0 || tiling > 3 || colstat_unit < 0) GYRE_FAIL(GYRE_ERR_INVALID, "ups4_plan: bad argument");
+    GemmParams p, p4;
+    GemmPlan pl;
+    TRY(ups4_test_problem(p, B, Hi, Wi, Cin, N, Hup, Wup));
+    const bool take = conv3_ups4_rule(p, tiling, B, colstat_unit, &p4, &pl);
+    out[0] = take ? 1 : 0; out[1] = take ? pl.cfg : 0; out[2] = take ? pl.splits : 0; out[3] = take ? pl.colstat_rows : 0;
+    return 0;
+}
+int gyre_op_upsample_conv_test(void* st, const gyre_upsample_conv_test_args* a) {
+    if (!a || !a->x || !a->w || !a->out || !a->scratch) GYRE_FAIL(GYRE_ERR_INVALID, "upsample_conv_test: null argument");
+    if (a->splits < 0 || a->splits > 64 || a->colstat_unit < 0 || (a->colstat_out && a->colstat_unit <= 0))
+        GYRE_FAIL(GYRE_ERR_INVALID, "upsample_conv_test: bad splits / colstat_unit");
+    if (((size_t)a->x & 15) || ((size_t)a->w & 15) || ((size_t)a->out & 15) || ((size_t)a->scratch & 15) || ((size_t)a->bias & 15) ||
+        ((size_t)a->colstat_out & 7) || ((size_t)a->ws & 15))
+        GYRE_FAIL(GYRE_ERR_INVALID, "upsample_conv_test: pointers need 16-byte alignment");
+    GemmParams p, p4;
+    GemmPlan pl;
+    TRY(ups4_test_problem(p, a->B, a->Hi, a->Wi, a->Cin, a->N, 0, 0));
+    if (a->splits > 1) p.force_cfg = 24 | (a->splits << 8);
+    p.A = (const bf16_t*)a->x; p.W = (const bf16_t*)a->w; p.bias = a->bias; p.out = a->out;
+    if (!conv3_ups4_rule(p, 0, a->B, a->colstat_out ? a->colstat_unit : 0, &p4, &pl))
+        GYRE_FAIL(GYRE_ERR_UNSUPPORTED, "upsample_conv_test: the four-parity form is not taken for this shape under the calling thread's planner state (gyre_debug_ups4_plan)");
+    if (a->scratch_bytes < (size_t)16 * a->N * a->Cin * 2) GYRE_FAIL(GYRE_ERR_WORKSPACE, "upsample_conv_test: scratch below 16 N Cin elements");
+    if (pl.splits > 1 && (!a->ws || a->ws_bytes < pl.ws_bytes)) GYRE_FAIL(GYRE_ERR_WORKSPACE, "upsample_conv_test: the plan runs in K slices and needs its slab space in ws");
+    if (a->colstat_out) {
+        if (pl.colstat_rows <= 0) GYRE_FAIL(GYRE_ERR_UNSUPPORTED, "upsample_conv_test: no column statistics for this shape / plan");
+        p4.colstat_unit = a->colstat_unit; p4.colstat_out = a->colstat_out;
+    }
+    TRY(launch_compose_ups4((hipStream_t)st, p.W, a->N, a->Cin, (bf16_t*)a->scratch));
+    p4.W = (const bf16_t*)a->scratch; p4.W_blk = p4.W;
+    p4.splitk_ws = (float*)a->ws; p4.splitk_ws_bytes = a->ws ? a->ws_bytes : 0;
+    return launch_gemm((hipStream_t)st, p4, pl);
+}
 int gyre_debug_gemm_tiles(int32_t* out, int cap) { return gemm_tile_table(out, out ? cap : 0); }
 int gyre_op_ln_linear(void* st, const void* x, int M, int K, const float* gamma, const float* beta, float eps, const void* w,
                       int N, const float* bias, int geglu, int qkv_tokens, void* vt_out, int ldt, const float* row_parts,
diff --git a/gyre_amd/csrc/model_impl.h b/gyre_amd/csrc/model_impl.h
--- a/gyre_amd/csrc/model_impl.h
+++ b/gyre_amd/csrc/model_impl.h
@@ -101,6 +101,7 @@
         DC_BLOCKED,
         DC_SHORTCUT,
         DC_PROJ_OUT,
+        DC_UPS4,
         DC_WIN_BIAS,
         DC_RDB_CHUNKED
     };
@@ -122,6 +123,10 @@
         *fresh = en.version == weights_version && en.tag == tag;
         en.version = weights_version; en.tag = tag;
         return en.p;
+    }
+    void derived_unfilled(Kind kind, const void* src) {
+        auto it = derived_.find(DKey{kind, src});
+        if (it != derived_.end() && it->second.p) it->second.version = 0;
     }
     bool derived_failed(Kind kind, const void* src) const {
         auto it = derived_.find(DKey{kind, src});
@@ -328,6 +333,21 @@
 struct ResSave { Tn h1; };
 struct TBlockSave { Tn h0, n1, h1, n2, h2, n3; MhaSave a1, a2; };
 struct TransSave { std::vector<TBlockSave> blocks; Tn hlast; };
+static inline bool conv3_ups4_rule(const GemmParams& p9, int tiling, int batch, int cs_unit, GemmParams* p4, GemmPlan* pl) {
+    if (!p9.ups || p9.mode != GEMM_CONV3 || p9.stride != 1 || p9.pad != 1 || tiling || p9.wrap || p9.A2 || p9.sc_K) return false;
+    if (p9.Hi <= 0 || p9.Wi <= 0 || p9.Ho != 2 * p9.Hi || p9.Wo != 2 * p9.Wi || p9.Cin % 64 || p9.lda % 8 || p9.N % 8) return false;
+    if (gemm_get_batch_invariant() > 0 || (gemm_planner_state() & GEMM_DBG_NO_UPS4)) return false;
+    GemmParams q = p9;
+    q.ups4 = 1; q.K = 4 * q.Cin;
+    if (!q.samples) q.samples = batch;
+    GemmParams qs = q;
+    qs.colstat_unit = cs_unit; qs.colstat_out = nullptr;
+    *pl = gemm_plan(qs);
+    if (pl->cfg != 24 || !gemm4s_supports(q, 24)) return false;
+    *p4 = q;
+    return true;
+}
+
 struct Exec {
     Arena arena;
     hipStream_t st = nullptr;
@@ -488,8 +508,43 @@
                 p.W = fw; p.bias = fb;
             }
         }
+        GemmParams p4; GemmPlan pl4;
+        if (!sc_x && store && conv3_ups4_rule(p, tiling, batch, cs_unit, &p4, &pl4)) return conv3_ups4(p, p4, w, y);
         TRY(attach_colstats(p, y, Ho * Wo));
         return run_gemm(p);
+    }
+    int conv3_ups4(GemmParams& p9, GemmParams& p4, const ConvW& w, Tn& y) {
+        p4.out = y.p;
+        TRY(attach_colstats(p4, y, p4.Ho * p4.Wo));
+        const GemmPlan pl = gemm_plan(p4);
+        Tn ws;
+        if (pl.ws_bytes) TRY(alloc_raw(ws, pl.ws_bytes));
+        int rc = 0;
+        if (!dry()) {
+            bf16_t* cw = nullptr;
+            if (!store->derived_failed(Store::DC_UPS4, w.w)) {
+                bool fresh = false;
+                cw = (bf16_t*)store->derived(Store::DC_UPS4, w.w, (size_t)16 * p4.N * p4.Cin * 2, &fresh);
+                if (cw && !fresh) {
+                    rc = launch_compose_ups4(st, w.w, p4.N, p4.Cin, cw);
+                    if (rc) store->derived_unfilled(Store::DC_UPS4, w.w);
+                }
+            }
+            if (cw && !rc) {
+                p4.W = cw; p4.W_blk = cw;
+                p4.splitk_ws = (float*)ws.p; p4.splitk_ws_bytes = pl.ws_bytes;
+                rc = launch_gemm(st, p4, pl);
+            } else if (!rc) {
+                y.cs_chunks = 0;
+                p9.samples = batch;
+                const GemmPlan pl9 = gemm_plan(p9);
+                rc = prep_blk(p9, pl9);
+                p9.splitk_ws = (float*)ws.p; p9.splitk_ws_bytes = pl.ws_bytes;
+                if (!rc) rc = launch_gemm(st, p9, pl9);
+            }
+        }
+        free(ws);
+        return rc;
     }
     void fill_shortcut(GemmParams& p, const Tn& sx, const Tn* sskip) const {
         p.sc_A = sx.p; p.sc_lda = sx.C; p.sc_C1 = sx.C; p.sc_K = sx.C;
diff --git a/include/gyre_hip.h b/include/gyre_hip.h
--- a/include/gyre_hip.h
+++ b/include/gyre_hip.h
@@ -284,6 +284,15 @@
 } gyre_gemm_test_args;
 int gyre_op_gemm_test(void* stream, const gyre_gemm_test_args* a);
 int gyre_debug_gemm_plan(const gyre_gemm_test_args* a, int32_t* out);
+int gyre_debug_ups4_plan(int B, int Hi, int Wi, int Cin, int N, int Hup, int Wup, int tiling, int colstat_unit, int32_t* out);
+typedef struct gyre_upsample_conv_test_args {
+    int32_t B, Hi, Wi, Cin, N, splits, colstat_unit;
+    const void* x; const void* w; const float* bias;
+    void* out; float* colstat_out;
+    void* scratch; size_t scratch_bytes;
+    void* ws; size_t ws_bytes;
+} gyre_upsample_conv_test_args;
+int gyre_op_upsample_conv_test(void* stream, const gyre_upsample_conv_test_args* a);
 int gyre_debug_gemm_tiles(int32_t* out, int cap);
 
 int gyre_set_batch_invariant(int canonical_samples);
```

New measurement: 9.306 (median of 6 runs). 2.4% higher.
